# leejaeyong7/tiny-cuda-nn

Measured on AMD Instinct MI355X. Metric: training_step throughput (samples/s) HashGrid+64-wide FFMLP, batch=256k; % fp16-MFMA peak, higher is better.
Workload: dtype f16

## Files before the change

### include/tcnn_amd.h

```cpp
#ifndef TCNN_AMD_H
#define TCNN_AMD_H

#include <stddef.h>
#include <stdint.h>

#ifdef __cplusplus
extern "C" {
#endif

#define TCNN_OK 0
#define TCNN_ERROR 1

#define TCNN_PRECISION_FP32 0
#define TCNN_PRECISION_FP16 1

#define TCNN_GRADIENT_IGNORE 0
#define TCNN_GRADIENT_OVERWRITE 1
#define TCNN_GRADIENT_ACCUMULATE 2

#define TCNN_LAYOUT_SOA 0
#define TCNN_LAYOUT_AOS 1

#define TCNN_LOG_INFO 0
#define TCNN_LOG_DEBUG 1
// ... 55 lines not shown
size_t      tcnn_module_n_params(tcnn_module_t m);
int         tcnn_module_param_precision(tcnn_module_t m);
int         tcnn_module_output_precision(tcnn_module_t m);
int         tcnn_module_initialize_params(tcnn_module_t m, uint64_t seed, float* params_full_precision, float scale);
const char* tcnn_module_hyperparams(tcnn_module_t m);
const char* tcnn_module_name(tcnn_module_t m);

int  tcnn_create_from_config(uint32_t n_input_dims, uint32_t n_output_dims, const char* config_json, tcnn_trainer_t* out);
int  tcnn_create_from_config_seeded(uint32_t n_input_dims, uint32_t n_output_dims, const char* config_json, uint32_t seed, tcnn_trainer_t* out);
int  tcnn_create_from_config_precision(uint32_t n_input_dims, uint32_t n_output_dims, const char* config_json, uint32_t seed, int precision, tcnn_trainer_t* out);
int  tcnn_trainer_precision(tcnn_trainer_t t);
void tcnn_trainer_destroy(tcnn_trainer_t t);

int  tcnn_trainer_training_step(tcnn_trainer_t t, tcnn_stream_t stream, uint32_t n_elements, const float* input, int input_layout,
                                const float* target, const float* data_pdf, int run_optimizer, float* dL_dinput, int use_inference_params,
                                int gradient_mode, const void* external_dL_dy, tcnn_train_ctx_t* ctx_out);
int  tcnn_trainer_loss(tcnn_trainer_t t, tcnn_stream_t stream, tcnn_train_ctx_t ctx, float* loss_out);
int  tcnn_trainer_forward(tcnn_trainer_t t, tcnn_stream_t stream, float loss_scale, uint32_t n_elements, const float* input, int input_layout, const float* target,
                          const float* data_pdf, int use_inference_params, int prepare_input_gradients, const void* external_dL_dy, tcnn_train_ctx_t* ctx_out);
int  tcnn_trainer_backward(tcnn_trainer_t t, tcnn_stream_t stream, tcnn_train_ctx_t ctx, uint32_t n_elements, const float* input, int input_layout,
                           float* dL_dinput, int use_inference_params, int gradient_mode);
int  tcnn_trainer_optimizer_step(tcnn_trainer_t t, tcnn_stream_t stream, float loss_scale);
void tcnn_train_ctx_destroy(tcnn_train_ctx_t ctx);
const void*  tcnn_train_ctx_output(tcnn_train_ctx_t ctx);
const void*  tcnn_train_ctx_dL_doutput(tcnn_train_ctx_t ctx);
const float* tcnn_train_ctx_L(tcnn_train_ctx_t ctx);

int  tcnn_trainer_inference(tcnn_trainer_t t, tcnn_stream_t stream, uint32_t n_elements, const float* input, int input_layout,
                            float* output, int output_layout, int use_inference_params);
int  tcnn_trainer_inference_mixed_precision(tcnn_trainer_t t, tcnn_stream_t stream, uint32_t n_elements, const float* input, int input_layout,
                                            void* output_half, int use_inference_params);

size_t   tcnn_trainer_n_params(tcnn_trainer_t t);
uint32_t tcnn_trainer_padded_output_width(tcnn_trainer_t t);
float*   tcnn_trainer_params_full_precision(tcnn_trainer_t t);
void*    tcnn_trainer_params(tcnn_trainer_t t);
void*    tcnn_trainer_params_inference(tcnn_trainer_t t);
void*    tcnn_trainer_param_gradients(tcnn_trainer_t t);
int      tcnn_trainer_set_params_full_precision(tcnn_trainer_t t, const float* params, size_t n_params, int device_ptr);
int      tcnn_trainer_set_params(tcnn_trainer_t t, const void* params_half, size_t n_params, int device_ptr);
int      tcnn_trainer_initialize_params(tcnn_trainer_t t);
int      tcnn_trainer_update_hyperparams(tcnn_trainer_t t, const char* json);
const char* tcnn_trainer_hyperparams(tcnn_trainer_t t);
int      tcnn_trainer_serialize(tcnn_trainer_t t, int serialize_optimizer, const void** out_bytes, size_t* out_size);
int      tcnn_trainer_deserialize(tcnn_trainer_t t, const void* bytes, size_t size);
const char* tcnn_trainer_network_hyperparams(tcnn_trainer_t t);
uint32_t tcnn_trainer_optimizer_step_count(tcnn_trainer_t t);
int  tcnn_trainer_profile_next_step(tcnn_trainer_t t);
int  tcnn_trainer_profile_collect(tcnn_trainer_t t, tcnn_stream_t stream, float* ms_per_piece , uint32_t* n_steps);
size_t tcnn_trainer_params_updated_in_flush(tcnn_trainer_t t);
size_t tcnn_trainer_image_preps(tcnn_trainer_t t);
size_t tcnn_trainer_scatter_wide_fallbacks(tcnn_trainer_t t);
size_t tcnn_trainer_optimizer_prologue_steps(tcnn_trainer_t t);
size_t tcnn_trainer_list_scatters(tcnn_trainer_t t);
size_t tcnn_module_list_scatters(tcnn_module_t m);
size_t tcnn_trainer_list_gradient_tails(tcnn_trainer_t t);
const char* tcnn_trainer_last_step_kernel(tcnn_trainer_t t);

int   tcnn_module_set_max_level(tcnn_module_t m, float max_level);
float tcnn_module_max_level(tcnn_module_t m);
int   tcnn_module_set_max_level_gpu(tcnn_module_t m, const float* per_sample);
int   tcnn_trainer_set_max_level(tcnn_trainer_t t, float max_level);
int   tcnn_trainer_set_max_level_gpu(tcnn_trainer_t t, const float* per_sample);
float tcnn_trainer_max_level(tcnn_trainer_t t);
int tcnn_train_ctx_keeps_weight_gradient_slabs(tcnn_trainer_t t, tcnn_train_ctx_t ctx);


int         tcnn_module_layer_sizes(tcnn_module_t m, uint32_t* rows_cols, size_t capacity, size_t* n_layers_out);
int         tcnn_optimizer_create(const char* optimizer_json, size_t n_params, const uint32_t* layer_sizes, size_t n_layers, tcnn_optimizer_t* out);
int         tcnn_optimizer_create_precision(const char* optimizer_json, size_t n_params, const uint32_t* layer_sizes, size_t n_layers, int weight_precision, tcnn_optimizer_t* out);
int         tcnn_optimizer_weight_precision(tcnn_optimizer_t o);
void        tcnn_optimizer_destroy(tcnn_optimizer_t o);
int         tcnn_optimizer_step(tcnn_optimizer_t o, tcnn_stream_t stream, float loss_scale, float* params_full_precision, void* params_half,
                                const void* gradients, int gradient_precision);
uint32_t    tcnn_optimizer_step_count(tcnn_optimizer_t o);
size_t      tcnn_optimizer_n_params(tcnn_optimizer_t o);
float       tcnn_optimizer_learning_rate(tcnn_optimizer_t o);
int         tcnn_optimizer_set_learning_rate(tcnn_optimizer_t o, float learning_rate);
int         tcnn_optimizer_update_hyperparams(tcnn_optimizer_t o, const char* json);
const char* tcnn_optimizer_hyperparams(tcnn_optimizer_t o);
void*       tcnn_optimizer_custom_weights(tcnn_optimizer_t o);
int         tcnn_optimizer_weights_restored(tcnn_optimizer_t o, tcnn_stream_t stream, const void* params_half);
int         tcnn_optimizer_serialize(tcnn_optimizer_t o, const void** out_bytes, size_t* out_size);
int         tcnn_optimizer_deserialize(tcnn_optimizer_t o, const void* bytes, size_t size);

#ifdef __cplusplus
}
#endif
#endif
```

### tiny-cuda-nn_amd/csrc/capi.cpp

```cpp
#include "../../include/tcnn_amd.h"

#include "model.h"

#include <mutex>
#include <string>

using namespace tcnn_amd;

namespace {
thread_local std::string g_last_error;
tcnn_amd::Switches g_switches;
std::mutex g_switches_mutex;

bool env_is(const char* name, char c) {
	const char* e = getenv(name);
	return e && e[0] == c;
}
int env_01(const char* name) {
	const char* e = getenv(name);
	return (e && (e[0] == '0' || e[0] == '1')) ? e[0] - '0' : -1;
}

template <typename F>
int guarded(F&& f) {
// ... 22 lines not shown
	std::string name_text;
};

struct tcnn_context_s {
	std::unique_ptr<ModelContext> ctx;
};

struct tcnn_trainer_s {
	std::unique_ptr<Trainer> trainer;
	std::string hyperparams_text;
	std::string network_hyperparams_text;
	std::vector<uint8_t> snapshot;
};

struct tcnn_train_ctx_s {
	std::unique_ptr<TrainContext> ctx;
};

struct tcnn_optimizer_s {
	std::unique_ptr<Optimizer> optimizer;
	size_t n_params = 0;
	std::string hyperparams_text;
	std::vector<uint8_t> snapshot;
};

namespace tcnn_amd {
Switches switches() {
	std::lock_guard<std::mutex> lock{g_switches_mutex};
	return g_switches;
}
void switches_reload() {
	Switches w;
	w.grid_planes = !env_is("TCNN_AMD_GRID_PLANES", '0');
	w.grid_rows_planes = !env_is("TCNN_AMD_GRID_ROWS_PLANES", '0');
	{ const char* e = getenv("TCNN_AMD_GRID_SCATTER"); w.grid_scatter_lds = !(e && std::string{e} == "atomic"); }
	w.scatter_records = !env_is("TCNN_AMD_SCATTER_RECORDS", '0');
	w.scatter_tune = !env_is("TCNN_AMD_SCATTER_TUNE", '0');
	w.scatter_lists = env_01("TCNN_AMD_SCATTER_LISTS");
	w.scatter_wide = env_is("TCNN_AMD_SCATTER_WIDE", '1');
	w.fused_step = !env_is("TCNN_AMD_FUSED_STEP", '0');
	w.side_jobs = !env_is("TCNN_AMD_SIDE_JOBS", '0');
	w.live_image = !env_is("TCNN_AMD_LIVE_IMAGE", '0');
	w.adam_steps32 = env_is("TCNN_AMD_ADAM_STEPS32", '1');
	w.adam_in_reduce = !env_is("TCNN_AMD_ADAM_IN_REDUCE", '0');
	w.adam_prologue = !env_is("TCNN_AMD_ADAM_PROLOGUE", '0');
	w.adam_prologue_refused = env_is("TCNN_AMD_ADAM_PROLOGUE", 'r');
	w.mlp_r32 = !env_is("TCNN_AMD_MLP_R32", '0');
	w.mlp_r32a = env_01("TCNN_AMD_MLP_R32A");
	w.mlp_regs = !env_is("TCNN_AMD_MLP_REGS", '0');
	w.mlp_fast = !env_is("TCNN_AMD_MLP_FAST", '0');
	if (const char* e = getenv("TCNN_AMD_MLP_PRIO")) w.mlp_prio = (uint32_t)atoi(e);
	w.listgrad_in_mlp = !env_is("TCNN_AMD_LISTGRAD_IN_MLP", '0');
	w.mlp_layerwise = env_is("TCNN_AMD_MLP_LAYERWISE", '1');
	std::lock_guard<std::mutex> lock{g_switches_mutex};
	g_switches = w;
}
}

extern "C" {

const char* tcnn_last_error(void) { return g_last_error.c_str(); }
const char* tcnn_version(void) { return "tcnn_amd 0.1 (gfx950)"; }

uint32_t tcnn_batch_size_granularity(void) { return BATCH_SIZE_GRANULARITY; }

int tcnn_device(int* device_out) {
	return guarded([&] { HIP_CHECK_THROW(hipGetDevice(device_out)); });
}

int tcnn_set_device(int device) {
	return guarded([&] { HIP_CHECK_THROW(hipSetDevice(device)); });
}

void tcnn_free_temporary_memory(void) { Arena::instance().release_all(); }

int tcnn_gpu_malloc(size_t bytes, void** out) {
	return guarded([&] {
		CHECK_THROW(out != nullptr);
		*out = nullptr;
		if (bytes) HIP_CHECK_THROW(hipMalloc(out, bytes));
	});
}
int tcnn_gpu_free(void* ptr) {
	return guarded([&] { if (ptr) HIP_CHECK_THROW(hipFree(ptr)); });
}
int tcnn_gpu_memcpy(void* dst, const void* src, size_t bytes, int kind) {
	return guarded([&] {
		const hipMemcpyKind k = kind == TCNN_MEMCPY_HOST_TO_DEVICE ? hipMemcpyHostToDevice : kind == TCNN_MEMCPY_DEVICE_TO_HOST ? hipMemcpyDeviceToHost : hipMemcpyDeviceToDevice;
		if (bytes) HIP_CHECK_THROW(hipMemcpy(dst, src, bytes, k));
	});
}
int tcnn_gpu_memset(void* ptr, int value, size_t bytes) {
	return guarded([&] { if (bytes) HIP_CHECK_THROW(hipMemset(ptr, value, bytes)); });
}
int tcnn_stream_synchronize(tcnn_stream_t stream) {
	return guarded([&] { HIP_CHECK_THROW(hipStreamSynchronize((hipStream_t)stream)); });
}
int tcnn_generate_random_uniform(tcnn_stream_t stream, uint64_t rng_state_inc[2], size_t n, float* out, float lower, float upper) {
	return guarded([&] {
		CHECK_THROW(rng_state_inc != nullptr && (out != nullptr || n == 0));
		generate_random_uniform((hipStream_t)stream, rng_state_inc, n, out, lower, upper);
		HIP_CHECK_THROW(hipGetLastError());
	});
}
int tcnn_has_networks(void) { return 1; }
float tcnn_default_loss_scale(int precision) { return precision == TCNN_PRECISION_FP32 ? 1.0f : LOSS_SCALE_FP16; }
// ... 206 lines not shown

int tcnn_trainer_backward(tcnn_trainer_t t, tcnn_stream_t stream, tcnn_train_ctx_t ctx, uint32_t n, const float* input, int input_layout, float* dL_dinput,
                          int use_inference_params, int gradient_mode) {
	return guarded([&] {
		CHECK_THROW(t && t->trainer && ctx && ctx->ctx);
		Trainer& tr = *t->trainer;
		const uint32_t w = tr.model().input_width();
		MatViewMut dx = make_view_mut(dL_dinput, w, n, input_layout);
		tr.backward((hipStream_t)stream, *ctx->ctx, n, make_view(input, w, n, input_layout), dL_dinput ? &dx : nullptr, use_inference_params != 0, (GradientMode)gradient_mode);
	});
}

int tcnn_trainer_optimizer_step(tcnn_trainer_t t, tcnn_stream_t stream, float loss_scale) {
	return guarded([&] {
		CHECK_THROW(t && t->trainer);
		t->trainer->optimizer_step((hipStream_t)stream, loss_scale);
	});
}

void tcnn_train_ctx_destroy(tcnn_train_ctx_t ctx) { delete ctx; }
const void* tcnn_train_ctx_output(tcnn_train_ctx_t ctx) { return ctx->ctx->output.data(); }
const void* tcnn_train_ctx_dL_doutput(tcnn_train_ctx_t ctx) {
	if (guarded([&] { ctx->ctx->materialize(); }) != 0) return nullptr;
	return ctx->ctx->dL_doutput_ptr;
}
const float* tcnn_train_ctx_L(tcnn_train_ctx_t ctx) {
	if (guarded([&] { ctx->ctx->materialize(); }) != 0) return nullptr;
	return ctx->ctx->L.as<float>();
}

int tcnn_trainer_inference(tcnn_trainer_t t, tcnn_stream_t stream, uint32_t n, const float* input, int input_layout, float* output, int output_layout, int use_inference_params) {
	return guarded([&] {
		CHECK_THROW(t && t->trainer);
		Trainer& tr = *t->trainer;
		tr.inference((hipStream_t)stream, n, make_view(input, tr.model().input_width(), n, input_layout), make_view_mut(output, tr.model().output_width(), n, output_layout),
		             use_inference_params != 0);
	});
}

int tcnn_trainer_inference_mixed_precision(tcnn_trainer_t t, tcnn_stream_t stream, uint32_t n, const float* input, int input_layout, void* output_half, int use_inference_params) {
	return guarded([&] {
		CHECK_THROW(t && t->trainer && (output_half || n == 0));
		Trainer& tr = *t->trainer;
		tr.inference_mixed_precision((hipStream_t)stream, n, make_view(input, tr.model().input_width(), n, input_layout), output_half, use_inference_params != 0);
	});
}

size_t tcnn_trainer_n_params(tcnn_trainer_t t) { return t->trainer->n_params(); }
size_t tcnn_trainer_params_updated_in_flush(tcnn_trainer_t t) { return t->trainer->params_updated_in_flush(); }
size_t tcnn_trainer_image_preps(tcnn_trainer_t t) { return t->trainer->image_preps(); }
size_t tcnn_trainer_optimizer_prologue_steps(tcnn_trainer_t t) {
	try { return (size_t)t->trainer->prologue_steps(); } catch (const std::exception& e) { g_last_error = e.what(); return (size_t)-1; }
}
size_t tcnn_trainer_scatter_wide_fallbacks(tcnn_trainer_t t) {
	try { return (size_t)t->trainer->scatter_wide_fallbacks(); } catch (const std::exception& e) { g_last_error = e.what(); return (size_t)-1; }
}
size_t tcnn_trainer_list_scatters(tcnn_trainer_t t) { return (size_t)t->trainer->list_scatters(); }
size_t tcnn_trainer_list_gradient_tails(tcnn_trainer_t t) { return (size_t)t->trainer->list_gradient_tails(); }
const char* tcnn_trainer_last_step_kernel(tcnn_trainer_t t) { return t->trainer->last_step_kernel(); }
int tcnn_trainer_set_max_level(tcnn_trainer_t t, float max_level) {
	return guarded([&] {
		CHECK_THROW(t && t->trainer);
		if (!t->trainer->model().set_max_level(max_level)) no_grid(t->trainer->model());
	});
}
int tcnn_trainer_set_max_level_gpu(tcnn_trainer_t t, const float* per_sample) {
	return guarded([&] {
		CHECK_THROW(t && t->trainer);
		if (!t->trainer->model().set_max_level_gpu(per_sample)) no_grid(t->trainer->model());
	});
}
float tcnn_trainer_max_level(tcnn_trainer_t t) {
	float v = std::numeric_limits<float>::quiet_NaN();
	const float* per_sample = nullptr;
	guarded([&] {
		CHECK_THROW(t && t->trainer);
		if (!t->trainer->model().get_max_level(v, per_sample)) no_grid(t->trainer->model());
		g_last_error.clear();
	});
	return v;
}
int tcnn_train_ctx_keeps_weight_gradient_slabs(tcnn_trainer_t t, tcnn_train_ctx_t ctx) {
	return (t && ctx && ctx->ctx && ctx->ctx->model_ctx && t->trainer->model().context_keeps_slabs(*ctx->ctx->model_ctx)) ? 1 : 0;
}
uint32_t tcnn_trainer_padded_output_width(tcnn_trainer_t t) { return t->trainer->model().padded_output_width(); }
float* tcnn_trainer_params_full_precision(tcnn_trainer_t t) { return t->trainer->params_full_precision(); }
void* tcnn_trainer_params(tcnn_trainer_t t) { return t->trainer->params(); }
void* tcnn_trainer_params_inference(tcnn_trainer_t t) {
	void* p = t->trainer->params_inference();
	return p == t->trainer->params_unexposed() ? t->trainer->params() : p;
}
void* tcnn_trainer_param_gradients(tcnn_trainer_t t) { return t->trainer->param_gradients(); }

int tcnn_trainer_set_params_full_precision(tcnn_trainer_t t, const float* params, size_t n_params, int device_ptr) {
	return guarded([&] { t->trainer->set_params_full_precision(params, n_params, device_ptr != 0); });
}

int tcnn_trainer_set_params(tcnn_trainer_t t, const void* params_half, size_t n_params, int device_ptr) {
	return guarded([&] { t->trainer->set_params(params_half, n_params, device_ptr != 0); });
}

int tcnn_trainer_initialize_params(tcnn_trainer_t t) {
	return guarded([&] { t->trainer->initialize_params(); });
}

int tcnn_trainer_update_hyperparams(tcnn_trainer_t t, const char* json) {
	return guarded([&] { t->trainer->update_hyperparams(parse_or_empty(json)); });
}

const char* tcnn_trainer_hyperparams(tcnn_trainer_t t) {
	t->hyperparams_text = t->trainer->hyperparams().dump();
	return t->hyperparams_text.c_str();
}

const char* tcnn_trainer_network_hyperparams(tcnn_trainer_t t) {
	t->network_hyperparams_text = t->trainer->model().hyperparams().dump();
	return t->network_hyperparams_text.c_str();
}

uint32_t tcnn_trainer_optimizer_step_count(tcnn_trainer_t t) { return t->trainer->optimizer().step_count(); }

int tcnn_trainer_profile_next_step(tcnn_trainer_t t) {
	return guarded([&] {
		CHECK_THROW(t && t->trainer);
		t->trainer->profile().arm();
	});
}

int tcnn_trainer_profile_collect(tcnn_trainer_t t, tcnn_stream_t stream, float* ms_per_piece, uint32_t* n_steps) {
	return guarded([&] {
		CHECK_THROW(t && t->trainer && ms_per_piece && n_steps);
		*n_steps = t->trainer->profile().collect((hipStream_t)stream, ms_per_piece);
	});
}

int tcnn_trainer_serialize(tcnn_trainer_t t, int serialize_optimizer, const void** out_bytes, size_t* out_size) {
	return guarded([&] {
		CHECK_THROW(out_bytes != nullptr && out_size != nullptr);
		t->snapshot = Json::to_msgpack(t->trainer->serialize(serialize_optimizer != 0));
		*out_bytes = t->snapshot.data();
		*out_size = t->snapshot.size();
	});
}

int tcnn_trainer_deserialize(tcnn_trainer_t t, const void* bytes, size_t size) {
	return guarded([&] {
		CHECK_THROW(bytes != nullptr && size > 0);
		t->trainer->deserialize(Json::from_msgpack((const uint8_t*)bytes, size));
	});
}

int tcnn_module_layer_sizes(tcnn_module_t m, uint32_t* rows_cols, size_t capacity, size_t* n_layers_out) {
	return guarded([&] {
		CHECK_THROW(m && m->model && n_layers_out && (rows_cols || capacity == 0));
		const auto sizes = m->model->layer_sizes();
		*n_layers_out = sizes.size();
		for (size_t i = 0; i < sizes.size() && i < capacity; ++i) {
			rows_cols[2 * i] = sizes[i].first;
			rows_cols[2 * i + 1] = sizes[i].second;
		}
	});
}

int tcnn_optimizer_create(const char* optimizer_json, size_t n_params, const uint32_t* layer_sizes, size_t n_layers, tcnn_optimizer_t* out) {
	return tcnn_optimizer_create_precision(optimizer_json, n_params, layer_sizes, n_layers, TCNN_PRECISION_FP16, out);
}

int tcnn_optimizer_weight_precision(tcnn_optimizer_t o) {
	int v = -1;
	guarded([&] { CHECK_THROW(o && o->optimizer); v = (int)o->optimizer->weight_precision(); });
	return v;
}

int tcnn_optimizer_create_precision(const char* optimizer_json, size_t n_params, const uint32_t* layer_sizes, size_t n_layers, int weight_precision, tcnn_optimizer_t* out) {
	switches_reload();
	return guarded([&] {
		CHECK_THROW(out != nullptr && (layer_sizes != nullptr || n_layers == 0));
		if (weight_precision != TCNN_PRECISION_FP32 && weight_precision != TCNN_PRECISION_FP16) throw std::runtime_error{"Unknown precision " + std::to_string(weight_precision)};
		auto o = std::make_unique<tcnn_optimizer_s>();
		o->optimizer = create_optimizer(parse_or_empty(optimizer_json));
		std::vector<std::pair<uint32_t, uint32_t>> sizes;
		size_t n_matrix = 0;
		for (size_t i = 0; i < n_layers; ++i) {
			sizes.emplace_back(layer_sizes[2 * i], layer_sizes[2 * i + 1]);
			n_matrix += (size_t)layer_sizes[2 * i] * layer_sizes[2 * i + 1];
// ... 91 lines not shown
```

### tiny-cuda-nn_amd/csrc/k_grid_planes.hip

```cpp
#include "grid_device.h"
#include "mlp_side_jobs.h"

#include <algorithm>
#include <cstdio>
#include <cstdlib>
#include <vector>

namespace tcnn_amd {
namespace {

constexpr int FP_THREADS = 128;
#ifndef TCNN_FP_LIST_THREADS
#define TCNN_FP_LIST_THREADS 256
#endif
constexpr int FP_LIST_THREADS = TCNN_FP_LIST_THREADS;

constexpr int FP_MAX_CHUNKS = GRID_FILTER_MAX_CHUNKS;
constexpr int FP_PER_LANE = FP_MAX_CHUNKS / 64;

template <int D, int F, int FP_SPT, bool LISTS>
__global__ void __launch_bounds__(LISTS ? FP_LIST_THREADS : FP_THREADS) k_grid_fwd_planes(
	const GridMeta* __restrict__ meta, const uint32_t* __restrict__ work, const uint32_t max_items, const uint32_t blocks_per_xcd, const uint32_t n, const MatView x,
	const half_t* __restrict__ grid, half_t* __restrict__ out, unsigned long long* __restrict__ bits, const MlpPrepJob prep, const GridHitLists lists
) {
// ... 290 lines not shown
						for (int k = 0; k < FP_SPT; ++k) if (base + k * 64 < n) dst[k] = mine[k];
					}
				}
			}
		}
	}
}

template <int D, int F, int SPT>
void launch_planes(hipStream_t s, const GridMeta* dm, const uint32_t* work, uint32_t max_items, uint32_t blocks_per_xcd, uint32_t n, MatView x, const void* grid, void* out, uint64_t* bits,
                   const MlpPrepJob* prep_job, const GridHitLists* hit_lists) {
	MlpPrepJob prep{};
	if (prep_job) prep = *prep_job;
	if (hit_lists) {
		if constexpr (SPT == 8) throw std::runtime_error{"grid_forward_planes: hit lists come from the 2- and 4-samples-per-thread shapes"};
		else
		hipLaunchKernelGGL((k_grid_fwd_planes<D, F, SPT, true>), dim3(8 * blocks_per_xcd), dim3(FP_LIST_THREADS), 0, s, dm, work, max_items, blocks_per_xcd, n, x, (const half_t*)grid, (half_t*)out,
		                   nullptr, prep, *hit_lists);
	} else {
		hipLaunchKernelGGL((k_grid_fwd_planes<D, F, SPT, false>), dim3(8 * blocks_per_xcd), dim3(FP_THREADS), 0, s, dm, work, max_items, blocks_per_xcd, n, x, (const half_t*)grid, (half_t*)out,
		                   (unsigned long long*)bits, prep, GridHitLists{});
	}
	HIP_CHECK_THROW(hipGetLastError());
}

uint32_t max_scatter_chunks(const GridMeta& meta) {
	uint32_t m = 1;
	for (uint32_t l = 0; l < meta.n_levels; ++l) m = std::max(m, meta.levels[l].scatter_n_chunks);
	return m;
}

}

uint32_t grid_hit_item_samples(const GridMeta& meta) { return FP_LIST_THREADS * grid_planes_spt(meta); }

uint32_t grid_planes_spt(const GridMeta& meta) {
	uint32_t forced = 0;
#ifdef TCNN_AMD_DEV
	static const uint32_t dev_forced = getenv("TCNN_AMD_FWD_SPT") ? (uint32_t)atoi(getenv("TCNN_AMD_FWD_SPT")) : 0u;
	forced = dev_forced;
#endif
	if (max_scatter_chunks(meta) > (uint32_t)FP_MAX_CHUNKS) return 2u;
	if (forced == 8 || forced == 4 || forced == 2) return forced;
	if (meta.n_pos_dims == 3 && grid_scatter_prefers_lists(meta)) return 2u;
	return 4u;
}

bool grid_planes_supported(const GridMeta& meta, uint32_t n) {
	const uint32_t F = meta.n_features_per_level;
	return (F == 2 || F == 4 || F == 8) && (meta.n_pos_dims == 2 || meta.n_pos_dims == 3) && meta.n_levels < 256 && n % 64 == 0 && n > 0 &&
	       div_round_up(n, FP_THREADS * grid_planes_spt(meta)) < (1u << 24);
}

void grid_planes_plan(const GridMeta& meta, uint32_t n, bool hit_lists, std::vector<uint32_t>& work, uint32_t& max_items, uint32_t& blocks_per_xcd) {
	const uint32_t threads = hit_lists ? FP_LIST_THREADS : FP_THREADS;
	const uint32_t items_per_level = div_round_up(n, threads * grid_planes_spt(meta));
	float coarse_cost = 0.6f;
#ifdef TCNN_AMD_DEV
	if (const char* e = getenv("TCNN_AMD_FWD_COARSE_COST")) coarse_cost = (float)atof(e);
#endif
	std::vector<float> cost(meta.n_levels);
	double total = 0;
	for (uint32_t l = 0; l < meta.n_levels; ++l) {
		const size_t bytes = (size_t)meta.levels[l].size * meta.n_features_per_level * 2;
		cost[l] = bytes > (256u << 10) ? 1.0f : coarse_cost;
		total += (double)cost[l] * items_per_level;
	}
	uint32_t dbg_lo = 0, dbg_hi = meta.n_levels;
#ifdef TCNN_AMD_DEV
	if (const char* e = getenv("TCNN_AMD_FWD_LEVELS")) sscanf(e, "%u,%u", &dbg_lo, &dbg_hi);
#endif
	(void)total;
	size_t wide_bytes = (size_t)4 << 20;
#ifdef TCNN_AMD_DEV
	if (const char* e = getenv("TCNN_AMD_FWD_WIDE_MB")) wide_bytes = (size_t)std::max(atoi(e), 0) << 20;
#endif
	auto is_wide = [&](uint32_t l) { return wide_bytes > 0 && (size_t)meta.levels[l].size * meta.n_features_per_level * 2 > wide_bytes; };
	double narrow_total = 0;
	for (uint32_t l = 0; l < meta.n_levels; ++l) if (l >= dbg_lo && l <= dbg_hi && !is_wide(l)) narrow_total += (double)cost[l] * items_per_level;
	std::vector<std::vector<uint32_t>> runs(8);
	double acc = 0;
	for (uint32_t l = 0; l < meta.n_levels; ++l) {
		if (l < dbg_lo || l > dbg_hi || is_wide(l)) continue;
		for (uint32_t i = 0; i < items_per_level; ++i) {
			const uint32_t bin = std::min<uint32_t>((uint32_t)((acc + 0.5 * cost[l]) * 8.0 / narrow_total), 7u);
			runs[bin].push_back(l << 24 | i);
			acc += cost[l];
		}
	}
	{
		size_t longest = 0;
		for (auto& r : runs) longest = std::max(longest, r.size());
		uint32_t next = 0;
		for (uint32_t l = 0; l < meta.n_levels; ++l) {
			if (l < dbg_lo || l > dbg_hi || !is_wide(l)) continue;
			for (uint32_t i = 0; i < items_per_level; ++i) {
				size_t best = next % 8;
				for (size_t b = 0; b < 8; ++b) if (runs[b].size() < runs[best].size()) best = b;
				runs[best].push_back(l << 24 | i);
				++next;
			}
		}
		(void)longest;
	}
	max_items = 0;
	for (auto& r : runs) max_items = std::max<uint32_t>(max_items, (uint32_t)r.size());
	work.assign(8 + (size_t)8 * max_items, 0xffffffffu);
	for (uint32_t b = 0; b < 8; ++b) {
		work[b] = (uint32_t)runs[b].size();
		std::copy(runs[b].begin(), runs[b].end(), work.begin() + 8 + (size_t)b * max_items);
	}
	blocks_per_xcd = std::max(1u, std::min(256u * FP_THREADS / threads, max_items));
#ifdef TCNN_AMD_DEV
	if (const char* e = getenv("TCNN_AMD_FWD_BLOCKS_PER_XCD")) blocks_per_xcd = std::max(1, atoi(e));
#endif
}

void grid_forward_planes(hipStream_t stream, const GridMeta& meta, const GridMeta* dev_meta, const uint32_t* dev_work, uint32_t max_items, uint32_t blocks_per_xcd, uint32_t n,
                         MatView x, const void* grid, void* out_planes, uint64_t* chunk_bits, const MlpPrepJob* prep_job, const GridHitLists* hit_lists) {
	CHECK_THROW(grid_planes_supported(meta, n));
	CHECK_THROW(!hit_lists || (hit_lists->elems && hit_lists->heads && hit_lists->stragglers && hit_lists->counts && n <= grid_hit_max_samples(meta) &&
// ... 74 lines not shown
```

### tiny-cuda-nn_amd/csrc/k_misc.hip

```cpp
#include "tcnn_common.h"
#include "adam_device.h"
#include "grid_fixed.h"
#include "mlp_side_jobs.h"
#include "oneblob_device.h"

#include <hip/hip_fp16.h>

#include <cmath>
#include <limits>

namespace tcnn_amd {
namespace {

typedef _Float16 half_t;
typedef _Float16 h8 __attribute__((ext_vector_type(8)));
typedef _Float16 h4 __attribute__((ext_vector_type(4)));

template <typename T>
__global__ void __launch_bounds__(256) k_oneblob_fwd(const uint32_t n, const uint32_t n_dims, const uint32_t log2_bins, const MatView x, T* __restrict__ out, const uint32_t out_stride) {
	const uint32_t gid = blockIdx.x * blockDim.x + threadIdx.x;
	const uint32_t i = gid / out_stride;
	if (i >= n) return;
	const uint32_t j = gid - i * out_stride;
	const uint32_t n_bins = 1u << log2_bins;
// ... 677 lines not shown
	hipLaunchKernelGGL(k_adam_widen_steps, dim3(blocks_for(n, 256)), dim3(256), 0, stream, n, (const uint16_t*)steps16, (uint32_t*)steps32);
}

void adam_step(hipStream_t stream, const AdamHyper& h, size_t n, size_t n_matrix, float loss_scale, uint32_t current_step,
               float* w_fp, void* w_half, const void* gradients, float* m1, float* m2, void* steps, bool steps16, const float* debias_table, GradientPrecision precision, Precision weight_precision) {
	if (n == 0) return;
	const AdamArgs a = make_adam_args(h, loss_scale, current_step);
	if (weight_precision == Precision::Fp32) {
		CHECK_THROW(precision == GradientPrecision::Fp32);
		adam_launch_steps(stream, a, n, n_matrix, w_fp, (float*)nullptr, (const float*)gradients, m1, m2, steps, steps16, debias_table);
	} else if (precision == GradientPrecision::Fp32) adam_launch_steps(stream, a, n, n_matrix, w_fp, (half_t*)w_half, (const float*)gradients, m1, m2, steps, steps16, debias_table);
	else adam_launch_steps(stream, a, n, n_matrix, w_fp, (half_t*)w_half, (const half_t*)gradients, m1, m2, steps, steps16, debias_table);
}

namespace {
constexpr uint32_t PRO_THREADS = SLAB_REDUCE_ELEMS * SLAB_REDUCE_GROUPS;
constexpr uint32_t PRO_MAX_BLOCKS_PER_RANGE = 64;
__host__ __device__ inline uint32_t pro_range_blocks(const uint32_t n_elems) { return min(PRO_MAX_BLOCKS_PER_RANGE, max(1u, (n_elems / 4 + PRO_THREADS - 1) / PRO_THREADS)); }

template <typename STEP_T, typename DebiasOf>
__device__ inline void adam_quad(const AdamArgs& a, DebiasOf&& from_table, const float debias, const bool quad_matrix, const size_t i4, const h4 gv,
                                 float* __restrict__ w_fp, half_t* __restrict__ w, float* __restrict__ m1, float* __restrict__ m2, STEP_T* __restrict__ steps) {
	if (!quad_matrix && gv[0] == (half_t)0.0f && gv[1] == (half_t)0.0f && gv[2] == (half_t)0.0f && gv[3] == (half_t)0.0f) return;
	float4 wf = *(const float4*)(w_fp + i4), a1 = *(const float4*)(m1 + i4), a2 = *(const float4*)(m2 + i4);
	uint4 st = adam_load_steps(steps + i4);
	half_t wh[4];
	bool up[4];
	adam_one(a, from_table, debias, quad_matrix, gv[0], wf.x, wh[0], a1.x, a2.x, st.x, up[0]);
	adam_one(a, from_table, debias, quad_matrix, gv[1], wf.y, wh[1], a1.y, a2.y, st.y, up[1]);
	adam_one(a, from_table, debias, quad_matrix, gv[2], wf.z, wh[2], a1.z, a2.z, st.z, up[2]);
	adam_one(a, from_table, debias, quad_matrix, gv[3], wf.w, wh[3], a1.w, a2.w, st.w, up[3]);
	*(float4*)(w_fp + i4) = wf;
	*(float4*)(m1 + i4) = a1;
	*(float4*)(m2 + i4) = a2;
	adam_store_steps(steps + i4, st);
	if (up[0] && up[1] && up[2] && up[3]) {
		*(h4*)(w + i4) = h4{wh[0], wh[1], wh[2], wh[3]};
	} else {
#pragma unroll
		for (int e = 0; e < 4; ++e) if (up[e]) w[i4 + e] = wh[e];
	}
}

struct PrologueArgs {
	uint32_t n_reduce_blocks, reduce_elems, reduce_slabs;
	int reduce_accumulate;
	const float* slabs;
	const GridScatterRange* ranges;
	uint32_t n_ranges, n_range_blocks;
	int accumulate;
	unsigned long long* scratch;
	size_t range_base;
	size_t bulk_begin;
};

#ifndef TCNN_PRO_BOUNDS
#define TCNN_PRO_BOUNDS __launch_bounds__(PRO_THREADS)
#endif
#ifndef TCNN_PRO_Q
#define TCNN_PRO_Q 1
#endif
constexpr int PRO_Q = TCNN_PRO_Q;
template <typename STEP_T>
__global__ void TCNN_PRO_BOUNDS k_adam_prologue(const AdamArgs a, const size_t n, const size_t n_matrix, float* __restrict__ w_fp, half_t* __restrict__ w, half_t* __restrict__ g,
                                                               float* __restrict__ m1, float* __restrict__ m2, STEP_T* __restrict__ steps, const float* __restrict__ debias_table, const PrologueArgs p) {
	__shared__ float part[SLAB_REDUCE_GROUPS * SLAB_REDUCE_ELEMS];
	const float debias = debias_table[a.common_step];
	const auto from_table = [&](const uint32_t t) { return debias_table[t]; };
	const uint32_t tid = threadIdx.x;
	if (blockIdx.x < p.n_reduce_blocks) {
		const uint32_t e = tid & (SLAB_REDUCE_ELEMS - 1), grp = tid / SLAB_REDUCE_ELEMS;
		const uint32_t i = blockIdx.x * SLAB_REDUCE_ELEMS + e;
		float q[4] = {0, 0, 0, 0};
		if (i < p.reduce_elems) {
			uint32_t k = grp;
			for (; k + 3 * SLAB_REDUCE_GROUPS < p.reduce_slabs; k += 4 * SLAB_REDUCE_GROUPS) {
#pragma unroll
				for (int u = 0; u < 4; ++u) q[u] += p.slabs[(size_t)(k + u * SLAB_REDUCE_GROUPS) * p.reduce_elems + i];
			}
			for (; k < p.reduce_slabs; k += SLAB_REDUCE_GROUPS) q[0] += p.slabs[(size_t)k * p.reduce_elems + i];
		}
		part[grp * SLAB_REDUCE_ELEMS + e] = (q[0] + q[1]) + (q[2] + q[3]);
		__syncthreads();
		if (grp == 0 && i < p.reduce_elems) {
			float s = 0;
#pragma unroll
			for (int gi = 0; gi < SLAB_REDUCE_GROUPS; ++gi) s += part[gi * SLAB_REDUCE_ELEMS + e];
			if (p.reduce_accumulate) s += (float)g[i];
			const half_t gh = (half_t)s;
			g[i] = gh;
			bool up;
			half_t wh;
			uint32_t st1 = steps[i];
			adam_one(a, from_table, debias, i < n_matrix, gh, w_fp[i], wh, m1[i], m2[i], st1, up);
			steps[i] = (STEP_T)st1;
			if (up) w[i] = wh;
		}
		return;
	}
	const uint32_t b = blockIdx.x - p.n_reduce_blocks;
	if (b < p.n_range_blocks) {
		uint32_t ri = 0, first = 0;
		for (uint32_t nb = pro_range_blocks(p.ranges[0].n_elems); b >= first + nb; nb = pro_range_blocks(p.ranges[ri].n_elems)) { first += nb; ++ri; }
		const GridScatterRange r = p.ranges[ri];
		const uint32_t my = b - first, of = pro_range_blocks(r.n_elems);
		typedef unsigned long long u64x2 __attribute__((ext_vector_type(2)));
		u64x2* sc = (u64x2*)(p.scratch + r.scratch_begin);
		const size_t g0 = p.range_base + r.grad_begin;
		for (uint32_t quad = my * PRO_THREADS + tid; quad < r.n_elems / 4; quad += of * PRO_THREADS) {
			const u64x2 lo = sc[2 * quad], hi = sc[2 * quad + 1];
			sc[2 * quad] = u64x2{0, 0};
			sc[2 * quad + 1] = u64x2{0, 0};
			long long s[4] = {(long long)lo.x, (long long)lo.y, (long long)hi.x, (long long)hi.y};
			const size_t i4 = g0 + 4 * (size_t)quad;
			if (p.accumulate) {
				const h4 old = *(const h4*)(g + i4);
#pragma unroll
				for (int e = 0; e < 4; ++e) s[e] += half_to_fixed(old[e]);
			}
			const h4 gv = h4{fixed_to_half(s[0]), fixed_to_half(s[1]), fixed_to_half(s[2]), fixed_to_half(s[3])};
			*(h4*)(g + i4) = gv;
			adam_quad(a, from_table, debias, i4 < n_matrix, i4, gv, w_fp, w, m1, m2, steps);
		}
		return;
	}
	h4 gv[PRO_Q];
	bool live[PRO_Q];
#pragma unroll
	for (int k = 0; k < PRO_Q; ++k) {
		const size_t i4 = p.bulk_begin + (((size_t)(b - p.n_range_blocks) * PRO_Q + k) * PRO_THREADS + tid) * 4;
		live[k] = i4 < n;
		for (uint32_t r = 0; r < p.n_ranges; ++r) {
			const size_t rb = p.range_base + p.ranges[r].grad_begin;
			if (i4 >= rb && i4 < rb + p.ranges[r].n_elems) live[k] = false;
		}
		if (live[k]) gv[k] = *(const h4*)(g + i4);
	}
#pragma unroll
	for (int k = 0; k < PRO_Q; ++k) {
		const size_t i4 = p.bulk_begin + (((size_t)(b - p.n_range_blocks) * PRO_Q + k) * PRO_THREADS + tid) * 4;
		if (live[k]) adam_quad(a, from_table, debias, i4 < n_matrix, i4, gv[k], w_fp, w, m1, m2, steps);
	}
}
}

bool adam_step_with_prologue(hipStream_t stream, const AdamHyper& h, size_t n, size_t n_matrix, float loss_scale, uint32_t current_step,
                             float* w_fp, void* w_half, void* g_half, float* m1, float* m2, void* steps, bool steps16, const float* debias_table, const AdamPrologue& pro) {
	const auto aligned = [](const void* ptr, size_t bytes) { return ((uintptr_t)ptr & (bytes - 1)) == 0; };
	if (n == 0 || !(aligned(w_fp, 16) && aligned(m1, 16) && aligned(m2, 16) && aligned(steps, steps16 ? 8 : 16) && aligned(w_half, 8) && aligned(g_half, 8))) return false;
	PrologueArgs p{};
	p.bulk_begin = 0;
	if (pro.has_reduce) {
		if (pro.reduce_elems % 4 != 0 || pro.reduce_elems > n || n_matrix % 4 != 0) return false;
		p.n_reduce_blocks = div_round_up(pro.reduce_elems, (uint32_t)SLAB_REDUCE_ELEMS);
		p.reduce_elems = pro.reduce_elems;
		p.reduce_slabs = pro.reduce_slabs;
		p.reduce_accumulate = pro.reduce_accumulate;
		p.slabs = pro.slabs;
		p.bulk_begin = pro.reduce_elems;
	} else if (n_matrix % 4 != 0) return false;
	if ((n - p.bulk_begin) % 4 != 0) return false;
	if (!pro.ranges.empty()) {
		if ((const char*)pro.grad_base < (const char*)g_half || !aligned(pro.scratch, 16)) return false;
		p.range_base = (size_t)((const half_t*)pro.grad_base - (const half_t*)g_half);
		if (p.range_base % 4 != 0) return false;
		for (const GridScatterRange& r : pro.ranges) {
			if (r.grad_begin % 4 != 0 || r.n_elems % 4 != 0 || r.scratch_begin % 2 != 0 || p.range_base + r.grad_begin + r.n_elems > n || p.range_base + r.grad_begin < p.bulk_begin) return false;
		}
		for (bool moved = true; moved;) {
			moved = false;
			for (const GridScatterRange& r : pro.ranges) {
				if (r.n_elems && p.range_base + r.grad_begin == p.bulk_begin) { p.bulk_begin += r.n_elems; moved = true; }
			}
		}
		p.ranges = pro.dev_ranges;
		p.n_ranges = (uint32_t)pro.ranges.size();
		for (const GridScatterRange& r : pro.ranges) p.n_range_blocks += pro_range_blocks(r.n_elems);
		p.scratch = (unsigned long long*)pro.scratch;
		p.accumulate = pro.accumulate ? 1 : 0;
	}
	const AdamArgs a = make_adam_args(h, loss_scale, current_step);
	const uint32_t bulk_blocks = div_round_up((uint32_t)((n - p.bulk_begin) / 4), PRO_THREADS * (uint32_t)PRO_Q);
	const dim3 grid(p.n_reduce_blocks + p.n_range_blocks + bulk_blocks);
	if (steps16) hipLaunchKernelGGL(k_adam_prologue<uint16_t>, grid, dim3(PRO_THREADS), 0, stream, a, n, n_matrix, w_fp, (half_t*)w_half, (half_t*)g_half, m1, m2, (uint16_t*)steps, debias_table, p);
	else hipLaunchKernelGGL(k_adam_prologue<uint32_t>, grid, dim3(PRO_THREADS), 0, stream, a, n, n_matrix, w_fp, (half_t*)w_half, (half_t*)g_half, m1, m2, (uint32_t*)steps, debias_table, p);
	HIP_CHECK_THROW(hipGetLastError());
	return true;
}

void adam_fill_debias_table(hipStream_t stream, float beta1, float beta2, uint32_t from, uint32_t to, float* table) {
	if (to <= from) return;
	hipLaunchKernelGGL(k_adam_debias_table, dim3(blocks_for(to - from, 256)), dim3(256), 0, stream, beta1, beta2, from, to, table);
}

namespace {
template <typename G, typename W>
__global__ void __launch_bounds__(256) k_sgd(const size_t n, const float loss_scale, const float learning_rate, const float l2_reg, float* __restrict__ w_fp, W* __restrict__ w,
                                             const G* __restrict__ g) {
	const size_t i = (size_t)blockIdx.x * blockDim.x + threadIdx.x;
	if (i >= n) return;
	const float weight_fp = w_fp[i];
	float gradient = (float)g[i] / loss_scale;
	gradient += l2_reg * weight_fp;
	const float new_weight = weight_fp - learning_rate * gradient;
	w_fp[i] = new_weight;
	if constexpr (sizeof(W) == 2) w[i] = (W)new_weight;
}

template <typename W>
__global__ void __launch_bounds__(256) k_ema(const size_t n, const float decay, const float debias_old, const float debias_new, const W* __restrict__ weights, W* __restrict__ weights_ema,
                                             float* __restrict__ tmp) {
	const size_t i = (size_t)blockIdx.x * blockDim.x + threadIdx.x;
	if (i >= n) return;
	const float previous = tmp ? tmp[i] : (float)weights_ema[i];
	const float filtered = (previous * decay * debias_old + (float)weights[i] * (1 - decay)) * debias_new;
	if (tmp) tmp[i] = filtered;
	weights_ema[i] = (W)filtered;
}
template <typename W>
__global__ void __launch_bounds__(256) k_average_step(const size_t n, const uint32_t n_samples, const W* __restrict__ weights, W* __restrict__ current, W* __restrict__ average) {
	const size_t i = (size_t)blockIdx.x * blockDim.x + threadIdx.x;
	if (i >= n) return;
	const W weight = weights[i];
	average[i] = (W)((float)average[i] + ((float)weight - (float)current[i]) / (float)n_samples);
	current[i] = weight;
}
template <typename G>
__global__ void __launch_bounds__(256) k_batched_accumulate(const size_t n, const int first, const uint32_t multiplier, const G* __restrict__ gradients, float* __restrict__ pool) {
	const size_t i = (size_t)blockIdx.x * blockDim.x + threadIdx.x;
	if (i >= n) return;
	float v = first ? 0.0f : pool[i];
	v += (float)gradients[i] / (float)multiplier;
	pool[i] = v;
}
template <typename G>
__global__ void __launch_bounds__(1024) k_novo_second_moment(const size_t n, const float loss_scale, const float beta2, const G* __restrict__ gradients, float* __restrict__ moment) {
	__shared__ float part[1024];
	float acc = 0.0f;
	for (size_t i = threadIdx.x; i < n; i += 1024) {
		const float g = (float)gradients[i];
// ... 159 lines not shown
```

### tiny-cuda-nn_amd/csrc/model.h

```cpp
#pragma once

#include "json_lite.h"
#include "tcnn_common.h"
#include "mlp_side_jobs.h"

#include <algorithm>
#include <cctype>
#include <cstdio>
#include <cmath>
#include <cstring>
#include <functional>
#include <limits>
#include <map>
#include <memory>
#include <mutex>
#include <numeric>
#include <random>
#include <unordered_map>
#include <vector>

namespace tcnn_amd {

struct LogSink {
	void (*callback)(int, const char*, void*) = nullptr;
// ... 131 lines not shown
	template <typename T> T* as() const { return (T*)m_ptr; }
	size_t bytes() const { return m_bytes; }
private:
	void* m_ptr = nullptr;
	size_t m_bytes = 0;
};

struct Pcg32 {
	uint64_t st[2] = {0x853c49e6748fea9bULL, 0xda3e39cb94b95bdbULL};
	static constexpr uint64_t MULT = 0x5851f42d4c957f2dULL;
	Pcg32() = default;
	explicit Pcg32(uint64_t initstate, uint64_t initseq = 1) {
		st[0] = 0;
		st[1] = (initseq << 1u) | 1u;
		next_uint();
		st[0] += initstate;
		next_uint();
	}
	uint32_t next_uint() {
		const uint64_t old = st[0];
		st[0] = old * MULT + st[1];
		const uint32_t xorshifted = (uint32_t)(((old >> 18u) ^ old) >> 27u);
		const uint32_t rot = (uint32_t)(old >> 59u);
		return (xorshifted >> rot) | (xorshifted << ((~rot + 1u) & 31));
	}
	float next_float() {
		const uint32_t u = (next_uint() >> 9) | 0x3f800000u;
		float f;
		memcpy(&f, &u, 4);
		return f - 1.0f;
	}
};

struct EncodingContext {
	ArenaBuf to_reduce;
	ArenaBuf dy_dx;
	ArenaBuf chunk_mask;
	ArenaBuf hit_elems;
	GridHitLists hit_lists;
	uint64_t hit_generation = 0;
	const void* hit_stream = nullptr;
	uint32_t n = 0;
	GridForwardRoute route;
	std::vector<EncodingContext> nested;
};

struct BackwardHandoff {
	const MlpReduceJob* reduce_job = nullptr;
	AdamPrologue* prologue = nullptr;
	void* list_gradients = nullptr;
	bool reduce_carried = false;
};

struct ForwardPlan {
	GridForwardRoute route;
	const MlpPrepJob* prep_job = nullptr;
	const GridItemMap* item_map = nullptr;
};

class Encoding {
public:
	virtual ~Encoding() {}
	virtual uint32_t input_width() const = 0;
	virtual uint32_t output_width() const = 0;
	uint32_t padded_output_width() const { return output_width() + m_n_to_pad; }
	virtual uint32_t required_output_alignment() const { return 1; }
	virtual void set_padded_output_width(uint32_t padded) {
		CHECK_THROW(padded >= output_width());
		m_n_to_pad = padded - output_width();
	}
	void set_alignment(uint32_t alignment) {
		const uint32_t a = std::lcm(alignment, required_output_alignment());
		set_padded_output_width(next_multiple(output_width(), a));
	}
	virtual size_t n_params() const { return 0; }
	virtual void initialize_params(Pcg32& rng, float* params_full_precision, float scale) {}
	virtual EncodingContext forward(hipStream_t stream, uint32_t n, MatView x, const void* params, void* out, bool prepare_input_gradients, bool prepare_param_gradients, const ForwardPlan* plan = nullptr) = 0;
	virtual void backward(hipStream_t stream, const EncodingContext& ctx, uint32_t n, MatView x, const void* dL_dy, MatViewMut* dL_dx, const void* params, void* grads, GradientMode mode, const GridBackwardRoute& route, BackwardHandoff* handoff = nullptr) = 0;
	virtual GridBackwardRoute backward_route(const Switches& sw, hipStream_t stream, const EncodingContext& ctx, uint32_t n, MatView x, GridDyForm offer, bool want_dL_dx, GradientMode mode) { return {}; }
	void backward_rows(hipStream_t stream, const EncodingContext& ctx, uint32_t n, MatView x, const void* dL_dy, MatViewMut* dL_dx, const void* params, void* grads, GradientMode mode) {
		backward(stream, ctx, n, x, dL_dy, dL_dx, params, grads, mode, backward_route(switches(), stream, ctx, n, x, GridDyForm::Rows, dL_dx != nullptr, mode));
	}
	virtual void backward_backward_input(hipStream_t stream, const EncodingContext& ctx, uint32_t n, MatView x, MatView dL_ddLdx, const void* dL_dy, void* dL_ddLdy,
	                                     MatViewMut* dL_dx, const void* params, void* grads, GradientMode mode) {
		throw std::runtime_error{"DifferentiableObject::backward_backward_input_impl: not implemented error"};
	}
	virtual bool has_second_order() const { return false; }
	virtual bool second_order_reads_dL_dy() const { return true; }
	virtual bool as_identity(float& scale, float& offset) const { return false; }
	virtual uint32_t as_oneblob() const { return 0; }
	virtual uint64_t scatter_wide_fallbacks() { return 0; }
	virtual uint64_t list_scatters() const { return 0; }
	virtual GridForwardRoute forward_route(const Switches& sw, uint32_t n, bool as_planes, bool prepare_input_gradients, bool prepare_param_gradients) const { return {}; }
	virtual Json hyperparams() const = 0;
	bool fp32() const { return m_fp32; }
	virtual bool set_max_level(float max_level) { return false; }
	virtual bool set_max_level_gpu(const float* per_sample) { return false; }
	virtual bool get_max_level(float& max_level, const float*& per_sample) const { return false; }
protected:
	explicit Encoding(bool fp32) : m_fp32{fp32} {}
	bool m_fp32;
	uint32_t m_n_to_pad = 0;
};

inline GridType string_to_grid_type(const std::string& s) {
	if (equals_case_insensitive(s, "Hash")) return GridType::Hash;
	if (equals_case_insensitive(s, "Dense")) return GridType::Dense;
	if (equals_case_insensitive(s, "Tiled") || equals_case_insensitive(s, "Tile")) return GridType::Tiled;
	throw std::runtime_error{"Invalid grid type: " + s};
}
inline HashType string_to_hash_type(const std::string& s) {
	if (equals_case_insensitive(s, "Prime")) return HashType::Prime;
	if (equals_case_insensitive(s, "CoherentPrime")) return HashType::CoherentPrime;
	if (equals_case_insensitive(s, "ReversedPrime")) return HashType::ReversedPrime;
	if (equals_case_insensitive(s, "Rng")) return HashType::Rng;
	throw std::runtime_error{"Invalid hash type: " + s};
}
inline InterpolationType string_to_interpolation_type(const std::string& s) {
	if (equals_case_insensitive(s, "Nearest")) return InterpolationType::Nearest;
	if (equals_case_insensitive(s, "Linear")) return InterpolationType::Linear;
	if (equals_case_insensitive(s, "Smoothstep")) return InterpolationType::Smoothstep;
	throw std::runtime_error{"Invalid interpolation type: " + s};
}

class GridEncoding : public Encoding {
public:
	GridEncoding(uint32_t n_dims_to_encode, const Json& enc, bool fp32) : Encoding{fp32} {
		const uint32_t F = enc.value("n_features_per_level", 2u);
		if (F != 1 && F != 2 && F != 4 && F != 8) throw std::runtime_error{"GridEncoding: n_features_per_level must be 1, 2, 4, or 8."};
		const uint32_t log2_hashmap_size = enc.value("log2_hashmap_size", 19u);
		const std::string encoding_type = enc.value("otype", "Grid");
		const std::string default_type = equals_case_insensitive(encoding_type, "TiledGrid") ? "Tiled" : (equals_case_insensitive(encoding_type, "DenseGrid") ? "Dense" : "Hash");
		uint32_t n_features;
		if (enc.contains("n_features") || enc.contains("n_grid_features")) {
			n_features = enc.contains("n_features") ? enc.value("n_features", 0u) : enc.value("n_grid_features", 0u);
			if (enc.contains("n_levels")) throw std::runtime_error{"GridEncoding: may not specify n_features and n_levels simultaneously (one determines the other)"};
		} else {
			n_features = F * enc.value("n_levels", 16u);
		}
		const uint32_t n_levels = n_features / F;
		const GridType grid_type = string_to_grid_type(enc.value("type", default_type));
		const uint32_t base_resolution = enc.value("base_resolution", 16u);
		const float per_level_scale = enc.value("per_level_scale", grid_type == GridType::Dense ? std::exp(std::log(256.0f / (float)base_resolution) / (n_levels - 1)) : 2.0f);
		const HashType hash_type = string_to_hash_type(enc.value("hash", "CoherentPrime"));
		m_stochastic_interpolation = enc.value("stochastic_interpolation", false);
		if (m_stochastic_interpolation) throw std::runtime_error{"GridEncoding: stochastic_interpolation is not supported by this build"};
// ... 35 lines not shown
			lv.size = params_in_level;
			lv.scale = scale;
			uint32_t stride = 1;
			for (uint32_t d = 0; d < 4; ++d) lv.stride[d] = 0;
			for (uint32_t d = 0; d < n_dims_to_encode && stride <= params_in_level; ++d) {
				lv.stride[d] = stride;
				stride *= resolution;
			}
			lv.hashed = (grid_type == GridType::Hash && params_in_level < stride) ? 1u : 0u;
			lv.size_mask = (params_in_level & (params_in_level - 1)) == 0 ? params_in_level - 1 : 0;
			m_resolutions.push_back(resolution);
			offset += params_in_level;
		}
		m_n_entries = offset;
		m_n_params = (size_t)offset * F;
		if (F >= 2) {
			grid_scatter_setup_levels(m_meta);
			for (uint32_t i = 0; i < n_levels; ++i) {
				m_scatter_levels_ok &= m_meta.levels[i].scatter_binned || m_meta.levels[i].scatter_n_chunks <= grid_scatter_max_chunks();
				m_any_binned |= m_meta.levels[i].scatter_binned != 0;
			}
		}
	}

	const GridMeta* dev_meta() {
		if (!m_dev_meta.data()) {
			m_dev_meta.resize(sizeof(GridMeta));
			HIP_CHECK_THROW(hipMemcpy(m_dev_meta.data(), &m_meta, sizeof(GridMeta), hipMemcpyHostToDevice));
		}
		return (const GridMeta*)m_dev_meta.data();
	}

	static uint32_t powi(uint32_t base, uint32_t exponent) {
		uint32_t result = 1;
		for (uint32_t i = 0; i < exponent; ++i) result *= base;
		return result;
	}

	uint32_t input_width() const override { return m_meta.n_pos_dims; }
	uint32_t output_width() const override { return m_n_features; }
	uint32_t required_output_alignment() const override { return m_meta.n_features_per_level; }
	size_t n_params() const override { return m_n_params; }
	const GridMeta& meta() const { return m_meta; }
	const std::vector<uint32_t>& resolutions() const { return m_resolutions; }

	void initialize_params(Pcg32& rng, float* params_full_precision, float scale) override {
		generate_random_uniform(nullptr, rng.st, n_params(), params_full_precision, -1e-4f * scale, 1e-4f * scale);
	}

	EncodingContext forward(hipStream_t stream, uint32_t n, MatView x, const void* params, void* out, bool prepare_input_gradients, bool prepare_param_gradients, const ForwardPlan* plan) override {
		EncodingContext ctx;
		if ((!out && !prepare_input_gradients) || padded_output_width() == 0 || n == 0) return ctx;
		const GridForwardRoute route = plan ? plan->route : forward_route(switches(), n, false, prepare_input_gradients, prepare_param_gradients);
		if (route.kernel == GridForwardKernel::Planes) return forward_planes(stream, route, n, x, params, out, plan->prep_job, plan->item_map);
		if (route.kernel == GridForwardKernel::PlanesToRows) {
			ArenaBuf planes{stream, (size_t)n * padded_output_width() * sizeof(uint16_t)};
			ctx = forward_planes(stream, route, n, x, params, planes.data());
			grid_planes_to_rows(stream, m_meta, n, padded_output_width(), planes.data(), out, padded_output_width());
			return ctx;
		}
		ctx.route = route;
		if (prepare_input_gradients) ctx.dy_dx = ArenaBuf{stream, (size_t)n * m_n_features * m_meta.n_pos_dims * sizeof(float)};
		const bool want_filter = route.recorded == GridRecorded::BitPlanes;
		ArenaBuf mask;
		if (want_filter) mask = ArenaBuf{stream, (size_t)m_meta.n_levels * n * (GRID_FILTER_MAX_CHUNKS / 64) * sizeof(uint64_t)};
		grid_forward(stream, m_meta, dev_meta(), m_fp32, n, x, params, out, padded_output_width(), ctx.dy_dx.as<float>(), mask.as<uint64_t>());
		if (max_level_forward_active()) {
			const uint32_t F = m_meta.n_features_per_level, D = m_meta.n_pos_dims;
			if (out) zero_levels(stream, m_fp32 ? 4 : 2, n, F, padded_output_width(), F, out, false);
			if (ctx.dy_dx) zero_levels(stream, 4, n, F * D, (uint64_t)m_n_features * D, (uint64_t)F * D, ctx.dy_dx.data(), false);
		}
		if (want_filter) {
			ctx.chunk_mask = ArenaBuf{stream, (size_t)m_meta.n_levels * grid_scatter_max_chunks() * (n / 64) * sizeof(uint64_t)};
			ctx.n = n;
			grid_mask_to_bits(stream, m_meta, dev_meta(), n, mask.as<uint64_t>(), ctx.chunk_mask.as<uint64_t>());
		}
		return ctx;
	}

	GridFacts facts() const { return GridFacts{&m_meta, m_fp32, m_scatter_levels_ok, m_any_binned, m_n_to_pad}; }
	GridForwardRoute forward_route(const Switches& sw, uint32_t n, bool as_planes, bool prepare_input_gradients, bool prepare_param_gradients) const override {
		return grid_forward_route(facts(), sw, n, as_planes, prepare_input_gradients, prepare_param_gradients);
	}

	struct PlanesPlan {
		DeviceBuf dev_work;
		uint32_t max_items = 0, blocks_per_xcd = 0;
	};
	PlanesPlan& planes_plan(uint32_t n_, bool hit_lists) {
		const uint32_t n = n_ | (hit_lists ? 0x80000000u : 0u);
		auto it = m_planes_plans.find(n);
		if (it != m_planes_plans.end()) return *it->second;
		auto plan = std::make_unique<PlanesPlan>();
		std::vector<uint32_t> work;
		grid_planes_plan(m_meta, n_, hit_lists, work, plan->max_items, plan->blocks_per_xcd);
		plan->dev_work.resize(work.size() * sizeof(uint32_t));
		HIP_CHECK_THROW(hipMemcpy(plan->dev_work.data(), work.data(), work.size() * sizeof(uint32_t), hipMemcpyHostToDevice));
		return *(m_planes_plans[n] = std::move(plan));
	}

	EncodingContext forward_planes(hipStream_t stream, const GridForwardRoute& route, uint32_t n, MatView x, const void* params, void* out_planes,
	                               const MlpPrepJob* prep_job = nullptr, const GridItemMap* item_map = nullptr) {
		EncodingContext ctx;
		CHECK_THROW(route.planned && route.kernel != GridForwardKernel::Rows);
		ctx.route = route;
		const bool want_lists = route.recorded == GridRecorded::HitLists;
		if (want_lists) {
			HitCounters& hc = hit_counters(stream);
			GridHitLists& hl = ctx.hit_lists;
			hl.item_samples = grid_hit_item_samples(m_meta);
			hl.n_items = div_round_up(n, hl.item_samples);
			hl.item_capacity = hl.item_samples << (m_meta.n_pos_dims - 1);
			hl.straggler_capacity = n << (m_meta.n_pos_dims - 1);
			hl.map = grid_item_map(hl.item_samples, 0, 1);
			if (item_map && item_map->n_windows > 1 && item_map->window * item_map->n_windows == hl.item_samples && n % hl.item_samples == 0 &&
			    item_map->stride == hl.n_items * item_map->window && item_map->window % (64 * grid_planes_spt(m_meta)) == 0) hl.map = *item_map;
			const size_t L = m_meta.n_levels;
			const size_t elems_bytes = L * hl.n_items * hl.item_capacity * GRID_HIT_WORDS * sizeof(uint32_t), sidx_bytes = next_multiple_sz(L * hl.n_items * hl.item_capacity * sizeof(uint16_t), 256);
			const size_t heads_bytes = next_multiple_sz(L * hl.n_items * GRID_HIT_HEADS * sizeof(uint32_t), 256);
			ctx.hit_elems = ArenaBuf{stream, elems_bytes + sidx_bytes + heads_bytes + L * hl.straggler_capacity * 2 * sizeof(uint32_t)};
			hl.elems = ctx.hit_elems.as<uint32_t>();
			hl.sidx = (uint16_t*)((char*)ctx.hit_elems.data() + elems_bytes);
			hl.heads = (uint32_t*)((char*)ctx.hit_elems.data() + elems_bytes + sidx_bytes);
			hl.stragglers = (uint32_t*)((char*)ctx.hit_elems.data() + elems_bytes + sidx_bytes + heads_bytes);
			hl.counts = hc.sets[hc.next].as<uint32_t>();
			hl.zero_counts = hc.sets[hc.next ^ 1].as<uint32_t>();
			hc.next ^= 1;
#ifdef TCNN_AMD_DEV
			if (const char* e = getenv("TCNN_AMD_FWD_LISTS_DEV")) hl.dev_flags = (uint32_t)atoi(e);
#endif
			ctx.hit_generation = ++hc.generation;
			ctx.hit_stream = (const void*)stream;
			ctx.n = n;
		} else if (route.recorded == GridRecorded::BitPlanes) {
			ctx.chunk_mask = ArenaBuf{stream, (size_t)m_meta.n_levels * grid_scatter_max_chunks() * (n / 64) * sizeof(uint64_t)};
			ctx.n = n;
		}
		PlanesPlan& plan = planes_plan(n, want_lists);
		grid_forward_planes(stream, m_meta, dev_meta(), plan.dev_work.as<uint32_t>(), plan.max_items, plan.blocks_per_xcd, n, x, params, out_planes, ctx.chunk_mask.as<uint64_t>(), prep_job,
		                    want_lists ? &ctx.hit_lists : nullptr);
		if (m_n_to_pad) HIP_CHECK_THROW(hipMemsetAsync((uint16_t*)out_planes + (size_t)n * m_n_features, 0, (size_t)n * m_n_to_pad * sizeof(uint16_t), stream));
		if (max_level_forward_active()) {
			const uint32_t F = m_meta.n_features_per_level;
			zero_levels(stream, 2, n, F, F, (uint64_t)n * F, out_planes, false);
		}
		return ctx;
	}

	bool lists_current(hipStream_t stream, const EncodingContext& ctx, uint32_t n) { return ctx.hit_elems && ctx.n == n && ctx.hit_stream == (const void*)stream && hit_counters(stream).generation == ctx.hit_generation; }
	GridMaxLevel max_level_state() const { return m_max_level_gpu ? GridMaxLevel::PerSample : (levels_on(true) < m_meta.n_levels ? GridMaxLevel::Scalar : GridMaxLevel::None); }
	GridBackwardRoute backward_route(const Switches& sw, hipStream_t stream, const EncodingContext& ctx, uint32_t n, MatView x, GridDyForm offer, bool want_dL_dx, GradientMode mode) override {
		GridBackwardRoute r = grid_backward_route(facts(), sw, ctx.route, lists_current(stream, ctx, n), n, offer, want_dL_dx, mode, max_level_state(), x.stride_dim == 1 && x.stride_sample == m_meta.n_pos_dims);
		const GridHitLists& hl = ctx.hit_lists;
		r.tail = r.tail && hl.map.n_windows >= 2 && hl.n_items * hl.item_samples == n;
		if (r.tail) {
			r.list_tail.sidx = hl.sidx, r.list_tail.heads = hl.heads, r.list_tail.map = hl.map;
			r.list_tail.n_items = hl.n_items, r.list_tail.item_capacity = hl.item_capacity;
			r.tail_bytes = grid_list_gradients_bytes(m_meta, hl);
		}
		return r;
	}

	void backward(hipStream_t stream, const EncodingContext& ctx, uint32_t n, MatView x, const void* dL_dy, MatViewMut* dL_dx, const void* params, void* grads, GradientMode mode, const GridBackwardRoute& route, BackwardHandoff* handoff) override {
		if ((!dL_dx && mode == GradientMode::Ignore) || n == 0) return;
		const BackwardHandoff offer = handoff ? *handoff : BackwardHandoff{};
		const auto all_levels = [&](const void* dy) {
			const bool carried = backward_all_levels(stream, ctx, n, x, dy, dL_dx, params, grads, mode, route, offer);
			if (handoff) handoff->reduce_carried = carried;
		};
		const GridMaxLevel max_level = max_level_state();
		if (max_level == GridMaxLevel::None) return all_levels(dL_dy);
		if (max_level == GridMaxLevel::PerSample) {
			const uint32_t F = m_meta.n_features_per_level;
			const bool dy_planes = route.dy == GridDyForm::Planes;
			const size_t elem = dy_planes ? 2 : (m_fp32 ? 4 : 2);
			ArenaBuf masked{stream, (size_t)n * padded_output_width() * elem};
			zero_levels(stream, elem, n, F, dy_planes ? F : padded_output_width(), dy_planes ? (uint64_t)n * F : F, masked.data(), true, dL_dy);
			return all_levels(masked.data());
		}
		GradientTail tail{*this, stream, grads, mode, levels_on(true)};
		all_levels(dL_dy);
		tail.settle();
	}

	bool backward_all_levels(hipStream_t stream, const EncodingContext& ctx, uint32_t n, MatView x, const void* dL_dy, MatViewMut* dL_dx, const void* params, void* grads, GradientMode mode,
	                         const GridBackwardRoute& route, const BackwardHandoff& offer) {
		const uint32_t F = m_meta.n_features_per_level;
		const bool dy_planes = route.dy != GridDyForm::Rows, accumulate = mode == GradientMode::Accumulate;
		uint32_t dy_stride_sample = dy_planes ? F : padded_output_width(), dy_stride_level = dy_planes ? n * F : F;
		bool carried = false;
		if (mode != GradientMode::Ignore) CHECK_THROW(grads != nullptr && route.kernel != GridGradientKernel::None);
		switch (mode == GradientMode::Ignore ? GridGradientKernel::None : route.kernel) {
		case GridGradientKernel::None: break;
// ... 211 lines not shown
private:
	void zero_levels(hipStream_t stream, size_t elem_bytes, uint32_t n, uint32_t width, uint64_t sample_stride, uint64_t level_stride, void* data, bool gradient_rule,
	                 const void* src = nullptr) const {
		const uint32_t level0 = m_max_level_gpu ? 0u : levels_on(gradient_rule);
		grid_zero_levels(stream, elem_bytes, n, m_meta.n_levels, level0, width, sample_stride, level_stride, data, src, m_max_level_gpu, m_n_features, m_meta.n_features_per_level, gradient_rule);
	}
	struct GradientTail {
		hipStream_t stream;
		char* tail = nullptr;
		size_t bytes = 0;
		bool accumulate = false;
		ArenaBuf saved;
		GradientTail(const GridEncoding& e, hipStream_t s, void* grads, GradientMode mode, uint32_t l_bwd) : stream{s} {
			if (!grads || mode == GradientMode::Ignore || l_bwd >= e.m_meta.n_levels) return;
			const size_t elem = e.m_fp32 ? 4 : 2, first = (size_t)e.m_meta.levels[l_bwd].offset * e.m_meta.n_features_per_level;
			tail = (char*)grads + first * elem;
			bytes = (e.n_params() - first) * elem;
			accumulate = mode == GradientMode::Accumulate;
			if (accumulate) {
				saved = ArenaBuf{stream, bytes};
				HIP_CHECK_THROW(hipMemcpyAsync(saved.data(), tail, bytes, hipMemcpyDeviceToDevice, stream));
			}
		}
		void settle() {
			if (!tail) return;
			if (accumulate) HIP_CHECK_THROW(hipMemcpyAsync(tail, saved.data(), bytes, hipMemcpyDeviceToDevice, stream));
			else HIP_CHECK_THROW(hipMemsetAsync(tail, 0, bytes, stream));
		}
	};

public:
	Json hyperparams() const override {
		static const char* types[] = {"Hash", "Dense", "Tiled"};
		static const char* interps[] = {"Nearest", "Linear", "Smoothstep"};
		static const char* hashes[] = {"Prime", "CoherentPrime", "ReversedPrime", "Rng"};
		Json j = Json::object();
		j["otype"] = "Grid";
		j["type"] = types[m_meta.grid_type];
		j["n_levels"] = m_meta.n_levels;
		j["n_features_per_level"] = m_meta.n_features_per_level;
		j["base_resolution"] = m_base_resolution;
		j["per_level_scale"] = m_per_level_scale;
		j["interpolation"] = interps[m_meta.interpolation];
		j["hash"] = hashes[m_meta.hash_type];
		if (m_meta.grid_type == (uint32_t)GridType::Hash) j["log2_hashmap_size"] = m_log2_hashmap_size;
		return j;
	}

private:
	GridMeta m_meta;
	DeviceBuf m_dev_meta;
	std::map<std::pair<uint32_t, const void*>, std::unique_ptr<ScatterPlan>> m_scatter_plans;
	std::map<const void*, std::unique_ptr<HitCounters>> m_hit_counters;
	std::map<uint32_t, std::unique_ptr<PlanesPlan>> m_planes_plans;
	bool m_scatter_levels_ok = true;
	bool m_any_binned = false;
	uint64_t m_list_scatters = 0;
	float m_max_level = 1000.f;
	const float* m_max_level_gpu = nullptr;
	std::vector<uint32_t> m_resolutions;
	uint32_t m_n_features, m_log2_hashmap_size, m_base_resolution, m_n_entries;
	float m_per_level_scale;
	bool m_stochastic_interpolation;
	size_t m_n_params;
};

class OneBlobEncoding : public Encoding {
public:
	OneBlobEncoding(uint32_t n_bins, uint32_t n_dims_to_encode, bool fp32) : Encoding{fp32}, m_n_bins{n_bins}, m_n_dims{n_dims_to_encode} {
		if ((n_bins & (n_bins - 1)) != 0 || n_bins == 0) throw std::runtime_error{"Number of bins must be a power of 2"};
	}
	uint32_t input_width() const override { return m_n_dims; }
	uint32_t output_width() const override { return m_n_dims * m_n_bins; }
	uint32_t as_oneblob() const override {
		const char* e = getenv("TCNN_AMD_FUSE_ONEBLOB");
		return (!m_fp32 && m_n_bins >= 32 && !(e && e[0] == '0')) ? m_n_bins : 0;
	}
	EncodingContext forward(hipStream_t stream, uint32_t n, MatView x, const void* params, void* out, bool prepare_input_gradients, bool prepare_param_gradients, const ForwardPlan* plan) override {
		if (out && padded_output_width() > 0) oneblob_forward(stream, m_fp32, n, m_n_dims, m_n_bins, x, out, padded_output_width());
		return {};
	}
	void backward(hipStream_t stream, const EncodingContext& ctx, uint32_t n, MatView x, const void* dL_dy, MatViewMut* dL_dx, const void* params, void* grads, GradientMode mode, const GridBackwardRoute&, BackwardHandoff*) override {
		if (!dL_dx) return;
		oneblob_backward_input(stream, m_fp32, n, m_n_dims, m_n_bins, x, dL_dy, padded_output_width(), *dL_dx);
	}
	Json hyperparams() const override {
		Json j = Json::object();
		j["otype"] = "OneBlob";
		j["n_bins"] = m_n_bins;
		return j;
	}
private:
	uint32_t m_n_bins, m_n_dims;
};

inline void zero_input_gradient(hipStream_t stream, uint32_t n, uint32_t n_dims, const MatViewMut& dL_dx) {
	if (n == 0 || n_dims == 0) return;
	const bool aos = dL_dx.stride_dim == 1 && dL_dx.stride_sample == n_dims, soa = dL_dx.stride_sample == 1 && dL_dx.stride_dim == n;
	if (aos || soa) {
		HIP_CHECK_THROW(hipMemsetAsync(dL_dx.data, 0, (size_t)n * n_dims * sizeof(float), stream));
	} else {
		for (uint32_t d = 0; d < n_dims; ++d) {
			HIP_CHECK_THROW(hipMemset2DAsync(dL_dx.data + (size_t)d * dL_dx.stride_dim, (size_t)dL_dx.stride_sample * sizeof(float), 0, sizeof(float), n, stream));
		}
	}
}

// ... 1045 lines not shown
	Activation m_activation, m_output_activation;
	MlpDesc m_desc;
	size_t m_n_params;
	mutable LiveImage m_live;
	mutable int m_live_state = 0;
};

struct ModelContext {
	virtual ~ModelContext() {}
};

class Model {
public:
	virtual ~Model() {}
	virtual uint32_t input_width() const = 0;
	virtual uint32_t output_width() const = 0;
	virtual uint32_t padded_output_width() const = 0;
	virtual size_t n_params() const = 0;
	virtual Precision precision() const = 0;
	virtual std::vector<std::pair<uint32_t, uint32_t>> layer_sizes() const = 0;
	virtual void initialize_params(Pcg32& rng, float* params_full_precision, float scale) = 0;
	virtual uint64_t list_scatters() const { return 0; }
	virtual uint64_t list_gradient_tails() const { return 0; }
	virtual Encoding* input_encoding() { return nullptr; }
	bool set_max_level(float max_level) { Encoding* e = input_encoding(); return e && e->set_max_level(max_level); }
	bool set_max_level_gpu(const float* per_sample) { Encoding* e = input_encoding(); return e && e->set_max_level_gpu(per_sample); }
	bool get_max_level(float& max_level, const float*& per_sample) { Encoding* e = input_encoding(); return e && e->get_max_level(max_level, per_sample); }
	virtual void inference(hipStream_t stream, uint32_t n, MatView input, void* output, const void* params) = 0;
	virtual void inference_f32(hipStream_t stream, uint32_t n, MatView input, MatViewMut output, const void* params) {
		check_batch(n);
		if (n == 0) return;
		const uint32_t pw = padded_output_width();
		ArenaBuf tmp{stream, (size_t)n * pw * (precision() == Precision::Fp32 ? 4 : 2)};
		inference(stream, n, input, tmp.data(), params);
		trim_and_cast(stream, precision() == Precision::Fp32, n, pw, output_width(), tmp.data(), output);
	}
	virtual std::unique_ptr<ModelContext> forward(hipStream_t stream, uint32_t n, MatView input, void* output, const void* params, bool prepare_input_gradients) = 0;
	virtual void backward(hipStream_t stream, const ModelContext& ctx, uint32_t n, MatView input, const void* output, const void* dL_doutput,
	                      MatViewMut* dL_dinput, const void* params, void* gradients, GradientMode mode) = 0;
	virtual void backward_backward_input(hipStream_t stream, const ModelContext& ctx, uint32_t n, MatView input, MatView dL_ddLdinput, const void* dL_doutput,
	                                     void* dL_ddLdoutput, MatViewMut* dL_dinput, const void* params, void* gradients, GradientMode mode) {
		throw std::runtime_error{"DifferentiableObject::backward_backward_input_impl: not implemented error"};
	}
	virtual Json hyperparams() const = 0;
	std::string name() const { return hyperparams().value("otype", "<Unknown>"); }

	static void check_batch(uint32_t n) {
		if (n % BATCH_SIZE_GRANULARITY != 0) throw std::runtime_error{"batch size " + std::to_string(n) + " is not a multiple of BATCH_SIZE_GRANULARITY = 256"};
	}
};

struct StepProfile {
	enum Piece { Encode = 0, MlpKernel = 1, EncodingBackward = 2, Optimizer = 3, N_PIECES = 4 };
	struct Sample { hipEvent_t begin[N_PIECES], end[N_PIECES]; bool used[N_PIECES]; };
	std::vector<Sample> samples;
	bool armed = false;
	Sample* current = nullptr;

	void arm() { armed = true; }
	void begin_step() {
		current = nullptr;
		if (!armed) return;
		armed = false;
		samples.emplace_back();
		current = &samples.back();
		for (int i = 0; i < N_PIECES; ++i) {
			current->used[i] = false;
			HIP_CHECK_THROW(hipEventCreateWithFlags(&current->begin[i], 0x20000000u));
			HIP_CHECK_THROW(hipEventCreateWithFlags(&current->end[i], 0x20000000u));
		}
	}
	void mark(hipStream_t stream, Piece p, bool end) {
		if (!current) return;
		HIP_CHECK_THROW(hipEventRecord(end ? current->end[p] : current->begin[p], stream));
		if (end) current->used[p] = true;
	}
	void end_step() { current = nullptr; }
	uint32_t collect(hipStream_t stream, float* ms) {
		HIP_CHECK_THROW(hipStreamSynchronize(stream));
		for (int i = 0; i < N_PIECES; ++i) ms[i] = 0.0f;
		for (Sample& s : samples) {
			for (int i = 0; i < N_PIECES; ++i) {
				float t = 0.0f;
				if (s.used[i]) HIP_CHECK_THROW(hipEventElapsedTime(&t, s.begin[i], s.end[i]));
				ms[i] += t;
				(void)hipEventDestroy(s.begin[i]);
				(void)hipEventDestroy(s.end[i]);
			}
		}
		const uint32_t n = (uint32_t)samples.size();
		samples.clear();
		return n;
	}
	~StepProfile() {
		for (Sample& s : samples)
			for (int i = 0; i < N_PIECES; ++i) {
				(void)hipEventDestroy(s.begin[i]);
				(void)hipEventDestroy(s.end[i]);
			}
	}
};

struct FusedStepData {
	const float* target = nullptr;
	const float* data_pdf = nullptr;
	const void* external_dL_dy = nullptr;
	LossType loss = LossType::L2;
	float loss_scale = 1.0f;
	void* out = nullptr;
	void* dL_dout = nullptr;
	float* L = nullptr;
	bool compact_context = false;
	MatViewMut* dL_dinput = nullptr;
	const void* params = nullptr;
	void* gradients = nullptr;
	GradientMode mode = GradientMode::Overwrite;
	StepProfile* profile = nullptr;
};
enum class OptimizerPlace { None, InReduce, Prologue, OwnLaunch };
struct OptimizerOffer {
	const AdamInReduce* in_reduce = nullptr;
	AdamPrologue* prologue = nullptr;
};

class NetworkWithInputEncoding : public Model {
public:
	NetworkWithInputEncoding(uint32_t n_dims_to_encode, uint32_t n_output_dims, const Json& encoding, const Json& network, Precision precision = Precision::Fp16) {
		m_encoding = create_encoding(n_dims_to_encode, encoding, Network::REQUIRED_ALIGNMENT, precision == Precision::Fp32);
		Json local = network.is_object() ? network : Json::object();
		local["n_input_dims"] = m_encoding->padded_output_width();
		local["n_output_dims"] = n_output_dims;
		m_network.reset(new Network{local, precision});
	}

	uint32_t input_width() const override { return m_encoding->input_width(); }
	uint32_t output_width() const override { return m_network->output_width(); }
	uint32_t padded_output_width() const override { return m_network->padded_output_width(); }
	size_t n_params() const override { return m_network->n_params() + m_encoding->n_params(); }
	Precision precision() const override { return m_network->precision(); }
	std::vector<std::pair<uint32_t, uint32_t>> layer_sizes() const override { return m_network->layer_sizes(); }
	Encoding& encoding() { return *m_encoding; }
	Encoding* input_encoding() override { return m_encoding.get(); }
	Network& network() { return *m_network; }

	void initialize_params(Pcg32& rng, float* params_full_precision, float scale) override {
		m_network->initialize_params(rng, params_full_precision, scale);
		m_encoding->initialize_params(rng, params_full_precision + m_network->n_params(), scale);
	}

	void inference(hipStream_t stream, uint32_t n, MatView input, void* output, const void* params) override {
		inference_fused(stream, n, input, output, nullptr, params);
	}
	void inference_f32(hipStream_t stream, uint32_t n, MatView input, MatViewMut output, const void* params) override {
		inference_fused(stream, n, input, nullptr, &output, params);
	}

	void inference_fused(hipStream_t stream, uint32_t n, MatView input, void* output_half, const MatViewMut* output_f32, const void* params) {
		check_batch(n);
		if (n == 0) return;
		const _Float16* p = (const _Float16*)params;
		if (m_network->layerwise()) {
			ArenaBuf network_input{stream, (size_t)n * m_encoding->padded_output_width() * elem()}, out_tmp;
			m_encoding->forward(stream, n, input, encoding_params(params), network_input.data(), false, false);
			if (!output_half) out_tmp = ArenaBuf{stream, (size_t)n * m_network->padded_output_width() * elem()};
			m_network->inference(stream, n, network_input.data(), output_half ? output_half : out_tmp.data(), params);
			if (output_f32) trim_and_cast(stream, elem() == 4, n, m_network->padded_output_width(), m_network->output_width(), output_half ? output_half : out_tmp.data(), *output_f32);
			return;
		}
		MlpIo io{};
		io.out_half = output_half;
		if (output_f32) {
			io.out_f32 = *output_f32;
			io.out_f32_dims = m_network->output_width();
		}
		ArenaBuf network_input;
		float scale = 1, offset = 0;
		if (m_encoding->as_identity(scale, offset)) {
			io.x_f32 = input;
			io.x_f32_dims = m_encoding->input_width();
			io.x_scale = scale;
			io.x_offset = offset;
		} else if (m_encoding->as_oneblob() && m_encoding->padded_output_width() == m_network->input_width() && (m_network->desc().width == 64 || m_network->desc().width == 128)) {
			io.x_f32 = input;
			io.x_f32_dims = m_encoding->input_width();
			io.x_oneblob_bins = m_encoding->as_oneblob();
		} else {
			network_input = ArenaBuf{stream, (size_t)n * m_encoding->padded_output_width() * 2};
			io.x_half = network_input.data();
			const ForwardPlan plan{m_encoding->forward_route(switches(), n, true, false, false)};
			io.x_plane_features = plan.route.plane_features;
			m_encoding->forward(stream, n, input, p + m_network->n_params(), network_input.data(), false, false, &plan);
		}
		m_network->inference_io(stream, n, io, p);
	}
// ... 91 lines not shown
			m_network->backward(stream, ctx.network_ctx, n, ctx.network_input.data(), output.data(), dL_doutput, g_e.data(), p, nullptr, GradientMode::Ignore);
		}
		Network::SecondOrderPass pass = m_network->second_order_begin(stream, n, ctx.network_input.data(), dL_doutput, p, want_grads || want_q);
		m_encoding->backward_backward_input(stream, ctx.encoding_ctx, n, input, dL_ddLdinput, g_e.data(), t.data(), dL_dinput, encoding_params(p), encoding_params(g), mode);
		if (want_q) q = ArenaBuf{stream, enc_bytes};
		m_network->second_order_finish(stream, pass, n, t.data(), dL_ddLdoutput, q.data(), p, g, mode);
		if (!want_q) return;
		ArenaBuf dx_more;
		MatViewMut dx_view{nullptr, m_encoding->input_width(), 1u};
		if (dL_dinput) {
			dx_more = ArenaBuf{stream, (size_t)n * m_encoding->input_width() * sizeof(float)};
			dx_view.data = dx_more.as<float>();
		}
		m_encoding->backward_rows(stream, ctx.encoding_ctx, n, input, q.data(), dL_dinput ? &dx_view : nullptr, encoding_params(p), enc_grads ? encoding_params(g) : nullptr,
		                          enc_grads ? GradientMode::Accumulate : GradientMode::Ignore);
		if (dL_dinput) add_input_gradient(stream, n, m_encoding->input_width(), MatView{dx_view.data, dx_view.stride_sample, dx_view.stride_dim}, *dL_dinput);
	}

	static bool use_fused_step() { return switches().fused_step; }
	bool fused_step_supported(uint32_t n) const { return use_fused_step() && !m_network->layerwise() && mlp_train_any_kernel(m_network->desc(), n); }
	bool reduction_carries_update(bool want_dL_dinput, GradientMode mode) const { return m_encoding->n_params() == 0 && !want_dL_dinput && mode == GradientMode::Overwrite; }
	bool live_image_kept() const { return m_live_image_kept; }
	void invalidate_live_image() { m_network->invalidate_live_image(); }
	size_t image_preps() const { return m_image_preps; }
	const char* last_train_kernel() const { return m_last_train_kernel; }
	uint64_t scatter_wide_fallbacks() { return m_encoding->scatter_wide_fallbacks(); }
	uint64_t list_scatters() const override { return m_encoding->list_scatters(); }
	uint64_t list_gradient_tails() const override { return m_list_gradient_tails; }
	bool context_keeps_slabs(const ModelContext& c) const { const Ctx* x = dynamic_cast<const Ctx*>(&c); return x && (bool)x->slabs_kept; }
	bool fused_compact_context_supported(uint32_t n) const {
		if (m_network->layerwise()) return false;
		const bool ok = use_fused_step() && mlp_train_compact_context(m_network->desc(), n) && m_network->padded_output_width() == 16;
		if (!ok && use_fused_step() && n > (1u << 22) && mlp_train_compact_context(m_network->desc(), 1u << 22)) {
			static bool told = false;
			if (!told) {
				told = true;
				const std::string msg = "training_step: batches of more than 4194304 rows run the general fused MLP kernel (several times slower for this network); split the batch to stay on the fast path";
				log_message(TCNN_LOG_WARNING, msg);
				fprintf(stderr, "tcnn_amd warning: %s\n", msg.c_str());
			}
		}
		return ok;
	}

	std::unique_ptr<ModelContext> fused_step(hipStream_t stream, uint32_t n, MatView input, const FusedStepData& step, const OptimizerOffer& optimizer) {
		check_batch(n);
		auto ctx = std::make_unique<Ctx>();
		if (step.profile) step.profile->mark(stream, StepProfile::Encode, false);
		const Switches sw = switches();
		const GridForwardRoute route = m_encoding->forward_route(sw, n, true, step.dL_dinput != nullptr, step.mode != GradientMode::Ignore);
		GridItemMap item_map;
		const bool mapped = sw.listgrad_in_mlp && route.recorded == GridRecorded::HitLists && route.plane_features &&
		                    mlp_train_item_map(mlp_train_plan(m_network->desc(), step_request(n, step, route.plane_features, 0, true, route.plane_features, false)), item_map);
		fused_encode(stream, *ctx, n, input, step.params, route, step.dL_dinput != nullptr, step.mode != GradientMode::Ignore, sw.side_jobs, mapped ? &item_map : nullptr);
		if (step.profile) step.profile->mark(stream, StepProfile::Encode, true);
		fused_mlp_and_scatter(stream, sw, *ctx, n, input, step, optimizer);
		return ctx;
	}

	void fused_encode(hipStream_t stream, Ctx& ctx, uint32_t n, MatView input, const void* params, const GridForwardRoute& route, bool prepare_input_gradients, bool prepare_param_gradients,
	                  bool prep_image = false, const GridItemMap* item_map = nullptr) {
		const _Float16* p = (const _Float16*)params;
		const uint32_t n_net = (uint32_t)m_network->n_params();
		if (m_network->layerwise()) throw std::runtime_error{"NetworkWithInputEncoding::fused_encode: a layer-by-layer network has no fused training step"};
		if (!prepare_input_gradients && m_encoding->as_oneblob() && m_encoding->padded_output_width() == m_network->input_width() &&
		    mlp_train_oneblob_in_kernel(m_network->desc(), n, m_encoding->as_oneblob())) {
			ctx.oneblob_bins = m_encoding->as_oneblob();
			ctx.fused = true;
			return;
		}
		ctx.network_input = ArenaBuf{stream, (size_t)n * m_encoding->padded_output_width() * 2};
		ForwardPlan plan{route, nullptr, item_map};
		MlpPrepJob job;
		if (route.plane_features && prep_image) {
			ctx.image = ArenaBuf{stream, mlp_image_bytes(m_network->desc())};
			job.desc = m_network->desc();
			job.params = params;
			job.image = ctx.image.data();
			plan.prep_job = &job;
		}
		ctx.encoding_ctx = m_encoding->forward(stream, n, input, p + n_net, ctx.network_input.data(), prepare_input_gradients, prepare_param_gradients, &plan);
		ctx.fused = true;
	}

	MlpTrainRequest step_request(uint32_t n, const FusedStepData& step, uint32_t x_plane_f, uint32_t oneblob_bins, bool need_dx, uint32_t plane_f, bool records) const {
		MlpTrainRequest request;
		request.n = n;
		request.x_plane_features = x_plane_f;
		request.oneblob_bins = oneblob_bins;
		request.oneblob_dims = oneblob_bins ? m_encoding->input_width() : 0u;
		request.dims = m_network->output_width();
		request.loss = step.loss;
		request.external_dL_dy = step.external_dL_dy != nullptr;
		request.data_pdf = step.data_pdf != nullptr;
		request.out = step.out != nullptr;
		request.dL_dx = need_dx;
		request.dx_plane_features = plane_f;
		request.dx_record_dims = records ? m_encoding->input_width() : 0u;
		request.gradients = step.mode != GradientMode::Ignore;
		request.compact_context = step.compact_context;
		return request;
	}

	void fused_mlp_and_scatter(hipStream_t stream, const Switches& sw, const Ctx& ctx, uint32_t n, MatView input, const FusedStepData& step, const OptimizerOffer& optimizer) {
		const void* params = step.params;
		MatViewMut* dL_dinput = step.dL_dinput;
		const GradientMode mode = step.mode;
		StepProfile* profile = step.profile;
		const _Float16* p = (const _Float16*)params;
		_Float16* g = (_Float16*)step.gradients;
		const uint32_t n_net = (uint32_t)m_network->n_params();
		const bool need_dx = m_encoding->n_params() > 0 || dL_dinput;
		ArenaBuf dL_dnetwork_input;
		const GridBackwardRoute route = need_dx ? m_encoding->backward_route(sw, stream, ctx.encoding_ctx, n, input, GridDyForm::Records, dL_dinput != nullptr, mode) : GridBackwardRoute{};
		const bool records = route.dy == GridDyForm::Records;
		if (need_dx) dL_dnetwork_input = ArenaBuf{stream, records ? (size_t)n * route.record_planes * 16 : (size_t)n * m_encoding->padded_output_width() * 2};

		const MlpDesc& d = m_network->desc();
		const bool with_adam = optimizer.in_reduce != nullptr;
		CHECK_THROW(!with_adam || reduction_carries_update(dL_dinput != nullptr, mode));
		Network::LiveImage* live = with_adam && !ctx.image && sw.live_image ? m_network->live_image() : nullptr;
		m_live_image_kept = false;
		ArenaBuf prepared;
		const void* image_data;
		if (ctx.image) image_data = ctx.image.data();
// ... 141 lines not shown
private:
	Precision m_precision;
	std::unique_ptr<Encoding> m_encoding;
};

inline LossType create_loss(const Json& loss) {
	const std::string otype = loss.value("otype", "RelativeL2");
	static const std::pair<const char*, LossType> table[] = {
		{"L2", LossType::L2}, {"RelativeL2", LossType::RelativeL2}, {"RelativeL2Luminance", LossType::RelativeL2Luminance}, {"L1", LossType::L1},
		{"RelativeL1", LossType::RelativeL1}, {"Mape", LossType::Mape}, {"Smape", LossType::Smape}, {"CrossEntropy", LossType::CrossEntropy}, {"Variance", LossType::Variance}};
	for (const auto& kv : table) if (equals_case_insensitive(otype, kv.first)) return kv.second;
	throw std::runtime_error{"Invalid loss type: " + otype};
}
inline const char* to_string(LossType t) {
	static const char* names[] = {"L2", "RelativeL2", "L1", "RelativeL1", "Mape", "Smape", "CrossEntropy", "Variance", "RelativeL2Luminance"};
	return names[(uint32_t)t];
}
inline bool loss_in_fused_kernel(LossType t) { return t == LossType::L2 || t == LossType::RelativeL2; }

inline Json device_to_binary(const void* device, size_t n_bytes) {
	std::vector<uint8_t> host(n_bytes);
	if (n_bytes) HIP_CHECK_THROW(hipMemcpy(host.data(), device, n_bytes, hipMemcpyDeviceToHost));
	return Json::binary(std::move(host));
}
inline std::vector<uint8_t> binary_of(const Json& j) {
	if (j.is_binary()) return j.get_binary();
	if (j.is_object()) {
		const Json& arr = j["bytes"];
		std::vector<uint8_t> bytes(arr.size());
		for (size_t i = 0; i < bytes.size(); ++i) bytes[i] = (uint8_t)arr.at(i).as_double();
		return bytes;
	}
	throw std::runtime_error{"Invalid json type: must be either binary or object"};
}

class Optimizer {
public:
	virtual ~Optimizer() {}
	virtual void allocate(size_t n_weights, const std::vector<std::pair<uint32_t, uint32_t>>& layer_sizes) = 0;
	void allocate(size_t n_weights, const std::vector<std::pair<uint32_t, uint32_t>>& layer_sizes, Precision weight_precision) {
		set_weight_precision(weight_precision);
		allocate(n_weights, layer_sizes);
	}
	virtual void set_weight_precision(Precision p) { m_weight_precision = p; }
	Precision weight_precision() const { return m_weight_precision; }
	bool fp32_weights() const { return m_weight_precision == Precision::Fp32; }
	size_t weight_bytes() const { return fp32_weights() ? sizeof(float) : 2; }
	virtual void step(hipStream_t stream, float loss_scale, float* weights_full_precision, void* weights, const void* gradients, GradientPrecision precision = GradientPrecision::Fp16) = 0;
	virtual bool takes_prologue() const { return false; }
	virtual bool can_step_in_reduce() const { return false; }
	virtual AdamInReduce begin_step_in_reduce(hipStream_t stream, float loss_scale, float* weights_full_precision, void* weights) {
		throw std::runtime_error{"Optimizer: this optimizer's step cannot be applied by the slab reduction"};
	}
	virtual bool step_with_prologue(hipStream_t stream, float loss_scale, float* weights_full_precision, void* weights, void* gradients, const AdamPrologue& prologue) { return false; }
	virtual float learning_rate() const = 0;
	virtual void set_learning_rate(float val) = 0;
	virtual uint32_t step_count() const = 0;
	virtual size_t n_weights() const = 0;
	virtual void* custom_weights() const { return nullptr; }
	virtual void update_hyperparams(const Json& params) = 0;
	virtual Json hyperparams() const = 0;
	virtual Json serialize() const = 0;
	virtual void deserialize(const Json& data, size_t n_weights) = 0;
	virtual void weights_restored(hipStream_t stream, const void* weights) {}
protected:
	void* checked_weights(float* weights_full_precision, void* weights, GradientPrecision precision) const {
		if (!fp32_weights()) return weights;
		if (weights != nullptr && weights != (void*)weights_full_precision) throw std::runtime_error{"Optimizer: with fp32 weights there is one weight vector (weights must be null or weights_full_precision)."};
		if (precision != GradientPrecision::Fp32) throw std::runtime_error{"Optimizer: with fp32 weights the gradients must be fp32."};
		return weights_full_precision;
	}
	Precision m_weight_precision = Precision::Fp16;
};
inline std::unique_ptr<Optimizer> create_optimizer(const Json& params);

class AdamOptimizer : public Optimizer {
public:
	explicit AdamOptimizer(const Json& params) { update_hyperparams(params); }
	float learning_rate() const override { return m_h.learning_rate; }
	void set_learning_rate(float val) override { m_h.learning_rate = val; }
	size_t n_weights() const override { return m_n_weights; }

	void allocate(size_t n_weights, const std::vector<std::pair<uint32_t, uint32_t>>& layer_sizes) override {
		m_n_weights = n_weights;
		if (n_weights * sizeof(float) > m_first_moments.bytes()) {
			m_first_moments.resize(n_weights * sizeof(float));
			m_second_moments.resize(n_weights * sizeof(float));
		}
		m_steps16 = narrow_steps_enabled();
		m_param_steps.resize(0);
		m_param_steps.resize(n_weights * step_bytes());
		m_first_moments.memset(0);
		m_second_moments.memset(0);
		m_param_steps.memset(0);
		m_n_matrix = 0;
		for (const auto& ls : layer_sizes) m_n_matrix += (size_t)ls.first * ls.second;
	}

	Json serialize() const override {
		auto blob = [](const DeviceBuf& buf, size_t n_bytes) { return device_to_binary(buf.data(), n_bytes); };
		Json data = Json::object();
		data["current_step"] = Json((uint32_t)m_current_step);
		data["base_learning_rate"] = Json((float)m_h.learning_rate);
		data["first_moments_binary"] = blob(m_first_moments, m_n_weights * sizeof(float));
		data["second_moments_binary"] = blob(m_second_moments, m_n_weights * sizeof(float));
		if (m_steps16) {
			std::vector<uint16_t> narrow(m_n_weights);
// ... 1 lines not shown
			std::vector<uint8_t> wide(m_n_weights * sizeof(uint32_t));
			for (size_t i = 0; i < m_n_weights; ++i) {
				const uint32_t v = narrow[i];
				std::memcpy(wide.data() + 4 * i, &v, 4);
			}
			data["param_steps_binary"] = Json::binary(std::move(wide));
		} else {
			data["param_steps_binary"] = blob(m_param_steps, m_n_weights * sizeof(uint32_t));
		}
		return data;
	}
	void deserialize(const Json& data, size_t n_weights) override {
		auto load = [&](DeviceBuf& buf, const std::vector<uint8_t>& bytes, size_t elem) {
			if (bytes.size() != n_weights * elem) throw std::runtime_error{"Adam: snapshot state has the wrong size."};
			buf.resize(bytes.size());
			if (!bytes.empty()) HIP_CHECK_THROW(hipMemcpy(buf.data(), bytes.data(), bytes.size(), hipMemcpyHostToDevice));
		};
		m_n_weights = n_weights;
		load(m_first_moments, binary_of(data["first_moments_binary"]), sizeof(float));
		load(m_second_moments, binary_of(data["second_moments_binary"]), sizeof(float));
		m_current_step = (uint32_t)data["current_step"].as_double();
		m_steps16 = narrow_steps_enabled() && m_current_step < NARROW_STEP_LIMIT;
		if (data.contains("param_steps_binary")) {
			const std::vector<uint8_t>& bytes = binary_of(data["param_steps_binary"]);
			if (bytes.size() != n_weights * sizeof(uint32_t)) throw std::runtime_error{"Adam: snapshot state has the wrong size."};
			std::vector<uint16_t> narrow(m_steps16 ? n_weights : 0);
			for (size_t i = 0; m_steps16 && i < n_weights; ++i) {
				uint32_t v;
				std::memcpy(&v, bytes.data() + 4 * i, 4);
				if (v >= NARROW_STEP_LIMIT) m_steps16 = false;
				else narrow[i] = (uint16_t)v;
			}
			m_param_steps.resize(0);
			m_param_steps.resize(n_weights * step_bytes());
			if (n_weights) HIP_CHECK_THROW(hipMemcpy(m_param_steps.data(), m_steps16 ? (const void*)narrow.data() : (const void*)bytes.data(), n_weights * step_bytes(), hipMemcpyHostToDevice));
		} else {
			m_param_steps.resize(0);
			m_param_steps.resize(n_weights * step_bytes());
			m_param_steps.memset(0);
		}
		m_h.learning_rate = (float)data["base_learning_rate"].as_double();
	}

	void step(hipStream_t stream, float loss_scale, float* weights_full_precision, void* weights, const void* gradients, GradientPrecision precision = GradientPrecision::Fp16) override {
		weights = checked_weights(weights_full_precision, weights, precision);
		++m_current_step;
		ensure_debias_table(stream);
		ensure_step_width(stream);
		adam_step(stream, m_h, m_n_weights, m_n_matrix, loss_scale, m_current_step, weights_full_precision, weights, gradients,
		          m_first_moments.as<float>(), m_second_moments.as<float>(), m_param_steps.data(), m_steps16, m_debias.as<float>(), precision, m_weight_precision);
	}

	bool takes_prologue() const override { return !fp32_weights(); }
	bool step_with_prologue(hipStream_t stream, float loss_scale, float* weights_full_precision, void* weights, void* gradients, const AdamPrologue& prologue) override {
		if (fp32_weights() || switches().adam_prologue_refused) return false;
		++m_current_step;
		ensure_debias_table(stream);
		ensure_step_width(stream);
		if (adam_step_with_prologue(stream, m_h, m_n_weights, m_n_matrix, loss_scale, m_current_step, weights_full_precision, weights, gradients, m_first_moments.as<float>(),
		                            m_second_moments.as<float>(), m_param_steps.data(), m_steps16, m_debias.as<float>(), prologue)) return true;
		--m_current_step;
		return false;
	}

	static constexpr uint32_t NARROW_STEP_LIMIT = 65535;
	static bool narrow_steps_enabled() { return !switches().adam_steps32; }
	size_t step_bytes() const { return m_steps16 ? sizeof(uint16_t) : sizeof(uint32_t); }
	void ensure_step_width(hipStream_t stream) {
		if (!m_steps16 || m_current_step < NARROW_STEP_LIMIT) return;
		DeviceBuf wide;
		wide.resize(m_n_weights * sizeof(uint32_t));
		adam_widen_steps(stream, m_n_weights, m_param_steps.data(), wide.data());
		HIP_CHECK_THROW(hipStreamSynchronize(stream));
		m_param_steps = std::move(wide);
		m_steps16 = false;
	}

	bool can_step_in_reduce() const override { return !fp32_weights(); }
	AdamInReduce begin_step_in_reduce(hipStream_t stream, float loss_scale, float* weights_full_precision, void* weights) override {
		if (fp32_weights()) return Optimizer::begin_step_in_reduce(stream, loss_scale, weights_full_precision, weights);
		++m_current_step;
		ensure_debias_table(stream);
		ensure_step_width(stream);
		AdamInReduce out;
		out.args = make_adam_args(m_h, loss_scale, m_current_step);
		out.w_fp = weights_full_precision;
		out.w_half = weights;
		out.m1 = m_first_moments.as<float>();
		out.m2 = m_second_moments.as<float>();
		out.steps = m_param_steps.data();
		out.steps16 = m_steps16 ? 1u : 0u;
		out.debias_table = m_debias.as<float>();
		return out;
	}

	void ensure_debias_table(hipStream_t stream) {
		const bool stale = m_debias_beta1 != m_h.beta1 || m_debias_beta2 != m_h.beta2;
		if (!stale && m_current_step < m_debias_filled) return;
		const uint32_t want = next_multiple(m_current_step + 1, 4096u) + 4096u;
		if ((size_t)want * sizeof(float) > m_debias.bytes()) {
			HIP_CHECK_THROW(hipStreamSynchronize(stream));
			m_debias.resize((size_t)want * 2 * sizeof(float));
			m_debias_filled = 0;
		}
		const uint32_t from = stale ? 0u : m_debias_filled;
		adam_fill_debias_table(stream, m_h.beta1, m_h.beta2, from, want, m_debias.as<float>());
		m_debias_filled = want;
		m_debias_beta1 = m_h.beta1;
		m_debias_beta2 = m_h.beta2;
	}

	void update_hyperparams(const Json& p) override {
		if (!p.is_object()) return;
		if (p.contains("beta1")) m_h.beta1 = (float)p["beta1"].as_double();
		if (p.contains("beta2")) m_h.beta2 = (float)p["beta2"].as_double();
// ... 638 lines not shown
	const void* dL_doutput_ptr = nullptr;
	ArenaBuf L;
	std::unique_ptr<ModelContext> model_ctx;
	uint32_t n = 0;

	bool compact = false;
	uint32_t dims = 0, padded_width = 0;
	hipStream_t stream = nullptr;
	ArenaBuf compact_dL_doutput;
	ArenaBuf compact_L;
	void materialize();
};

inline void TrainContext::materialize() {
	if (!compact || L) return;
	L = ArenaBuf{stream, (size_t)n * padded_width * sizeof(float)};
	dL_doutput = ArenaBuf{stream, (size_t)n * padded_width * 2};
	dL_doutput_ptr = dL_doutput.data();
	CHECK_THROW(padded_width == 16);
	mlp_expand_context(stream, n, dims, compact_dL_doutput.data(), compact_L.as<float>(), dL_doutput.data(), L.as<float>());
}

inline MatView make_view(const float* data, uint32_t width, uint32_t n, int layout) {
	return layout == 1 ? MatView{data, width, 1u} : MatView{data, 1u, n};
}
inline MatViewMut make_view_mut(float* data, uint32_t width, uint32_t n, int layout) {
	return layout == 1 ? MatViewMut{data, width, 1u} : MatViewMut{data, 1u, n};
}

class Trainer {
public:
	Trainer(uint32_t n_input_dims, uint32_t n_output_dims, const Json& config, uint32_t seed, Precision precision = Precision::Fp16) : m_fp32{precision == Precision::Fp32} {
		const Json encoding = config.value("encoding", Json::object());
		const Json loss = config.value("loss", Json::object());
		const Json optimizer = config.value("optimizer", Json::object());
		const Json network = config.value("network", Json::object());
		m_loss = create_loss(loss);
		m_optimizer = create_optimizer(optimizer);
		if (m_fp32) {
			const std::string otype = network.is_object() ? network.value("otype", "MLP") : std::string{"MLP"};
			if (equals_case_insensitive(otype, "MegakernelMLP") || equals_case_insensitive(otype, "FullyFusedMLP")) {
				throw std::runtime_error{"FullyFusedMLP can only be used if the network precision is set to __half."};
			}
		}
		m_model.reset(new NetworkWithInputEncoding{n_input_dims, n_output_dims, encoding, network, precision});
		std::seed_seq seq{seed};
		std::vector<uint32_t> seeds(2);
		seq.generate(std::begin(seeds), std::end(seeds));
		m_rng = Pcg32{seeds.front()};
		m_scalar.resize(sizeof(float) * 2048);
		initialize_params();
	}

	void initialize_params() {
		const size_t n = m_model->n_params();
		m_optimizer->allocate(n, m_model->layer_sizes(), precision());
		m_params_fp.resize(n * sizeof(float));
		m_grads.resize(n * elem());
		m_params_fp.memset(0);
		m_grads.memset(0);
		m_model->initialize_params(m_rng, m_params_fp.as<float>(), 1.0f);
		if (!m_fp32) {
			m_params.resize(n * 2);
			m_params.memset(0);
			cast_float_to_half(nullptr, n, m_params_fp.as<float>(), m_params.data());
		}
		HIP_CHECK_THROW(hipDeviceSynchronize());
	}

	std::unique_ptr<TrainContext> forward(hipStream_t stream, float loss_scale, uint32_t n, MatView input, const float* target, const float* data_pdf,
	                                      bool use_inference_params, bool prepare_input_gradients, const void* external_dL_dy) {
		auto ctx = std::make_unique<TrainContext>();
		ctx->n = n;
		const uint32_t pw = m_model->padded_output_width();
		ctx->output = ArenaBuf{stream, (size_t)n * pw * elem()};
		ctx->model_ctx = m_model->forward(stream, n, input, ctx->output.data(), use_inference_params ? params_inference() : working_params(), prepare_input_gradients);
		ctx->L = ArenaBuf{stream, (size_t)n * pw * sizeof(float)};
		if (external_dL_dy) {
			ctx->dL_doutput_ptr = external_dL_dy;
			HIP_CHECK_THROW(hipMemsetAsync(ctx->L.data(), 0, ctx->L.bytes(), stream));
		} else {
			CHECK_THROW(target != nullptr);
			ctx->dL_doutput = ArenaBuf{stream, (size_t)n * pw * elem()};
			ctx->dL_doutput_ptr = ctx->dL_doutput.data();
			loss_evaluate(stream, m_loss, n, pw, m_model->output_width(), loss_scale, ctx->output.data(), target, ctx->L.as<float>(), ctx->dL_doutput.data(), data_pdf, precision());
		}
		return ctx;
	}

	void backward(hipStream_t stream, const TrainContext& ctx, uint32_t n, MatView input, MatViewMut* dL_dinput, bool use_inference_params, GradientMode mode) {
		const_cast<TrainContext&>(ctx).materialize();
		m_model->backward(stream, *ctx.model_ctx, n, input, ctx.output.data(), ctx.dL_doutput_ptr, dL_dinput, use_inference_params ? params_inference() : working_params(), m_grads.data(), mode);
	}

	size_t params_updated_in_flush() const { return m_params_updated_in_flush; }
	size_t m_prologue_steps = 0;

	OptimizerPlace optimizer_place(bool run_optimizer, GradientMode mode, bool want_dL_dinput) const {
		if (!run_optimizer) return OptimizerPlace::None;
		const Switches sw = switches();
		if (sw.adam_in_reduce && m_optimizer->can_step_in_reduce() && m_model->reduction_carries_update(want_dL_dinput, mode)) return OptimizerPlace::InReduce;
		if (sw.adam_prologue && mode != GradientMode::Ignore && m_optimizer->takes_prologue()) return OptimizerPlace::Prologue;
		return OptimizerPlace::OwnLaunch;
	}

	void run_prologue_alone(hipStream_t stream, const AdamPrologue& p) {
		MlpReduceJob job;
		if (p.has_reduce) {
			job.n_elems = p.reduce_elems;
			job.n_slabs = p.reduce_slabs;
			job.slabs = p.slabs;
			job.grad = m_grads.data();
			job.accumulate = p.reduce_accumulate;
		}
		if (!p.ranges.empty()) grid_scatter_finalize(stream, p.dev_ranges, (uint32_t)p.ranges.size(), p.scratch, p.grad_base, p.accumulate, p.has_reduce ? &job : nullptr);
		else if (p.has_reduce) mlp_reduce_slabs(stream, p.reduce_elems, p.reduce_slabs, p.slabs, m_grads.data(), p.reduce_accumulate != 0);
	}

	void optimizer_step(hipStream_t stream, float loss_scale) {
		m_model->invalidate_live_image();
		m_optimizer->step(stream, loss_scale, m_params_fp.as<float>(), working_params(), m_grads.data(), m_fp32 ? GradientPrecision::Fp32 : GradientPrecision::Fp16);
	}

	std::unique_ptr<TrainContext> training_step(hipStream_t stream, uint32_t n, MatView input, const float* target, const float* data_pdf, bool run_optimizer,
	                                            MatViewMut* dL_dinput, bool use_inference_params, GradientMode mode, const void* external_dL_dy) {
		const float loss_scale = m_fp32 ? 1.0f : LOSS_SCALE_FP16;
		std::unique_ptr<TrainContext> ctx;
		const bool other_weights = use_inference_params && params_inference() != working_params();
		if (!m_fp32 && m_model->fused_step_supported(n) && (external_dL_dy || loss_in_fused_kernel(m_loss)) && !other_weights) {
			ctx = std::make_unique<TrainContext>();
			ctx->n = n;
			const uint32_t pw = m_model->padded_output_width();
			ctx->output = ArenaBuf{stream, (size_t)n * pw * 2};
			ctx->compact = !external_dL_dy && mode != GradientMode::Ignore && m_model->fused_compact_context_supported(n);
			if (ctx->compact) {
				CHECK_THROW(target != nullptr);
				ctx->dims = m_model->output_width();
				ctx->padded_width = pw;
				ctx->stream = stream;
				ctx->compact_dL_doutput = ArenaBuf{stream, (size_t)n * ctx->dims * 2};
				ctx->compact_L = ArenaBuf{stream, (size_t)n * ctx->dims * sizeof(float)};
			} else {
				ctx->L = ArenaBuf{stream, (size_t)n * pw * sizeof(float)};
				if (external_dL_dy) {
					ctx->dL_doutput_ptr = external_dL_dy;
					HIP_CHECK_THROW(hipMemsetAsync(ctx->L.data(), 0, ctx->L.bytes(), stream));
				} else {
					CHECK_THROW(target != nullptr);
					ctx->dL_doutput = ArenaBuf{stream, (size_t)n * pw * 2};
					ctx->dL_doutput_ptr = ctx->dL_doutput.data();
				}
			}
			m_params_updated_in_flush = 0;
			m_profile.begin_step();
			const OptimizerPlace place = optimizer_place(run_optimizer, mode, dL_dinput != nullptr);
			AdamInReduce in_reduce;
			AdamPrologue prologue;
			OptimizerOffer offer;
			if (place == OptimizerPlace::InReduce) {
				in_reduce = m_optimizer->begin_step_in_reduce(stream, loss_scale, m_params_fp.as<float>(), m_params.data());
				offer.in_reduce = &in_reduce;
			} else if (place == OptimizerPlace::Prologue) offer.prologue = &prologue;
			FusedStepData step;
			step.target = target, step.data_pdf = data_pdf, step.external_dL_dy = external_dL_dy;
			step.loss = m_loss;
			step.loss_scale = loss_scale;
			step.out = ctx->output.data();
			step.dL_dout = ctx->compact ? ctx->compact_dL_doutput.data() : ctx->dL_doutput.data();
			step.L = ctx->compact ? ctx->compact_L.as<float>() : ctx->L.as<float>();
			step.compact_context = ctx->compact;
			step.dL_dinput = dL_dinput;
			step.params = m_params.data(), step.gradients = m_grads.data();
			step.mode = mode;
			step.profile = &m_profile;
			ctx->model_ctx = m_model->fused_step(stream, n, input, step, offer);
			if (m_params_exposed || (place != OptimizerPlace::None && !m_model->live_image_kept())) m_model->invalidate_live_image();
			if (place != OptimizerPlace::None) {
				m_profile.mark(stream, StepProfile::Optimizer, false);
				if (place == OptimizerPlace::InReduce) m_params_updated_in_flush = m_model->n_params();
				else if (prologue.pending && m_optimizer->step_with_prologue(stream, loss_scale, m_params_fp.as<float>(), m_params.data(), m_grads.data(), prologue)) ++m_prologue_steps;
				else {
					if (prologue.pending) run_prologue_alone(stream, prologue);
					m_optimizer->step(stream, loss_scale, m_params_fp.as<float>(), m_params.data(), m_grads.data());
				}
				m_profile.mark(stream, StepProfile::Optimizer, true);
			}
			m_profile.end_step();
			m_last_step_kernel = m_model->last_train_kernel();
			return ctx;
		} else {
			m_last_step_kernel = "unfused";
			ctx = forward(stream, loss_scale, n, input, target, data_pdf, use_inference_params, dL_dinput != nullptr, external_dL_dy);
			backward(stream, *ctx, n, input, dL_dinput, use_inference_params, mode);
		}
		m_params_updated_in_flush = 0;
		if (run_optimizer) optimizer_step(stream, loss_scale);
		return ctx;
	}

	float loss(hipStream_t stream, const TrainContext& ctx) {
		float* partials = m_scalar.as<float>();
		float* result = partials + 1024;
		if (ctx.compact && !ctx.L) reduce_sum(stream, (size_t)ctx.n * ctx.dims, ctx.compact_L.as<float>(), partials, result);
		else reduce_sum(stream, (size_t)ctx.n * m_model->padded_output_width(), ctx.L.as<float>(), partials, result);
		float host = 0;
		HIP_CHECK_THROW(hipMemcpyAsync(&host, result, sizeof(float), hipMemcpyDeviceToHost, stream));
		HIP_CHECK_THROW(hipStreamSynchronize(stream));
		return host;
	}

	void inference(hipStream_t stream, uint32_t n, MatView input, MatViewMut output, bool use_inference_params) {
		Model::check_batch(n);
		if (n == 0) return;
		m_model->inference_f32(stream, n, input, output, use_inference_params ? params_inference() : working_params());
	}

	void inference_mixed_precision(hipStream_t stream, uint32_t n, MatView input, void* output_half, bool use_inference_params) {
		Model::check_batch(n);
		if (n == 0) return;
		m_model->inference(stream, n, input, output_half, use_inference_params ? params_inference() : working_params());
	}

	void set_params_full_precision(const float* params, size_t n_params, bool device_ptr) {
		if (n_params != m_model->n_params()) throw std::runtime_error{"Can't set fp params because buffer has the wrong size."};
		m_model->invalidate_live_image();
		HIP_CHECK_THROW(hipMemcpy(m_params_fp.data(), params, sizeof(float) * n_params, device_ptr ? hipMemcpyDeviceToDevice : hipMemcpyHostToDevice));
		if (!m_fp32) cast_float_to_half(nullptr, n_params, m_params_fp.as<float>(), m_params.data());
		if (params_inference() != working_params()) HIP_CHECK_THROW(hipMemcpy(params_inference(), working_params(), elem() * n_params, hipMemcpyDeviceToDevice));
		HIP_CHECK_THROW(hipDeviceSynchronize());
	}

	void set_params(const void* params, size_t n_params, bool device_ptr) {
		if (n_params != m_model->n_params()) throw std::runtime_error{"Can't set params because buffer has the wrong size."};
		if (m_fp32) return set_params_full_precision((const float*)params, n_params, device_ptr);
		m_model->invalidate_live_image();
		HIP_CHECK_THROW(hipMemcpy(m_params.data(), params, 2 * n_params, device_ptr ? hipMemcpyDeviceToDevice : hipMemcpyHostToDevice));
		cast_half_to_float(nullptr, n_params, m_params.data(), m_params_fp.as<float>());
		if (params_inference() != m_params.data()) HIP_CHECK_THROW(hipMemcpy(params_inference(), m_params.data(), 2 * n_params, hipMemcpyDeviceToDevice));
		HIP_CHECK_THROW(hipDeviceSynchronize());
	}

	void update_hyperparams(const Json& params) {
		m_optimizer->update_hyperparams(params.value("optimizer", Json::object()));
	}

	Json serialize(bool serialize_optimizer) {
		HIP_CHECK_THROW(hipDeviceSynchronize());
		const size_t n = m_model->n_params();
		Json data = Json::object();
		data["n_params"] = Json((uint64_t)n);
		data["params_type"] = m_fp32 ? "float" : "__half";
		data["params_binary"] = device_to_binary(params_inference(), elem() * n);
		if (serialize_optimizer) data["optimizer"] = m_optimizer->serialize();
		return data;
	}

	void deserialize(const Json& data) {
		const std::string type = data.value("params_type", "__half");
		const std::vector<uint8_t> bytes = binary_of(data["params_binary"]);
		if (type == "float") {
			if (bytes.size() % sizeof(float) != 0) throw std::runtime_error{"Can't set fp params because buffer has the wrong size."};
			set_params_full_precision((const float*)bytes.data(), bytes.size() / sizeof(float), false);
		} else if (type == "__half" && m_fp32) {
			if (bytes.size() != 2 * m_model->n_params()) throw std::runtime_error{"Can't set params because buffer has the wrong size."};
			DeviceBuf half;
			half.resize(bytes.size());
			DeviceBuf wide;
			wide.resize(bytes.size() * 2);
			if (!bytes.empty()) HIP_CHECK_THROW(hipMemcpy(half.data(), bytes.data(), bytes.size(), hipMemcpyHostToDevice));
			cast_half_to_float(nullptr, bytes.size() / 2, half.data(), wide.as<float>());
			HIP_CHECK_THROW(hipDeviceSynchronize());
			set_params_full_precision(wide.as<float>(), bytes.size() / 2, true);
		} else if (type == "__half") {
			if (bytes.size() % 2 != 0) throw std::runtime_error{"Can't set params because buffer has the wrong size."};
			set_params(bytes.data(), bytes.size() / 2, false);
		} else {
			throw std::runtime_error{"Trainer: snapshot parameters must be of type float of __half"};
		}
		if (data.contains("optimizer")) {
			m_optimizer->deserialize(data["optimizer"], m_model->n_params());
			m_optimizer->weights_restored(nullptr, working_params());
		}
		HIP_CHECK_THROW(hipDeviceSynchronize());
	}

	Json hyperparams() const {
		Json j = Json::object();
		j["otype"] = "Trainer";
		j["optimizer"] = m_optimizer->hyperparams();
		Json l = Json::object();
		l["otype"] = to_string(m_loss);
		j["loss"] = l;
		return j;
	}

	NetworkWithInputEncoding& model() { return *m_model; }
	Optimizer& optimizer() { return *m_optimizer; }
	StepProfile& profile() { return m_profile; }
	void* params_inference() const { void* custom = m_optimizer->custom_weights(); return custom ? custom : working_params(); }
	Precision precision() const { return m_fp32 ? Precision::Fp32 : Precision::Fp16; }
	size_t elem() const { return m_fp32 ? sizeof(float) : 2; }
	void* working_params() const { return m_fp32 ? m_params_fp.data() : m_params.data(); }
	size_t n_params() const { return m_model->n_params(); }
	float* params_full_precision() { expose_params(); return m_params_fp.as<float>(); }
	void* params() { expose_params(); return working_params(); }
	const void* params_unexposed() const { return working_params(); }
	size_t image_preps() const { return m_model->image_preps(); }
	uint64_t scatter_wide_fallbacks() { return m_model->scatter_wide_fallbacks(); }
	uint64_t list_scatters() const { return m_model->list_scatters(); }
	uint64_t list_gradient_tails() const { return m_model->list_gradient_tails(); }
	size_t prologue_steps() const { return m_prologue_steps; }
	const char* last_step_kernel() const { return m_last_step_kernel; }
	void* param_gradients() const { return m_grads.data(); }

private:
	std::unique_ptr<NetworkWithInputEncoding> m_model;
	std::unique_ptr<Optimizer> m_optimizer;
	LossType m_loss;
	Pcg32 m_rng;
	DeviceBuf m_params_fp, m_params, m_grads, m_scalar;
	StepProfile m_profile;
	size_t m_params_updated_in_flush = 0;
	const char* m_last_step_kernel = "";
	bool m_params_exposed = false;
	const bool m_fp32 = false;
	void expose_params() {
		m_params_exposed = true;
		m_model->invalidate_live_image();
	}
};

}
```

### tiny-cuda-nn_amd/csrc/tcnn_common.h

```cpp
#pragma once

#include <hip/hip_runtime.h>

#include <cstddef>
#include <cstdint>
#include <stdexcept>
#include <string>
#include <vector>

namespace tcnn_amd {

enum class Activation : uint32_t { None = 0, ReLU = 1, LeakyReLU = 2, Exponential = 3, Sine = 4, Sigmoid = 5, Squareplus = 6, Softplus = 7, Tanh = 8 };
enum class GridType : uint32_t { Hash = 0, Dense = 1, Tiled = 2 };
enum class HashType : uint32_t { Prime = 0, CoherentPrime = 1, ReversedPrime = 2, Rng = 3 };
enum class InterpolationType : uint32_t { Nearest = 0, Linear = 1, Smoothstep = 2 };
enum class LossType : uint32_t { L2 = 0, RelativeL2 = 1, L1 = 2, RelativeL1 = 3, Mape = 4, Smape = 5, CrossEntropy = 6, Variance = 7, RelativeL2Luminance = 8 };
enum class Precision : uint32_t { Fp32 = 0, Fp16 = 1 };
enum class GradientPrecision : uint32_t { Fp32 = 0, Fp16 = 1 };
enum class GradientMode : uint32_t { Ignore = 0, Overwrite = 1, Accumulate = 2 };

constexpr uint32_t BATCH_SIZE_GRANULARITY = 256;
constexpr float LOSS_SCALE_FP16 = 128.0f;
constexpr uint32_t MAX_N_LEVELS = 128;
constexpr uint32_t MAX_MLP_LAYERS = 16;

#define TCNN_STR2(x) #x
#define TCNN_STR(x) TCNN_STR2(x)
#define CHECK_THROW(x) \
	do { if (!(x)) throw std::runtime_error{std::string{__FILE__ ":" TCNN_STR(__LINE__) " check failed: " #x}}; } while (0)
#define HIP_CHECK_THROW(x) \
	do { hipError_t _e = (x); if (_e != hipSuccess) throw std::runtime_error{std::string{__FILE__ ":" TCNN_STR(__LINE__) " " #x " failed: "} + hipGetErrorString(_e)}; } while (0)

inline uint32_t div_round_up(uint32_t v, uint32_t d) { return (v + d - 1) / d; }

struct Switches {
	bool grid_planes = true;
	bool grid_rows_planes = true;
	bool grid_scatter_lds = true;
	bool scatter_records = true;
	bool scatter_tune = true;
	int scatter_lists = -1;
	bool scatter_wide = false;
	bool fused_step = true;
	bool side_jobs = true;
	bool live_image = true;
	bool adam_steps32 = false;
	bool adam_in_reduce = true;
	bool adam_prologue = true;
	bool adam_prologue_refused = false;
	bool mlp_r32 = true;
	int mlp_r32a = -1;
	bool mlp_regs = true;
	bool mlp_fast = true;
	uint32_t mlp_prio = 1;
	bool listgrad_in_mlp = true;
	bool mlp_layerwise = false;
};
Switches switches();
void switches_reload();
inline uint32_t next_multiple(uint32_t v, uint32_t d) { return div_round_up(v, d) * d; }

struct GridLevel {
	uint32_t offset;
	uint32_t size;
	float    scale;
	uint32_t hashed;
	uint32_t stride[4];
	uint32_t size_mask;
	uint32_t scatter_per_chunk;
	uint32_t scatter_shift;
	uint32_t scatter_n_chunks;
	uint32_t scatter_binned;
};

struct GridMeta {
	uint32_t n_pos_dims;
	uint32_t n_features_per_level;
	uint32_t n_levels;
	uint32_t grid_type;
	uint32_t hash_type;
	uint32_t interpolation;
	uint32_t primes[4];
	GridLevel levels[MAX_N_LEVELS];
};

struct MatView {
	const float* data;
	uint32_t stride_sample;
	uint32_t stride_dim;
};
struct MatViewMut {
	float* data;
	uint32_t stride_sample;
	uint32_t stride_dim;
};

void grid_forward(hipStream_t stream, const GridMeta& meta, const GridMeta* dev_meta, bool fp32, uint32_t n, MatView x, const void* grid, void* out, uint32_t out_stride, float* dy_dx,
                  uint64_t* chunk_mask);
bool grid_planes_supported(const GridMeta& meta, uint32_t n);
bool grid_planes_to_rows_supported(const GridMeta& meta, uint32_t n, uint32_t width);
void grid_planes_to_rows(hipStream_t stream, const GridMeta& meta, uint32_t n, uint32_t width, const void* planes, void* rows, uint32_t row_stride);
void grid_rows_to_planes(hipStream_t stream, const GridMeta& meta, uint32_t n, uint32_t width, const void* rows, uint32_t row_stride, void* planes);
uint32_t grid_planes_spt(const GridMeta& meta);
void grid_planes_plan(const GridMeta& meta, uint32_t n, bool hit_lists, std::vector<uint32_t>& work, uint32_t& max_items, uint32_t& blocks_per_xcd);
struct MlpPrepJob;
inline constexpr uint32_t grid_hit_mask_shift(uint32_t n_pos_dims) { return 32u - (1u << n_pos_dims); }
constexpr uint32_t GRID_HIT_COUNT_STRIDE = 64;
constexpr uint32_t GRID_HIT_HEADS = 65;
constexpr uint32_t GRID_HIT_WORDS = 2;
struct GridItemMap {
	uint32_t window = 0, window_shift = 0, stride = 0, n_windows = 0;
	bool operator==(const GridItemMap& o) const { return window == o.window && window_shift == o.window_shift && stride == o.stride && n_windows == o.n_windows; }
};
inline GridItemMap grid_item_map(uint32_t window, uint32_t stride, uint32_t n_windows) {
	GridItemMap m;
	m.window = window, m.stride = stride, m.n_windows = n_windows;
	while ((1u << m.window_shift) < window) ++m.window_shift;
	return m;
}
#if defined(__HIPCC__)
__host__ __device__
#endif
inline uint32_t grid_item_sample(const GridItemMap& m, uint32_t item, uint32_t pos) { return (item << m.window_shift) + (pos & (m.window - 1u)) + (pos >> m.window_shift) * m.stride; }
struct GridHitLists {
	uint32_t* elems = nullptr;
	uint16_t* sidx = nullptr;
	uint32_t* heads = nullptr;
	uint32_t* stragglers = nullptr;
	uint32_t* counts = nullptr;
	uint32_t* zero_counts = nullptr;
	uint32_t n_items = 0, item_samples = 0, item_capacity = 0, straggler_capacity = 0;
	GridItemMap map;
	uint32_t dev_flags = 0;
};
struct GridListTail {
	const uint16_t* sidx = nullptr;
	const uint32_t* heads = nullptr;
	void* gvals = nullptr;
	uint32_t n_items = 0, item_capacity = 0, n_levels = 0, level_mask = 0;
	GridItemMap map;
};
uint32_t grid_hit_item_samples(const GridMeta& meta);
inline uint32_t grid_hit_max_samples(const GridMeta& meta) { return meta.n_pos_dims <= 2 ? (1u << 24) : (1u << 22); }
void grid_forward_planes(hipStream_t stream, const GridMeta& meta, const GridMeta* dev_meta, const uint32_t* dev_work, uint32_t max_items, uint32_t blocks_per_xcd, uint32_t n,
                         MatView x, const void* grid, void* out_planes, uint64_t* chunk_bits, const MlpPrepJob* prep_job = nullptr, const GridHitLists* hit_lists = nullptr);
void grid_backward(hipStream_t stream, const GridMeta& meta, const GridMeta* dev_meta, bool fp32_grad, uint32_t n, MatView x, const void* dL_dy, bool dy_fp32, uint32_t dy_stride, void* grad);

struct GridScatterTask {
	uint32_t level;
	uint32_t entry_begin, n_entries;
	uint32_t sample_begin, sample_end;
	uint32_t flush_atomic;
	uint32_t scratch_begin;
	uint32_t pad;
};
struct GridScatterRange { size_t grad_begin; uint32_t n_elems; uint32_t scratch_begin; uint32_t pad; };
struct MlpReduceJob;
// ... 8 lines not shown
bool grid_backward_lds(hipStream_t stream, const GridMeta& meta, const GridMeta* dev_meta, const GridScatterTask* dev_tasks, uint32_t n_tasks,
                       const GridScatterRange* dev_ranges, uint32_t n_ranges, uint64_t* scratch, uint32_t n, MatView x,
                       const void* dL_dy, uint32_t dy_stride_sample, uint32_t dy_stride_level, void* grad, const uint64_t* chunk_bits, bool accumulate, bool dy_records = false,
                       uint64_t* task_times = nullptr,
                       const MlpReduceJob* reduce_job = nullptr);
uint32_t grid_scatter_lists_lds_bytes();
void grid_scatter_lists_plan(const GridMeta& meta, uint32_t n, std::vector<GridScatterTask>& tasks, std::vector<GridScatterRange>& shared_ranges, size_t& scratch_elems);
bool grid_backward_lists(hipStream_t stream, const GridMeta& meta, const GridMeta* dev_meta, const GridScatterTask* dev_tasks, uint32_t n_tasks,
                         const GridScatterRange* dev_ranges, uint32_t n_ranges, uint64_t* scratch, uint32_t n, MatView x,
                         const void* dL_dy, uint32_t dy_stride_sample, uint32_t dy_stride_level, void* grad, const GridHitLists& lists, void* gvals, bool accumulate,
                         const MlpReduceJob* reduce_job, uint32_t* fallback_count = nullptr, bool gvals_filled = false);
size_t grid_list_gradients_bytes(const GridMeta& meta, const GridHitLists& lists);
bool grid_scatter_finalize(hipStream_t stream, const GridScatterRange* dev_ranges, uint32_t n_ranges, uint64_t* scratch, void* grad, bool accumulate, const MlpReduceJob* reduce_job);
bool grid_scatter_records_supported(const GridMeta& meta);
uint32_t grid_scatter_record_planes(const GridMeta& meta);

struct GridFacts {
	const GridMeta* meta;
	bool fp32, scatter_levels_ok, any_binned;
	uint32_t n_to_pad;
};
enum class GridForwardKernel : uint32_t { Rows, Planes, PlanesToRows };
enum class GridRecorded : uint32_t { Nothing, BitPlanes, HitLists };
struct GridForwardRoute {
	bool planned = false;
	GridForwardKernel kernel = GridForwardKernel::Rows;
	GridRecorded recorded = GridRecorded::Nothing;
	bool lds = false;
	uint32_t plane_features = 0;
};
inline bool grid_lds_gradients(const GridFacts& g, const Switches& sw, uint32_t n) {
	return !g.fp32 && g.meta->n_features_per_level >= 2 && sw.grid_scatter_lds && g.scatter_levels_ok && n % 64 == 0;
}
inline bool grid_hit_lists_wanted(const GridFacts& g, const Switches& sw, uint32_t n) {
	const GridMeta& meta = *g.meta;
	if (sw.scatter_lists == 0) return false;
	if (g.any_binned || n > grid_hit_max_samples(meta) || meta.n_pos_dims > 3 || meta.hash_type == (uint32_t)HashType::Rng) return false;
	if (sw.scatter_lists == 1) return true;
	if (meta.n_pos_dims == 2 && n < (1u << 16)) return false;
	return grid_scatter_prefers_lists(meta);
}
inline GridForwardRoute grid_forward_route(const GridFacts& g, const Switches& sw, uint32_t n, bool as_planes, bool input_gradients, bool param_gradients) {
	const GridMeta& meta = *g.meta;
	const uint32_t F = meta.n_features_per_level;
	GridForwardRoute r;
	r.planned = true;
	r.lds = grid_lds_gradients(g, sw, n);
	const bool planes = !input_gradients && !g.fp32 && sw.grid_planes && g.n_to_pad % F == 0 && grid_planes_supported(meta, n);
	if (planes && as_planes) r.kernel = GridForwardKernel::Planes;
	else if (planes && sw.grid_rows_planes && grid_planes_to_rows_supported(meta, n, meta.n_levels * F + g.n_to_pad)) r.kernel = GridForwardKernel::PlanesToRows;
	if (r.kernel == GridForwardKernel::Planes) r.plane_features = F;
	if (param_gradients && r.lds) r.recorded = (r.kernel != GridForwardKernel::Rows && grid_hit_lists_wanted(g, sw, n)) ? GridRecorded::HitLists : GridRecorded::BitPlanes;
	return r;
}

enum class GridDyForm : uint32_t { Rows, Planes, Records };
enum class GridGradientKernel : uint32_t { None, Atomic, AtomicScratch32, BitPlanes, Lists };
enum class GridMaxLevel : uint32_t { None, Scalar, PerSample };
struct GridBackwardRoute {
	GridDyForm dy = GridDyForm::Rows;
	uint32_t plane_features = 0, record_planes = 0;
	GridGradientKernel kernel = GridGradientKernel::None;
	bool binned = false, tune = false, prologue = false;
	bool tail = false;
	GridListTail list_tail;
	size_t tail_bytes = 0;
};
inline GridBackwardRoute grid_backward_route(const GridFacts& g, const Switches& sw, const GridForwardRoute& fwd, bool lists_current, uint32_t n, GridDyForm offer, bool want_dL_dx,
                                             GradientMode mode, GridMaxLevel max_level, bool x_contiguous) {
	const GridMeta& meta = *g.meta;
	const uint32_t F = meta.n_features_per_level;
	GridBackwardRoute r;
	if (mode == GradientMode::Ignore) return r;
	if (!(fwd.planned ? fwd.lds : grid_lds_gradients(g, sw, n))) {
		r.kernel = (!g.fp32 && F == 1) ? GridGradientKernel::AtomicScratch32 : GridGradientKernel::Atomic;
		return r;
	}
	const bool lists = fwd.recorded == GridRecorded::HitLists && lists_current;
	r.kernel = lists ? GridGradientKernel::Lists : GridGradientKernel::BitPlanes;
	r.binned = !lists && g.any_binned;
	r.tune = !lists && sw.scatter_tune;
	r.prologue = max_level != GridMaxLevel::Scalar && !g.any_binned;
	if (offer == GridDyForm::Rows || want_dL_dx) return r;
	r.dy = GridDyForm::Planes, r.plane_features = F;
	if (offer == GridDyForm::Records && fwd.recorded != GridRecorded::HitLists && g.n_to_pad == 0 && max_level != GridMaxLevel::PerSample && sw.scatter_records && !g.any_binned &&
	    grid_scatter_records_supported(meta) && x_contiguous) {
		r.dy = GridDyForm::Records, r.record_planes = grid_scatter_record_planes(meta);
		return r;
	}
	r.tail = offer == GridDyForm::Records && lists && F == 2 && max_level == GridMaxLevel::None && sw.listgrad_in_mlp && meta.n_levels <= 16 &&
	         (grid_hit_item_samples(meta) << (meta.n_pos_dims - 1)) <= 2048;
	if (r.tail) {
		r.list_tail.n_levels = meta.n_levels;
		for (uint32_t l = 0; l < meta.n_levels; ++l) {
			const GridLevel& lv = meta.levels[l];
			if (lv.scatter_n_chunks > 1 && lv.scatter_n_chunks <= GRID_FILTER_MAX_CHUNKS && !lv.scatter_binned) r.list_tail.level_mask |= 1u << l;
		}
	}
	return r;
}

void ppng1_forward(hipStream_t stream, bool fp32_out, uint32_t n, uint32_t F, uint32_t Q, uint32_t C, uint32_t R, int32_t log2_min_freq, int32_t log2_max_freq, MatView x,
                   const void* features, void* out, uint32_t out_stride);
void ppng1_backward(hipStream_t stream, bool fp32_dy, uint32_t n, uint32_t F, uint32_t Q, uint32_t C, uint32_t R, int32_t log2_min_freq, int32_t log2_max_freq, MatView x,
                    const void* features, const void* dL_dy, uint32_t dy_stride, uint64_t* scratch, void* grad, bool accumulate);

// ... 149 lines not shown
void mlp_layer_backward_keep_f32(hipStream_t stream, uint32_t n, const float* d_out, uint32_t ldo, const float* wt, uint32_t rows, uint32_t cols, uint32_t activation, const float* aux,
                                 float* g_in, float* d_in, uint32_t ldi);
void mlp_layer_curvature_backward_f32(hipStream_t stream, uint32_t n, const float* p_out, uint32_t ldo, const float* wt, uint32_t rows, uint32_t cols, uint32_t activation,
                                      const float* aux, const float* r_in, float* p_in, uint32_t ldi);
void mlp_layer_delta_f32(hipStream_t stream, size_t n_elems, uint32_t activation, const float* g, const float* aux, float* delta);
void mlp_activation_backward_output_f32(hipStream_t stream, size_t n_elems, uint32_t activation, const float* dL_dout, const float* out, float* result);
size_t wgrad_panels_workspace_floats_f32(const WgradPanel* panels, uint32_t count, uint32_t n);
void mlp_wgrad_panels_f32(hipStream_t stream, uint32_t n, const WgradPanel* panels, uint32_t count, bool accumulate, float* workspace);

void loss_evaluate(hipStream_t stream, LossType type, uint32_t n, uint32_t stride, uint32_t dims, float loss_scale,
                   const void* pred_half, const float* target, float* values, void* grads_half, const float* data_pdf, Precision precision = Precision::Fp16);
void reduce_sum(hipStream_t stream, size_t n, const float* values, float* partials, float* result_dev);

struct AdamHyper {
	float learning_rate = 1e-3f, beta1 = 0.9f, beta2 = 0.999f, epsilon = 1e-8f, l2_reg = 1e-8f;
	float relative_decay = 0.0f, absolute_decay = 0.0f, clipping_magnitude = 0.0f, non_matrix_learning_rate_factor = 1.0f;
	bool adabound = false, optimize_matrix_params = true, optimize_non_matrix_params = true;
};
struct AdamArgs {
	float relative_weight_decay, absolute_weight_decay, weight_clipping_magnitude, loss_scale, learning_rate, non_matrix_learning_rate_factor;
	float beta1, beta2, epsilon, lower_lr_bound, upper_lr_bound, l2_reg;
	uint32_t optimize_matrix_params, optimize_non_matrix_params;
	float inv_loss_scale;
	uint32_t inv_loss_scale_exact;
	uint32_t common_step;
};
AdamArgs make_adam_args(const AdamHyper& h, float loss_scale, uint32_t current_step);
constexpr uint32_t IMAGE_INV_WIDTH = 4;
struct AdamInReduce {
	AdamArgs args;
	float* w_fp = nullptr;
	void* w_half = nullptr;
	float* m1 = nullptr;
	float* m2 = nullptr;
	void* steps = nullptr;
	uint32_t steps16 = 0;
	const float* debias_table = nullptr;
	void* image = nullptr;
	const uint32_t* image_inv = nullptr;
};
struct AdamPrologue {
	bool pending = false;
	const GridScatterRange* dev_ranges = nullptr;
	std::vector<GridScatterRange> ranges;
	uint64_t* scratch = nullptr;
	void* grad_base = nullptr;
	bool accumulate = false;
	bool has_reduce = false;
	uint32_t reduce_elems = 0, reduce_slabs = 0;
	const float* slabs = nullptr;
	int reduce_accumulate = 0;
};
bool adam_step_with_prologue(hipStream_t stream, const AdamHyper& h, size_t n, size_t n_matrix, float loss_scale, uint32_t current_step,
                             float* w_fp, void* w_half, void* g_half, float* m1, float* m2, void* steps, bool steps16, const float* debias_table, const AdamPrologue& p);
void adam_step(hipStream_t stream, const AdamHyper& h, size_t n, size_t n_matrix, float loss_scale, uint32_t current_step,
               float* w_fp, void* w_half, const void* gradients, float* m1, float* m2, void* steps, bool steps16, const float* debias_table,
               GradientPrecision precision = GradientPrecision::Fp16, Precision weight_precision = Precision::Fp16);
void adam_widen_steps(hipStream_t stream, size_t n, const void* steps16, void* steps32);
void adam_fill_debias_table(hipStream_t stream, float beta1, float beta2, uint32_t from, uint32_t to, float* table);
void copy_columns(hipStream_t stream, size_t elem_bytes, uint32_t n, const void* src, uint32_t src_stride, uint32_t src_col, void* dst, uint32_t dst_stride, uint32_t dst_col, uint32_t width);
void sgd_step(hipStream_t stream, size_t n, float loss_scale, float learning_rate, float l2_reg, float* weights_full_precision, void* weights, const void* gradients,
              GradientPrecision precision = GradientPrecision::Fp16, Precision weight_precision = Precision::Fp16);
void ema_step(hipStream_t stream, size_t n, float decay, float debias_old, float debias_new, const void* weights, void* weights_ema, float* tmp, Precision weight_precision = Precision::Fp16);
void average_step(hipStream_t stream, size_t n, uint32_t n_samples, const void* weights, void* current_sample, void* average, Precision weight_precision = Precision::Fp16);
void batched_accumulate(hipStream_t stream, size_t n, bool first, uint32_t multiplier, const void* gradients, float* pool, GradientPrecision precision = GradientPrecision::Fp16);
void lookahead_step(hipStream_t stream, size_t n, float alpha, float* weights_full_precision, void* weights, void* weights_lookahead, Precision weight_precision = Precision::Fp16);
void novograd_layer_step(hipStream_t stream, size_t n, float relative_decay, float absolute_decay, float loss_scale, float learning_rate, float beta1, float beta2, float epsilon,
                         float* weights_full_precision, void* weights, const void* gradients, float* first_moments, float* layer_second_moment,
                         GradientPrecision precision = GradientPrecision::Fp16, Precision weight_precision = Precision::Fp16);

void generate_random_uniform(hipStream_t stream, uint64_t* state_inc_host, size_t n, float* out, float lower, float upper);
void cast_float_to_half(hipStream_t stream, size_t n, const float* in, void* out);
void cast_half_to_float(hipStream_t stream, size_t n, const void* in, float* out);
void trim_and_cast(hipStream_t stream, bool fp32, uint32_t n, uint32_t in_stride, uint32_t dims, const void* in, MatViewMut out);
void fill_half(hipStream_t stream, size_t n, void* out, float value);
void grid_zero_levels(hipStream_t stream, size_t elem_bytes, uint32_t n, uint32_t n_levels, uint32_t level0, uint32_t width, uint64_t sample_stride, uint64_t level_stride,
                      void* data, const void* src, const float* per_sample, uint32_t n_grid_features, uint32_t F, bool gradient_rule);

}
```

### tiny-cuda-nn_amd/tinycudann/_C.py

```python
import ctypes as C
import json
import os

_PKG = os.path.dirname(os.path.dirname(os.path.abspath(__file__)))
LIB_PATH = os.path.join(_PKG, "libtcnn_amd.so")
if os.environ.get("TCNN_AMD_LIB"):
    LIB_PATH = os.path.abspath(os.environ["TCNN_AMD_LIB"])

if not os.path.exists(LIB_PATH):
    raise ImportError(
        f"{LIB_PATH} not found: the HIP extension has not been built. Run `python tiny-cuda-nn_amd/build.py` "
        "(or __graft_entry__.build()). There is no CPU fallback."
    )

import torch

lib = C.CDLL(LIB_PATH)

_hip = None


def hip_runtime():
    global _hip
    if _hip is None:
# ... 36 lines not shown
    "tcnn_create_network_precision": (_int, [_u32, _u32, _cp, _int, _pp]),
    "tcnn_module_destroy": (None, [_vp]),
    "tcnn_module_inference": (_int, [_vp, _vp, _u32, _vp, _vp, _vp]),
    "tcnn_module_forward": (_int, [_vp, _vp, _u32, _vp, _vp, _vp, _int, _pp]),
    "tcnn_module_backward": (_int, [_vp, _vp, _vp, _u32, _vp, _vp, _vp, _vp, _vp, _vp]),
    "tcnn_module_backward_backward_input": (_int, [_vp, _vp, _vp, _u32, _vp, _vp, _vp, _vp, _vp, _vp, _vp]),
    "tcnn_module_backward_backward_input_mode": (_int, [_vp, _vp, _vp, _u32, _vp, _vp, _vp, _vp, _vp, _vp, _vp, _int]),
    "tcnn_context_destroy": (None, [_vp]),
    "tcnn_module_n_input_dims": (_u32, [_vp]),
    "tcnn_module_n_output_dims": (_u32, [_vp]),
    "tcnn_module_n_params": (_sz, [_vp]),
    "tcnn_module_list_scatters": (_sz, [_vp]),
    "tcnn_module_set_max_level": (_int, [_vp, _f32]),
    "tcnn_module_max_level": (_f32, [_vp]),
    "tcnn_module_set_max_level_gpu": (_int, [_vp, _vp]),
    "tcnn_module_param_precision": (_int, [_vp]),
    "tcnn_module_output_precision": (_int, [_vp]),
    "tcnn_module_initialize_params": (_int, [_vp, _u64, _vp, _f32]),
    "tcnn_module_hyperparams": (_cp, [_vp]),
    "tcnn_module_name": (_cp, [_vp]),
    "tcnn_create_from_config": (_int, [_u32, _u32, _cp, _pp]),
    "tcnn_create_from_config_seeded": (_int, [_u32, _u32, _cp, _u32, _pp]),
    "tcnn_create_from_config_precision": (_int, [_u32, _u32, _cp, _u32, _int, _pp]),
    "tcnn_trainer_precision": (_int, [_vp]),
    "tcnn_trainer_destroy": (None, [_vp]),
    "tcnn_trainer_training_step": (_int, [_vp, _vp, _u32, _vp, _int, _vp, _vp, _int, _vp, _int, _int, _vp, _pp]),
    "tcnn_trainer_loss": (_int, [_vp, _vp, _vp, C.POINTER(C.c_float)]),
    "tcnn_trainer_forward": (_int, [_vp, _vp, _f32, _u32, _vp, _int, _vp, _vp, _int, _int, _vp, _pp]),
    "tcnn_trainer_backward": (_int, [_vp, _vp, _vp, _u32, _vp, _int, _vp, _int, _int]),
    "tcnn_trainer_optimizer_step": (_int, [_vp, _vp, _f32]),
    "tcnn_train_ctx_destroy": (None, [_vp]),
    "tcnn_train_ctx_output": (_vp, [_vp]),
    "tcnn_train_ctx_dL_doutput": (_vp, [_vp]),
    "tcnn_train_ctx_L": (_vp, [_vp]),
    "tcnn_trainer_inference": (_int, [_vp, _vp, _u32, _vp, _int, _vp, _int, _int]),
    "tcnn_trainer_inference_mixed_precision": (_int, [_vp, _vp, _u32, _vp, _int, _vp, _int]),
    "tcnn_trainer_n_params": (_sz, [_vp]),
    "tcnn_trainer_padded_output_width": (_u32, [_vp]),
    "tcnn_trainer_params_full_precision": (_vp, [_vp]),
    "tcnn_trainer_params": (_vp, [_vp]),
    "tcnn_trainer_params_inference": (_vp, [_vp]),
    "tcnn_trainer_param_gradients": (_vp, [_vp]),
    "tcnn_trainer_set_params_full_precision": (_int, [_vp, _vp, _sz, _int]),
    "tcnn_trainer_set_params": (_int, [_vp, _vp, _sz, _int]),
    "tcnn_trainer_initialize_params": (_int, [_vp]),
    "tcnn_trainer_update_hyperparams": (_int, [_vp, _cp]),
    "tcnn_trainer_hyperparams": (_cp, [_vp]),
    "tcnn_trainer_network_hyperparams": (_cp, [_vp]),
    "tcnn_trainer_optimizer_step_count": (_u32, [_vp]),
    "tcnn_trainer_params_updated_in_flush": (C.c_size_t, [_vp]),
    "tcnn_trainer_image_preps": (C.c_size_t, [_vp]),
    "tcnn_trainer_scatter_wide_fallbacks": (C.c_size_t, [_vp]),
    "tcnn_trainer_optimizer_prologue_steps": (C.c_size_t, [_vp]),
    "tcnn_trainer_list_scatters": (C.c_size_t, [_vp]),
    "tcnn_trainer_list_gradient_tails": (C.c_size_t, [_vp]),
    "tcnn_trainer_last_step_kernel": (_cp, [_vp]),
    "tcnn_trainer_set_max_level": (_int, [_vp, _f32]),
    "tcnn_trainer_set_max_level_gpu": (_int, [_vp, _vp]),
    "tcnn_trainer_max_level": (_f32, [_vp]),
    "tcnn_train_ctx_keeps_weight_gradient_slabs": (C.c_int, [_vp, _vp]),
    "tcnn_trainer_profile_next_step": (_int, [_vp]),
    "tcnn_trainer_profile_collect": (_int, [_vp, _vp, C.POINTER(C.c_float), C.POINTER(_u32)]),
    "tcnn_trainer_serialize": (_int, [_vp, _int, _pp, C.POINTER(_sz)]),
    "tcnn_trainer_deserialize": (_int, [_vp, _vp, _sz]),
    "tcnn_module_layer_sizes": (_int, [_vp, C.POINTER(_u32), _sz, C.POINTER(_sz)]),
    "tcnn_optimizer_create": (_int, [_cp, _sz, C.POINTER(_u32), _sz, _pp]),
    "tcnn_optimizer_create_precision": (_int, [_cp, _sz, C.POINTER(_u32), _sz, _int, _pp]),
    "tcnn_optimizer_weight_precision": (_int, [_vp]),
    "tcnn_optimizer_destroy": (None, [_vp]),
    "tcnn_optimizer_step": (_int, [_vp, _vp, _f32, _vp, _vp, _vp, _int]),
    "tcnn_optimizer_step_count": (_u32, [_vp]),
    "tcnn_optimizer_n_params": (_sz, [_vp]),
    "tcnn_optimizer_learning_rate": (_f32, [_vp]),
    "tcnn_optimizer_set_learning_rate": (_int, [_vp, _f32]),
    "tcnn_optimizer_update_hyperparams": (_int, [_vp, _cp]),
    "tcnn_optimizer_hyperparams": (_cp, [_vp]),
    "tcnn_optimizer_custom_weights": (_vp, [_vp]),
    "tcnn_optimizer_weights_restored": (_int, [_vp, _vp, _vp]),
    "tcnn_optimizer_serialize": (_int, [_vp, _pp, C.POINTER(_sz)]),
    "tcnn_optimizer_deserialize": (_int, [_vp, _vp, _sz]),
}

for _name, (_res, _args) in _SIGNATURES.items():
    _fn = getattr(lib, _name)
    _fn.restype = _res
    _fn.argtypes = _args


class Precision:
    Fp32 = 0
    Fp16 = 1


class LogSeverity:
    Info, Debug, Warning, Error, Success = range(5)


def check(status):
    if status != 0:
        raise RuntimeError(lib.tcnn_last_error().decode("utf-8", "replace"))


def to_json_bytes(obj):
    if obj is None:
        return b"{}"
    if isinstance(obj, (bytes, bytearray)):
# ... 25 lines not shown
```

### tiny-cuda-nn_amd/tinycudann/native.py

```python
import ctypes as C
import json

import torch

from . import _C

LAYOUT_SOA, LAYOUT_AOS = 0, 1
GRADIENT_IGNORE, GRADIENT_OVERWRITE, GRADIENT_ACCUMULATE = 0, 1, 2


_PRECISIONS = {None: _C.Precision.Fp16, torch.float16: _C.Precision.Fp16, torch.float32: _C.Precision.Fp32}


def _trainer_precision(dtype):
    if dtype not in _PRECISIONS:
        raise ValueError(f"Trainer only supports fp32 or fp16 precision, but got {dtype}")
    return _PRECISIONS[dtype]


def _ptr(t):
    return None if t is None else t.data_ptr()


def _stream(stream=None):
# ... 35 lines not shown


class Trainer:

    def __init__(self, n_input_dims, n_output_dims, config, seed=1337, dtype=None):
        precision = _trainer_precision(dtype)
        if not torch.cuda.is_available():
            raise EnvironmentError("tcnn_amd needs a ROCm GPU (gfx950): torch.cuda.is_available() is False.")
        torch.cuda.init()
        h = C.c_void_p()
        _C.check(_C.lib.tcnn_create_from_config_precision(n_input_dims, n_output_dims, _C.to_json_bytes(config), seed, precision, C.byref(h)))
        self._h = h
        self.dtype = torch.float32 if precision == _C.Precision.Fp32 else torch.half
        self.default_loss_scale = _C.default_loss_scale(precision)
        self.n_input_dims = n_input_dims
        self.n_output_dims = n_output_dims
        self.padded_output_width = int(_C.lib.tcnn_trainer_padded_output_width(h))
        self._max_level_gpu = None

    def __del__(self):
        h, self._h = getattr(self, "_h", None), None
        if h and _C is not None and getattr(_C, 'lib', None) is not None:
            _C.lib.tcnn_trainer_destroy(h)

    def training_step(self, input, target, data_pdf=None, run_optimizer=True, dL_dinput=None, use_inference_params=False,
                      gradient_mode=GRADIENT_OVERWRITE, external_dL_dy=None, input_layout=LAYOUT_AOS, stream=None):
        n = input.shape[0] if input_layout == LAYOUT_AOS else input.shape[1]
        self._check_max_level_rows(n)
        ctx = C.c_void_p()
        _C.check(_C.lib.tcnn_trainer_training_step(self._h, _stream(stream), n, _ptr(input), input_layout, _ptr(target), _ptr(data_pdf),
                                                   int(run_optimizer), _ptr(dL_dinput), int(use_inference_params), gradient_mode,
                                                   _ptr(self._checked_dy(external_dL_dy)), C.byref(ctx)))
        return ForwardContext(ctx, n, self.padded_output_width, self.dtype)

    def _checked_dy(self, external_dL_dy):
        if external_dL_dy is not None and self.dtype == torch.float32 and external_dL_dy.dtype != torch.float32:
            raise TypeError(f"tcnn: external_dL_dy must be {self.dtype}, the trainer's precision, not {external_dL_dy.dtype}")
        return external_dL_dy

    PROFILE_PIECES = ("encode", "mlp_kernel", "encoding_backward", "optimizer")

    def profile_next_step(self):
        _C.check(_C.lib.tcnn_trainer_profile_next_step(self._h))

    def params_updated_in_flush(self):
        return int(_C.lib.tcnn_trainer_params_updated_in_flush(self._h))

    def image_preps(self):
        return int(_C.lib.tcnn_trainer_image_preps(self._h))

    def optimizer_prologue_steps(self):
        return int(_C.lib.tcnn_trainer_optimizer_prologue_steps(self._h))

    def list_scatters(self):
        return int(_C.lib.tcnn_trainer_list_scatters(self._h))

    def list_gradient_tails(self):
        return int(_C.lib.tcnn_trainer_list_gradient_tails(self._h))

    def last_step_kernel(self):
        return _C.lib.tcnn_trainer_last_step_kernel(self._h).decode()

    def context_keeps_slabs(self, ctx):
        return bool(_C.lib.tcnn_train_ctx_keeps_weight_gradient_slabs(self._h, ctx._h))

    def scatter_wide_fallbacks(self):
        return int(_C.lib.tcnn_trainer_scatter_wide_fallbacks(self._h))

    def profile_collect(self, stream=None):
        ms = (C.c_float * 4)()
        n = C.c_uint32()
        _C.check(_C.lib.tcnn_trainer_profile_collect(self._h, _stream(stream), ms, C.byref(n)))
        k = max(n.value, 1)
        return {name: ms[i] / k for i, name in enumerate(self.PROFILE_PIECES)}, n.value

    def loss(self, ctx, stream=None):
        out = C.c_float()
        _C.check(_C.lib.tcnn_trainer_loss(self._h, _stream(stream), ctx._h, C.byref(out)))
        return out.value

    def forward(self, input, target, loss_scale=None, data_pdf=None, prepare_input_gradients=False, external_dL_dy=None, input_layout=LAYOUT_AOS, stream=None):
        n = input.shape[0] if input_layout == LAYOUT_AOS else input.shape[1]
        self._check_max_level_rows(n)
        ctx = C.c_void_p()
        loss_scale = self.default_loss_scale if loss_scale is None else loss_scale
        _C.check(_C.lib.tcnn_trainer_forward(self._h, _stream(stream), loss_scale, n, _ptr(input), input_layout, _ptr(target), _ptr(data_pdf), 0,
                                             int(prepare_input_gradients), _ptr(self._checked_dy(external_dL_dy)), C.byref(ctx)))
        return ForwardContext(ctx, n, self.padded_output_width, self.dtype)

    def backward(self, ctx, input, dL_dinput=None, gradient_mode=GRADIENT_OVERWRITE, input_layout=LAYOUT_AOS, stream=None):
        self._check_max_level_rows(ctx.n)
        _C.check(_C.lib.tcnn_trainer_backward(self._h, _stream(stream), ctx._h, ctx.n, _ptr(input), input_layout, _ptr(dL_dinput), 0, gradient_mode))

    def optimizer_step(self, loss_scale=None, stream=None):
        loss_scale = self.default_loss_scale if loss_scale is None else loss_scale
        _C.check(_C.lib.tcnn_trainer_optimizer_step(self._h, _stream(stream), loss_scale))

    def inference(self, input, output=None, input_layout=LAYOUT_AOS, output_layout=LAYOUT_AOS, stream=None):
        n = input.shape[0] if input_layout == LAYOUT_AOS else input.shape[1]
        if output is None:
            shape = (n, self.n_output_dims) if output_layout == LAYOUT_AOS else (self.n_output_dims, n)
            output = torch.empty(shape, dtype=torch.float32, device=input.device)
        self._check_max_level_rows(n)
        _C.check(_C.lib.tcnn_trainer_inference(self._h, _stream(stream), n, _ptr(input), input_layout, _ptr(output), output_layout, 1))
        return output

# ... 98 lines not shown
```

Baseline: 1.411 billion.

## Defer fine-level Adam update to overlap with next step's coarse grid forward

Splits the Adam update at a hash-grid level boundary. Parameters below the split are updated in the prologue kernel as before, while the fine-level tail is deferred to a separate range kernel on a side stream. The next step's planes forward runs the coarse levels first, then waits on an event before the fine levels that need the updated parameters. A cost model picks the split level that hides the most optimizer time, and a host join is added wherever parameters or gradients are exposed. This adds an extra kernel launch and event dependency, plus concurrency that may contend with the forward kernel for bandwidth.

```diff
diff --git a/include/tcnn_amd.h b/include/tcnn_amd.h
--- a/include/tcnn_amd.h
+++ b/include/tcnn_amd.h
@@ -131,6 +131,7 @@
 size_t tcnn_trainer_image_preps(tcnn_trainer_t t);
 size_t tcnn_trainer_scatter_wide_fallbacks(tcnn_trainer_t t);
 size_t tcnn_trainer_optimizer_prologue_steps(tcnn_trainer_t t);
+size_t tcnn_trainer_deferred_optimizer_steps(tcnn_trainer_t t);
 size_t tcnn_trainer_list_scatters(tcnn_trainer_t t);
 size_t tcnn_module_list_scatters(tcnn_module_t m);
 size_t tcnn_trainer_list_gradient_tails(tcnn_trainer_t t);
diff --git a/tiny-cuda-nn_amd/csrc/capi.cpp b/tiny-cuda-nn_amd/csrc/capi.cpp
--- a/tiny-cuda-nn_amd/csrc/capi.cpp
+++ b/tiny-cuda-nn_amd/csrc/capi.cpp
@@ -98,6 +98,9 @@
 	if (const char* e = getenv("TCNN_AMD_MLP_PRIO")) w.mlp_prio = (uint32_t)atoi(e);
 	w.listgrad_in_mlp = !env_is("TCNN_AMD_LISTGRAD_IN_MLP", '0');
 	w.mlp_layerwise = env_is("TCNN_AMD_MLP_LAYERWISE", '1');
+	w.adam_overlap = !env_is("TCNN_AMD_ADAM_OVERLAP", '0');
+	if (const char* e = getenv("TCNN_AMD_ADAM_OVERLAP_SPLIT")) w.adam_overlap_split = *e ? atoi(e) : -1;
+	if (const char* e = getenv("TCNN_AMD_ADAM_OVERLAP_WGS")) w.adam_overlap_wgs = (uint32_t)std::max(1, atoi(e));
 	std::lock_guard<std::mutex> lock{g_switches_mutex};
 	g_switches = w;
 }
@@ -410,6 +413,9 @@
 size_t tcnn_trainer_optimizer_prologue_steps(tcnn_trainer_t t) {
 	try { return (size_t)t->trainer->prologue_steps(); } catch (const std::exception& e) { g_last_error = e.what(); return (size_t)-1; }
 }
+size_t tcnn_trainer_deferred_optimizer_steps(tcnn_trainer_t t) {
+	try { return (size_t)t->trainer->deferred_steps(); } catch (const std::exception& e) { g_last_error = e.what(); return (size_t)-1; }
+}
 size_t tcnn_trainer_scatter_wide_fallbacks(tcnn_trainer_t t) {
 	try { return (size_t)t->trainer->scatter_wide_fallbacks(); } catch (const std::exception& e) { g_last_error = e.what(); return (size_t)-1; }
 }
@@ -488,7 +494,7 @@
 int tcnn_trainer_profile_collect(tcnn_trainer_t t, tcnn_stream_t stream, float* ms_per_piece, uint32_t* n_steps) {
 	return guarded([&] {
 		CHECK_THROW(t && t->trainer && ms_per_piece && n_steps);
-		*n_steps = t->trainer->profile().collect((hipStream_t)stream, ms_per_piece);
+		*n_steps = t->trainer->profile_collect((hipStream_t)stream, ms_per_piece);
 	});
 }
 
diff --git a/tiny-cuda-nn_amd/csrc/k_grid_planes.hip b/tiny-cuda-nn_amd/csrc/k_grid_planes.hip
--- a/tiny-cuda-nn_amd/csrc/k_grid_planes.hip
+++ b/tiny-cuda-nn_amd/csrc/k_grid_planes.hip
@@ -366,7 +366,7 @@
 	       div_round_up(n, FP_THREADS * grid_planes_spt(meta)) < (1u << 24);
 }
 
-void grid_planes_plan(const GridMeta& meta, uint32_t n, bool hit_lists, std::vector<uint32_t>& work, uint32_t& max_items, uint32_t& blocks_per_xcd) {
+void grid_planes_plan(const GridMeta& meta, uint32_t n, bool hit_lists, std::vector<uint32_t>& work, uint32_t& max_items, uint32_t& blocks_per_xcd, uint32_t level_begin, uint32_t level_end) {
 	const uint32_t threads = hit_lists ? FP_LIST_THREADS : FP_THREADS;
 	const uint32_t items_per_level = div_round_up(n, threads * grid_planes_spt(meta));
 	float coarse_cost = 0.6f;
@@ -380,7 +380,8 @@
 		cost[l] = bytes > (256u << 10) ? 1.0f : coarse_cost;
 		total += (double)cost[l] * items_per_level;
 	}
-	uint32_t dbg_lo = 0, dbg_hi = meta.n_levels;
+	uint32_t dbg_lo = level_begin, dbg_hi = std::min(level_end, meta.n_levels) - 1;
+	if (level_end <= level_begin) dbg_lo = 1, dbg_hi = 0;
 #ifdef TCNN_AMD_DEV
 	if (const char* e = getenv("TCNN_AMD_FWD_LEVELS")) sscanf(e, "%u,%u", &dbg_lo, &dbg_hi);
 #endif
diff --git a/tiny-cuda-nn_amd/csrc/k_misc.hip b/tiny-cuda-nn_amd/csrc/k_misc.hip
--- a/tiny-cuda-nn_amd/csrc/k_misc.hip
+++ b/tiny-cuda-nn_amd/csrc/k_misc.hip
@@ -753,6 +753,7 @@
 	unsigned long long* scratch;
 	size_t range_base;
 	size_t bulk_begin;
+	size_t bulk_end;
 };
 
 #ifndef TCNN_PRO_BOUNDS
@@ -830,7 +831,7 @@
 #pragma unroll
 	for (int k = 0; k < PRO_Q; ++k) {
 		const size_t i4 = p.bulk_begin + (((size_t)(b - p.n_range_blocks) * PRO_Q + k) * PRO_THREADS + tid) * 4;
-		live[k] = i4 < n;
+		live[k] = i4 < p.bulk_end;
 		for (uint32_t r = 0; r < p.n_ranges; ++r) {
 			const size_t rb = p.range_base + p.ranges[r].grad_begin;
 			if (i4 >= rb && i4 < rb + p.ranges[r].n_elems) live[k] = false;
@@ -846,7 +847,7 @@
 }
 
 bool adam_step_with_prologue(hipStream_t stream, const AdamHyper& h, size_t n, size_t n_matrix, float loss_scale, uint32_t current_step,
-                             float* w_fp, void* w_half, void* g_half, float* m1, float* m2, void* steps, bool steps16, const float* debias_table, const AdamPrologue& pro) {
+                             float* w_fp, void* w_half, void* g_half, float* m1, float* m2, void* steps, bool steps16, const float* debias_table, const AdamPrologue& pro, size_t bulk_end) {
 	const auto aligned = [](const void* ptr, size_t bytes) { return ((uintptr_t)ptr & (bytes - 1)) == 0; };
 	if (n == 0 || !(aligned(w_fp, 16) && aligned(m1, 16) && aligned(m2, 16) && aligned(steps, steps16 ? 8 : 16) && aligned(w_half, 8) && aligned(g_half, 8))) return false;
 	PrologueArgs p{};
@@ -860,13 +861,14 @@
 		p.slabs = pro.slabs;
 		p.bulk_begin = pro.reduce_elems;
 	} else if (n_matrix % 4 != 0) return false;
-	if ((n - p.bulk_begin) % 4 != 0) return false;
+	p.bulk_end = std::min(bulk_end, n);
+	if (p.bulk_end < p.bulk_begin || (p.bulk_end - p.bulk_begin) % 4 != 0 || (n - p.bulk_end) % 4 != 0 || (p.bulk_end < n && p.bulk_end < n_matrix)) return false;
 	if (!pro.ranges.empty()) {
 		if ((const char*)pro.grad_base < (const char*)g_half || !aligned(pro.scratch, 16)) return false;
 		p.range_base = (size_t)((const half_t*)pro.grad_base - (const half_t*)g_half);
 		if (p.range_base % 4 != 0) return false;
 		for (const GridScatterRange& r : pro.ranges) {
-			if (r.grad_begin % 4 != 0 || r.n_elems % 4 != 0 || r.scratch_begin % 2 != 0 || p.range_base + r.grad_begin + r.n_elems > n || p.range_base + r.grad_begin < p.bulk_begin) return false;
+			if (r.grad_begin % 4 != 0 || r.n_elems % 4 != 0 || r.scratch_begin % 2 != 0 || p.range_base + r.grad_begin + r.n_elems > p.bulk_end || p.range_base + r.grad_begin < p.bulk_begin) return false;
 		}
 		for (bool moved = true; moved;) {
 			moved = false;
@@ -881,12 +883,45 @@
 		p.accumulate = pro.accumulate ? 1 : 0;
 	}
 	const AdamArgs a = make_adam_args(h, loss_scale, current_step);
-	const uint32_t bulk_blocks = div_round_up((uint32_t)((n - p.bulk_begin) / 4), PRO_THREADS * (uint32_t)PRO_Q);
+	p.bulk_begin = std::min(p.bulk_begin, p.bulk_end);
+	const uint32_t bulk_blocks = div_round_up((uint32_t)((p.bulk_end - p.bulk_begin) / 4), PRO_THREADS * (uint32_t)PRO_Q);
 	const dim3 grid(p.n_reduce_blocks + p.n_range_blocks + bulk_blocks);
 	if (steps16) hipLaunchKernelGGL(k_adam_prologue<uint16_t>, grid, dim3(PRO_THREADS), 0, stream, a, n, n_matrix, w_fp, (half_t*)w_half, (half_t*)g_half, m1, m2, (uint16_t*)steps, debias_table, p);
 	else hipLaunchKernelGGL(k_adam_prologue<uint32_t>, grid, dim3(PRO_THREADS), 0, stream, a, n, n_matrix, w_fp, (half_t*)w_half, (half_t*)g_half, m1, m2, (uint32_t*)steps, debias_table, p);
 	HIP_CHECK_THROW(hipGetLastError());
 	return true;
+}
+
+namespace {
+template <typename STEP_T>
+__global__ void __launch_bounds__(256) k_adam_range(const AdamArgs a, const size_t begin, const size_t end, const size_t n_matrix, float* __restrict__ w_fp, half_t* __restrict__ w,
+                                                    const half_t* __restrict__ g, float* __restrict__ m1, float* __restrict__ m2, STEP_T* __restrict__ steps, const float* __restrict__ debias_table) {
+	const float debias = debias_table[a.common_step];
+	const auto from_table = [&](const uint32_t t) { return debias_table[t]; };
+	const size_t stride = (size_t)gridDim.x * 1024;
+	for (size_t i4 = begin + ((size_t)blockIdx.x * 256 + threadIdx.x) * 4; i4 < end; i4 += stride) {
+		const h4 gv = *(const h4*)(g + i4);
+		adam_quad(a, from_table, debias, i4 < n_matrix, i4, gv, w_fp, w, m1, m2, steps);
+	}
+}
+}
+
+void adam_step_range(hipStream_t stream, const AdamHyper& h, size_t begin, size_t end, size_t n_matrix, float loss_scale, uint32_t current_step,
+                     float* w_fp, void* w_half, const void* g_half, float* m1, float* m2, void* steps, bool steps16, const float* debias_table, uint32_t wgs_per_cu) {
+	if (end <= begin) return;
+	const auto aligned = [](const void* ptr, size_t bytes) { return ((uintptr_t)ptr & (bytes - 1)) == 0; };
+	CHECK_THROW(begin % 4 == 0 && (end - begin) % 4 == 0 && aligned(w_fp, 16) && aligned(m1, 16) && aligned(m2, 16) && aligned(steps, steps16 ? 8 : 16) && aligned(w_half, 8) && aligned(g_half, 8));
+	static const uint32_t n_cus = [] {
+		int dev = 0, cus = 0;
+		if (hipGetDevice(&dev) != hipSuccess || hipDeviceGetAttribute(&cus, hipDeviceAttributeMultiprocessorCount, dev) != hipSuccess || cus <= 0) cus = 256;
+		return (uint32_t)cus;
+	}();
+	const AdamArgs a = make_adam_args(h, loss_scale, current_step);
+	const size_t quads = (end - begin) / 4;
+	const uint32_t blocks = (uint32_t)std::min<size_t>((size_t)n_cus * std::max(wgs_per_cu, 1u), (quads + 255) / 256);
+	if (steps16) hipLaunchKernelGGL(k_adam_range<uint16_t>, dim3(blocks), dim3(256), 0, stream, a, begin, end, n_matrix, w_fp, (half_t*)w_half, (const half_t*)g_half, m1, m2, (uint16_t*)steps, debias_table);
+	else hipLaunchKernelGGL(k_adam_range<uint32_t>, dim3(blocks), dim3(256), 0, stream, a, begin, end, n_matrix, w_fp, (half_t*)w_half, (const half_t*)g_half, m1, m2, (uint32_t*)steps, debias_table);
+	HIP_CHECK_THROW(hipGetLastError());
 }
 
 void adam_fill_debias_table(hipStream_t stream, float beta1, float beta2, uint32_t from, uint32_t to, float* table) {
diff --git a/tiny-cuda-nn_amd/csrc/model.h b/tiny-cuda-nn_amd/csrc/model.h
--- a/tiny-cuda-nn_amd/csrc/model.h
+++ b/tiny-cuda-nn_amd/csrc/model.h
@@ -207,10 +207,15 @@
 	bool reduce_carried = false;
 };
 
+struct ForwardSplit {
+	uint32_t split_level = 0;
+	hipEvent_t ready = nullptr;
+};
 struct ForwardPlan {
 	GridForwardRoute route;
 	const MlpPrepJob* prep_job = nullptr;
 	const GridItemMap* item_map = nullptr;
+	const ForwardSplit* split = nullptr;
 };
 
 class Encoding {
@@ -247,6 +252,7 @@
 	virtual uint64_t scatter_wide_fallbacks() { return 0; }
 	virtual uint64_t list_scatters() const { return 0; }
 	virtual GridForwardRoute forward_route(const Switches& sw, uint32_t n, bool as_planes, bool prepare_input_gradients, bool prepare_param_gradients) const { return {}; }
+	virtual bool grid_facts(GridFacts& out) const { return false; }
 	virtual Json hyperparams() const = 0;
 	bool fp32() const { return m_fp32; }
 	virtual bool set_max_level(float max_level) { return false; }
@@ -388,7 +394,7 @@
 		EncodingContext ctx;
 		if ((!out && !prepare_input_gradients) || padded_output_width() == 0 || n == 0) return ctx;
 		const GridForwardRoute route = plan ? plan->route : forward_route(switches(), n, false, prepare_input_gradients, prepare_param_gradients);
-		if (route.kernel == GridForwardKernel::Planes) return forward_planes(stream, route, n, x, params, out, plan->prep_job, plan->item_map);
+		if (route.kernel == GridForwardKernel::Planes) return forward_planes(stream, route, n, x, params, out, plan->prep_job, plan->item_map, plan->split);
 		if (route.kernel == GridForwardKernel::PlanesToRows) {
 			ArenaBuf planes{stream, (size_t)n * padded_output_width() * sizeof(uint16_t)};
 			ctx = forward_planes(stream, route, n, x, params, planes.data());
@@ -415,6 +421,7 @@
 	}
 
 	GridFacts facts() const { return GridFacts{&m_meta, m_fp32, m_scatter_levels_ok, m_any_binned, m_n_to_pad}; }
+	bool grid_facts(GridFacts& out) const override { out = facts(); return true; }
 	GridForwardRoute forward_route(const Switches& sw, uint32_t n, bool as_planes, bool prepare_input_gradients, bool prepare_param_gradients) const override {
 		return grid_forward_route(facts(), sw, n, as_planes, prepare_input_gradients, prepare_param_gradients);
 	}
@@ -423,20 +430,21 @@
 		DeviceBuf dev_work;
 		uint32_t max_items = 0, blocks_per_xcd = 0;
 	};
-	PlanesPlan& planes_plan(uint32_t n_, bool hit_lists) {
-		const uint32_t n = n_ | (hit_lists ? 0x80000000u : 0u);
+	PlanesPlan& planes_plan(uint32_t n_, bool hit_lists, uint32_t level_begin = 0, uint32_t level_end = MAX_N_LEVELS) {
+		level_end = std::min(level_end, m_meta.n_levels);
+		const uint64_t n = n_ | (hit_lists ? 0x80000000u : 0u) | (uint64_t)level_begin << 32 | (uint64_t)level_end << 40;
 		auto it = m_planes_plans.find(n);
 		if (it != m_planes_plans.end()) return *it->second;
 		auto plan = std::make_unique<PlanesPlan>();
 		std::vector<uint32_t> work;
-		grid_planes_plan(m_meta, n_, hit_lists, work, plan->max_items, plan->blocks_per_xcd);
+		grid_planes_plan(m_meta, n_, hit_lists, work, plan->max_items, plan->blocks_per_xcd, level_begin, level_end);
 		plan->dev_work.resize(work.size() * sizeof(uint32_t));
 		HIP_CHECK_THROW(hipMemcpy(plan->dev_work.data(), work.data(), work.size() * sizeof(uint32_t), hipMemcpyHostToDevice));
 		return *(m_planes_plans[n] = std::move(plan));
 	}
 
 	EncodingContext forward_planes(hipStream_t stream, const GridForwardRoute& route, uint32_t n, MatView x, const void* params, void* out_planes,
-	                               const MlpPrepJob* prep_job = nullptr, const GridItemMap* item_map = nullptr) {
+	                               const MlpPrepJob* prep_job = nullptr, const GridItemMap* item_map = nullptr, const ForwardSplit* split = nullptr) {
 		EncodingContext ctx;
 		CHECK_THROW(route.planned && route.kernel != GridForwardKernel::Rows);
 		ctx.route = route;
@@ -472,9 +480,22 @@
 			ctx.chunk_mask = ArenaBuf{stream, (size_t)m_meta.n_levels * grid_scatter_max_chunks() * (n / 64) * sizeof(uint64_t)};
 			ctx.n = n;
 		}
-		PlanesPlan& plan = planes_plan(n, want_lists);
-		grid_forward_planes(stream, m_meta, dev_meta(), plan.dev_work.as<uint32_t>(), plan.max_items, plan.blocks_per_xcd, n, x, params, out_planes, ctx.chunk_mask.as<uint64_t>(), prep_job,
-		                    want_lists ? &ctx.hit_lists : nullptr);
+		if (split && split->split_level > 0 && split->split_level < m_meta.n_levels) {
+			PlanesPlan& early = planes_plan(n, want_lists, 0, split->split_level);
+			PlanesPlan& late = planes_plan(n, want_lists, split->split_level, m_meta.n_levels);
+			GridHitLists early_lists = ctx.hit_lists;
+			early_lists.zero_counts = nullptr;
+			grid_forward_planes(stream, m_meta, dev_meta(), early.dev_work.as<uint32_t>(), early.max_items, early.blocks_per_xcd, n, x, params, out_planes, ctx.chunk_mask.as<uint64_t>(), prep_job,
+			                    want_lists ? &early_lists : nullptr);
+			HIP_CHECK_THROW(hipStreamWaitEvent(stream, split->ready, 0));
+			grid_forward_planes(stream, m_meta, dev_meta(), late.dev_work.as<uint32_t>(), late.max_items, late.blocks_per_xcd, n, x, params, out_planes, ctx.chunk_mask.as<uint64_t>(), nullptr,
+			                    want_lists ? &ctx.hit_lists : nullptr);
+		} else {
+			if (split) HIP_CHECK_THROW(hipStreamWaitEvent(stream, split->ready, 0));
+			PlanesPlan& plan = planes_plan(n, want_lists);
+			grid_forward_planes(stream, m_meta, dev_meta(), plan.dev_work.as<uint32_t>(), plan.max_items, plan.blocks_per_xcd, n, x, params, out_planes, ctx.chunk_mask.as<uint64_t>(), prep_job,
+			                    want_lists ? &ctx.hit_lists : nullptr);
+		}
 		if (m_n_to_pad) HIP_CHECK_THROW(hipMemsetAsync((uint16_t*)out_planes + (size_t)n * m_n_features, 0, (size_t)n * m_n_to_pad * sizeof(uint16_t), stream));
 		if (max_level_forward_active()) {
 			const uint32_t F = m_meta.n_features_per_level;
@@ -792,7 +813,7 @@
 	DeviceBuf m_dev_meta;
 	std::map<std::pair<uint32_t, const void*>, std::unique_ptr<ScatterPlan>> m_scatter_plans;
 	std::map<const void*, std::unique_ptr<HitCounters>> m_hit_counters;
-	std::map<uint32_t, std::unique_ptr<PlanesPlan>> m_planes_plans;
+	std::map<uint64_t, std::unique_ptr<PlanesPlan>> m_planes_plans;
 	bool m_scatter_levels_ok = true;
 	bool m_any_binned = false;
 	uint64_t m_list_scatters = 0;
@@ -1944,7 +1965,8 @@
 
 struct StepProfile {
 	enum Piece { Encode = 0, MlpKernel = 1, EncodingBackward = 2, Optimizer = 3, N_PIECES = 4 };
-	struct Sample { hipEvent_t begin[N_PIECES], end[N_PIECES]; bool used[N_PIECES]; };
+	static constexpr int OptimizerLate = 4, N_EVENTS = 5;
+	struct Sample { hipEvent_t begin[N_EVENTS], end[N_EVENTS]; bool used[N_EVENTS]; };
 	std::vector<Sample> samples;
 	bool armed = false;
 	Sample* current = nullptr;
@@ -1956,13 +1978,13 @@
 		armed = false;
 		samples.emplace_back();
 		current = &samples.back();
-		for (int i = 0; i < N_PIECES; ++i) {
+		for (int i = 0; i < N_EVENTS; ++i) {
 			current->used[i] = false;
 			HIP_CHECK_THROW(hipEventCreateWithFlags(&current->begin[i], 0x20000000u));
 			HIP_CHECK_THROW(hipEventCreateWithFlags(&current->end[i], 0x20000000u));
 		}
 	}
-	void mark(hipStream_t stream, Piece p, bool end) {
+	void mark(hipStream_t stream, int p, bool end) {
 		if (!current) return;
 		HIP_CHECK_THROW(hipEventRecord(end ? current->end[p] : current->begin[p], stream));
 		if (end) current->used[p] = true;
@@ -1972,10 +1994,11 @@
 		HIP_CHECK_THROW(hipStreamSynchronize(stream));
 		for (int i = 0; i < N_PIECES; ++i) ms[i] = 0.0f;
 		for (Sample& s : samples) {
-			for (int i = 0; i < N_PIECES; ++i) {
+			for (int i = 0; i < N_EVENTS; ++i) {
 				float t = 0.0f;
+				if (s.used[i] && i == OptimizerLate) HIP_CHECK_THROW(hipEventSynchronize(s.end[i]));
 				if (s.used[i]) HIP_CHECK_THROW(hipEventElapsedTime(&t, s.begin[i], s.end[i]));
-				ms[i] += t;
+				ms[i == OptimizerLate ? (int)Optimizer : i] += t;
 				(void)hipEventDestroy(s.begin[i]);
 				(void)hipEventDestroy(s.end[i]);
 			}
@@ -1986,7 +2009,7 @@
 	}
 	~StepProfile() {
 		for (Sample& s : samples)
-			for (int i = 0; i < N_PIECES; ++i) {
+			for (int i = 0; i < N_EVENTS; ++i) {
 				(void)hipEventDestroy(s.begin[i]);
 				(void)hipEventDestroy(s.end[i]);
 			}
@@ -2008,6 +2031,7 @@
 	void* gradients = nullptr;
 	GradientMode mode = GradientMode::Overwrite;
 	StepProfile* profile = nullptr;
+	const ForwardSplit* split = nullptr;
 };
 enum class OptimizerPlace { None, InReduce, Prologue, OwnLaunch };
 struct OptimizerOffer {
@@ -2032,6 +2056,7 @@
 	Precision precision() const override { return m_network->precision(); }
 	std::vector<std::pair<uint32_t, uint32_t>> layer_sizes() const override { return m_network->layer_sizes(); }
 	Encoding& encoding() { return *m_encoding; }
+	size_t n_network_params() const { return m_network->n_params(); }
 	Encoding* input_encoding() override { return m_encoding.get(); }
 	Network& network() { return *m_network; }
 
@@ -2229,14 +2254,16 @@
 		GridItemMap item_map;
 		const bool mapped = sw.listgrad_in_mlp && route.recorded == GridRecorded::HitLists && route.plane_features &&
 		                    mlp_train_item_map(mlp_train_plan(m_network->desc(), step_request(n, step, route.plane_features, 0, true, route.plane_features, false)), item_map);
-		fused_encode(stream, *ctx, n, input, step.params, route, step.dL_dinput != nullptr, step.mode != GradientMode::Ignore, sw.side_jobs, mapped ? &item_map : nullptr);
+		const bool split_here = step.split && route.kernel == GridForwardKernel::Planes;
+		if (step.split && !split_here) HIP_CHECK_THROW(hipStreamWaitEvent(stream, step.split->ready, 0));
+		fused_encode(stream, *ctx, n, input, step.params, route, step.dL_dinput != nullptr, step.mode != GradientMode::Ignore, sw.side_jobs, mapped ? &item_map : nullptr, split_here ? step.split : nullptr);
 		if (step.profile) step.profile->mark(stream, StepProfile::Encode, true);
 		fused_mlp_and_scatter(stream, sw, *ctx, n, input, step, optimizer);
 		return ctx;
 	}
 
 	void fused_encode(hipStream_t stream, Ctx& ctx, uint32_t n, MatView input, const void* params, const GridForwardRoute& route, bool prepare_input_gradients, bool prepare_param_gradients,
-	                  bool prep_image = false, const GridItemMap* item_map = nullptr) {
+	                  bool prep_image = false, const GridItemMap* item_map = nullptr, const ForwardSplit* split = nullptr) {
 		const _Float16* p = (const _Float16*)params;
 		const uint32_t n_net = (uint32_t)m_network->n_params();
 		if (m_network->layerwise()) throw std::runtime_error{"NetworkWithInputEncoding::fused_encode: a layer-by-layer network has no fused training step"};
@@ -2247,7 +2274,7 @@
 			return;
 		}
 		ctx.network_input = ArenaBuf{stream, (size_t)n * m_encoding->padded_output_width() * 2};
-		ForwardPlan plan{route, nullptr, item_map};
+		ForwardPlan plan{route, nullptr, item_map, split};
 		MlpPrepJob job;
 		if (route.plane_features && prep_image) {
 			ctx.image = ArenaBuf{stream, mlp_image_bytes(m_network->desc())};
@@ -2495,7 +2522,10 @@
 	virtual AdamInReduce begin_step_in_reduce(hipStream_t stream, float loss_scale, float* weights_full_precision, void* weights) {
 		throw std::runtime_error{"Optimizer: this optimizer's step cannot be applied by the slab reduction"};
 	}
-	virtual bool step_with_prologue(hipStream_t stream, float loss_scale, float* weights_full_precision, void* weights, void* gradients, const AdamPrologue& prologue) { return false; }
+	virtual bool step_with_prologue(hipStream_t stream, float loss_scale, float* weights_full_precision, void* weights, void* gradients, const AdamPrologue& prologue, size_t bulk_end) { return false; }
+	virtual void step_late_range(hipStream_t stream, float loss_scale, float* weights_full_precision, void* weights, const void* gradients, size_t begin, uint32_t wgs_per_cu) {
+		throw std::runtime_error{"Optimizer::step_late_range: this optimizer does not split its step"};
+	}
 	virtual float learning_rate() const = 0;
 	virtual void set_learning_rate(float val) = 0;
 	virtual uint32_t step_count() const = 0;
@@ -2603,15 +2633,21 @@
 	}
 
 	bool takes_prologue() const override { return !fp32_weights(); }
-	bool step_with_prologue(hipStream_t stream, float loss_scale, float* weights_full_precision, void* weights, void* gradients, const AdamPrologue& prologue) override {
+	bool step_with_prologue(hipStream_t stream, float loss_scale, float* weights_full_precision, void* weights, void* gradients, const AdamPrologue& prologue, size_t bulk_end) override {
 		if (fp32_weights() || switches().adam_prologue_refused) return false;
 		++m_current_step;
 		ensure_debias_table(stream);
 		ensure_step_width(stream);
 		if (adam_step_with_prologue(stream, m_h, m_n_weights, m_n_matrix, loss_scale, m_current_step, weights_full_precision, weights, gradients, m_first_moments.as<float>(),
-		                            m_second_moments.as<float>(), m_param_steps.data(), m_steps16, m_debias.as<float>(), prologue)) return true;
+		                            m_second_moments.as<float>(), m_param_steps.data(), m_steps16, m_debias.as<float>(), prologue, bulk_end)) return true;
 		--m_current_step;
 		return false;
+	}
+
+	void step_late_range(hipStream_t stream, float loss_scale, float* weights_full_precision, void* weights, const void* gradients, size_t begin, uint32_t wgs_per_cu) override {
+		CHECK_THROW(!fp32_weights() && begin <= m_n_weights);
+		adam_step_range(stream, m_h, begin, m_n_weights, m_n_matrix, loss_scale, m_current_step, weights_full_precision, weights, gradients, m_first_moments.as<float>(),
+		                m_second_moments.as<float>(), m_param_steps.data(), m_steps16, m_debias.as<float>(), wgs_per_cu);
 	}
 
 	static constexpr uint32_t NARROW_STEP_LIMIT = 65535;
@@ -3356,7 +3392,18 @@
 		initialize_params();
 	}
 
+	~Trainer() {
+		if (m_late_done) {
+			(void)hipEventSynchronize(m_late_done);
+			(void)hipEventDestroy(m_late_done);
+			(void)hipEventDestroy(m_early_done);
+		}
+	}
+	Trainer(const Trainer&) = delete;
+	Trainer& operator=(const Trainer&) = delete;
+
 	void initialize_params() {
+		join_deferred_host();
 		const size_t n = m_model->n_params();
 		m_optimizer->allocate(n, m_model->layer_sizes(), precision());
 		m_params_fp.resize(n * sizeof(float));
@@ -3374,6 +3421,7 @@
 
 	std::unique_ptr<TrainContext> forward(hipStream_t stream, float loss_scale, uint32_t n, MatView input, const float* target, const float* data_pdf,
 	                                      bool use_inference_params, bool prepare_input_gradients, const void* external_dL_dy) {
+		join_deferred(stream);
 		auto ctx = std::make_unique<TrainContext>();
 		ctx->n = n;
 		const uint32_t pw = m_model->padded_output_width();
@@ -3393,12 +3441,76 @@
 	}
 
 	void backward(hipStream_t stream, const TrainContext& ctx, uint32_t n, MatView input, MatViewMut* dL_dinput, bool use_inference_params, GradientMode mode) {
+		join_deferred(stream);
 		const_cast<TrainContext&>(ctx).materialize();
 		m_model->backward(stream, *ctx.model_ctx, n, input, ctx.output.data(), ctx.dL_doutput_ptr, dL_dinput, use_inference_params ? params_inference() : working_params(), m_grads.data(), mode);
 	}
 
 	size_t params_updated_in_flush() const { return m_params_updated_in_flush; }
 	size_t m_prologue_steps = 0;
+
+	static hipStream_t side_stream() {
+		static std::mutex mutex;
+		static std::map<int, hipStream_t> streams;
+		int device = 0;
+		HIP_CHECK_THROW(hipGetDevice(&device));
+		std::lock_guard<std::mutex> lock{mutex};
+		auto it = streams.find(device);
+		if (it != streams.end()) return it->second;
+		hipStream_t s = nullptr;
+		HIP_CHECK_THROW(hipStreamCreateWithFlags(&s, hipStreamNonBlocking));
+		return streams[device] = s;
+	}
+	void join_deferred(hipStream_t stream) {
+		if (!m_late.pending) return;
+		HIP_CHECK_THROW(hipStreamWaitEvent(stream, m_late_done, 0));
+		m_late.pending = false;
+	}
+	void join_deferred_host() {
+		if (!m_late.pending) return;
+		HIP_CHECK_THROW(hipEventSynchronize(m_late_done));
+		m_late.pending = false;
+	}
+	OptimizerOverlapPlan overlap_plan(hipStream_t stream, const Switches& sw, uint32_t n, OptimizerPlace place, const AdamPrologue& prologue, bool want_dL_dinput, GradientMode mode) {
+		OptimizerOverlapFacts f;
+		GridFacts grid;
+		if (m_model->encoding().grid_facts(grid)) f.grid = &grid;
+		f.forward_kernel = m_model->encoding().forward_route(sw, n, true, want_dL_dinput, mode != GradientMode::Ignore).kernel;
+		f.batch = n;
+		f.n_params = m_model->n_params();
+		f.n_matrix = m_model->n_network_params();
+		f.grid_begin = m_model->n_network_params();
+		f.shared = prologue.ranges.data();
+		f.n_shared = (uint32_t)prologue.ranges.size();
+		f.shared_base = prologue.ranges.empty() ? 0 : (size_t)((const uint16_t*)prologue.grad_base - (const uint16_t*)m_grads.data());
+		f.adam_in_prologue = place == OptimizerPlace::Prologue && prologue.pending && m_optimizer->n_weights() == f.n_params;
+		f.params_exposed = m_params_exposed;
+		if (stream) {
+			hipStreamCaptureStatus status = hipStreamCaptureStatusNone;
+			f.capturing = hipStreamIsCapturing(stream, &status) != hipSuccess || status != hipStreamCaptureStatusNone;
+		}
+		return optimizer_overlap_plan(f, sw);
+	}
+	void defer_late_half(hipStream_t stream, const Switches& sw, float loss_scale, uint32_t n, const OptimizerOverlapPlan& plan) {
+		if (!m_late_done) {
+			HIP_CHECK_THROW(hipEventCreateWithFlags(&m_early_done, hipEventDisableTiming | 0x20000000u));
+			HIP_CHECK_THROW(hipEventCreateWithFlags(&m_late_done, hipEventDisableTiming | 0x20000000u));
+		}
+		const hipStream_t side = side_stream();
+		HIP_CHECK_THROW(hipEventRecord(m_early_done, stream));
+		HIP_CHECK_THROW(hipStreamWaitEvent(side, m_early_done, 0));
+		m_profile.mark(side, StepProfile::OptimizerLate, false);
+		m_optimizer->step_late_range(side, loss_scale, m_params_fp.as<float>(), m_params.data(), m_grads.data(), plan.early_end, sw.adam_overlap_wgs);
+		m_profile.mark(side, StepProfile::OptimizerLate, true);
+		HIP_CHECK_THROW(hipEventRecord(m_late_done, side));
+		m_late.pending = true, m_late.n = n, m_late.stream = stream, m_late.split_level = plan.split_level;
+		++m_deferred_steps;
+	}
+	size_t deferred_steps() const { return m_deferred_steps; }
+	uint32_t profile_collect(hipStream_t stream, float* ms) {
+		join_deferred(stream);
+		return m_profile.collect(stream, ms);
+	}
 
 	OptimizerPlace optimizer_place(bool run_optimizer, GradientMode mode, bool want_dL_dinput) const {
 		if (!run_optimizer) return OptimizerPlace::None;
@@ -3422,6 +3534,7 @@
 	}
 
 	void optimizer_step(hipStream_t stream, float loss_scale) {
+		join_deferred(stream);
 		m_model->invalidate_live_image();
 		m_optimizer->step(stream, loss_scale, m_params_fp.as<float>(), working_params(), m_grads.data(), m_fp32 ? GradientPrecision::Fp32 : GradientPrecision::Fp16);
 	}
@@ -3431,7 +3544,9 @@
 		const float loss_scale = m_fp32 ? 1.0f : LOSS_SCALE_FP16;
 		std::unique_ptr<TrainContext> ctx;
 		const bool other_weights = use_inference_params && params_inference() != working_params();
-		if (!m_fp32 && m_model->fused_step_supported(n) && (external_dL_dy || loss_in_fused_kernel(m_loss)) && !other_weights) {
+		const bool fused = !m_fp32 && m_model->fused_step_supported(n) && (external_dL_dy || loss_in_fused_kernel(m_loss)) && !other_weights;
+		if (!(fused && n == m_late.n && stream == m_late.stream)) join_deferred(stream);
+		if (fused) {
 			ctx = std::make_unique<TrainContext>();
 			ctx->n = n;
 			const uint32_t pw = m_model->padded_output_width();
@@ -3477,13 +3592,28 @@
 			step.params = m_params.data(), step.gradients = m_grads.data();
 			step.mode = mode;
 			step.profile = &m_profile;
+			ForwardSplit split;
+			if (m_late.pending) {
+				split.split_level = m_late.split_level, split.ready = m_late_done;
+				step.split = &split;
+				m_late.pending = false;
+			}
 			ctx->model_ctx = m_model->fused_step(stream, n, input, step, offer);
 			if (m_params_exposed || (place != OptimizerPlace::None && !m_model->live_image_kept())) m_model->invalidate_live_image();
 			if (place != OptimizerPlace::None) {
+				bool stepped = false;
 				m_profile.mark(stream, StepProfile::Optimizer, false);
 				if (place == OptimizerPlace::InReduce) m_params_updated_in_flush = m_model->n_params();
-				else if (prologue.pending && m_optimizer->step_with_prologue(stream, loss_scale, m_params_fp.as<float>(), m_params.data(), m_grads.data(), prologue)) ++m_prologue_steps;
-				else {
+				else if (prologue.pending) {
+					const Switches sw = switches();
+					const OptimizerOverlapPlan overlap = overlap_plan(stream, sw, n, place, prologue, dL_dinput != nullptr, mode);
+					if (m_optimizer->step_with_prologue(stream, loss_scale, m_params_fp.as<float>(), m_params.data(), m_grads.data(), prologue, overlap.active ? overlap.early_end : m_model->n_params())) {
+						++m_prologue_steps;
+						if (overlap.active) defer_late_half(stream, sw, loss_scale, n, overlap);
+						stepped = true;
+					}
+				}
+				if (place != OptimizerPlace::InReduce && !stepped) {
 					if (prologue.pending) run_prologue_alone(stream, prologue);
 					m_optimizer->step(stream, loss_scale, m_params_fp.as<float>(), m_params.data(), m_grads.data());
 				}
@@ -3516,17 +3646,20 @@
 	void inference(hipStream_t stream, uint32_t n, MatView input, MatViewMut output, bool use_inference_params) {
 		Model::check_batch(n);
 		if (n == 0) return;
+		join_deferred(stream);
 		m_model->inference_f32(stream, n, input, output, use_inference_params ? params_inference() : working_params());
 	}
 
 	void inference_mixed_precision(hipStream_t stream, uint32_t n, MatView input, void* output_half, bool use_inference_params) {
 		Model::check_batch(n);
 		if (n == 0) return;
+		join_deferred(stream);
 		m_model->inference(stream, n, input, output_half, use_inference_params ? params_inference() : working_params());
 	}
 
 	void set_params_full_precision(const float* params, size_t n_params, bool device_ptr) {
 		if (n_params != m_model->n_params()) throw std::runtime_error{"Can't set fp params because buffer has the wrong size."};
+		join_deferred_host();
 		m_model->invalidate_live_image();
 		HIP_CHECK_THROW(hipMemcpy(m_params_fp.data(), params, sizeof(float) * n_params, device_ptr ? hipMemcpyDeviceToDevice : hipMemcpyHostToDevice));
 		if (!m_fp32) cast_float_to_half(nullptr, n_params, m_params_fp.as<float>(), m_params.data());
@@ -3537,6 +3670,7 @@
 	void set_params(const void* params, size_t n_params, bool device_ptr) {
 		if (n_params != m_model->n_params()) throw std::runtime_error{"Can't set params because buffer has the wrong size."};
 		if (m_fp32) return set_params_full_precision((const float*)params, n_params, device_ptr);
+		join_deferred_host();
 		m_model->invalidate_live_image();
 		HIP_CHECK_THROW(hipMemcpy(m_params.data(), params, 2 * n_params, device_ptr ? hipMemcpyDeviceToDevice : hipMemcpyHostToDevice));
 		cast_half_to_float(nullptr, n_params, m_params.data(), m_params_fp.as<float>());
@@ -3549,6 +3683,7 @@
 	}
 
 	Json serialize(bool serialize_optimizer) {
+		join_deferred_host();
 		HIP_CHECK_THROW(hipDeviceSynchronize());
 		const size_t n = m_model->n_params();
 		Json data = Json::object();
@@ -3560,6 +3695,7 @@
 	}
 
 	void deserialize(const Json& data) {
+		join_deferred_host();
 		const std::string type = data.value("params_type", "__half");
 		const std::vector<uint8_t> bytes = binary_of(data["params_binary"]);
 		if (type == "float") {
@@ -3615,7 +3751,7 @@
 	uint64_t list_gradient_tails() const { return m_model->list_gradient_tails(); }
 	size_t prologue_steps() const { return m_prologue_steps; }
 	const char* last_step_kernel() const { return m_last_step_kernel; }
-	void* param_gradients() const { return m_grads.data(); }
+	void* param_gradients() { join_deferred_host(); return m_grads.data(); }
 
 private:
 	std::unique_ptr<NetworkWithInputEncoding> m_model;
@@ -3628,7 +3764,11 @@
 	const char* m_last_step_kernel = "";
 	bool m_params_exposed = false;
 	const bool m_fp32 = false;
+	struct { bool pending = false; uint32_t n = 0, split_level = 0; hipStream_t stream = nullptr; } m_late;
+	hipEvent_t m_early_done = nullptr, m_late_done = nullptr;
+	size_t m_deferred_steps = 0;
 	void expose_params() {
+		join_deferred_host();
 		m_params_exposed = true;
 		m_model->invalidate_live_image();
 	}
diff --git a/tiny-cuda-nn_amd/csrc/tcnn_common.h b/tiny-cuda-nn_amd/csrc/tcnn_common.h
--- a/tiny-cuda-nn_amd/csrc/tcnn_common.h
+++ b/tiny-cuda-nn_amd/csrc/tcnn_common.h
@@ -2,6 +2,7 @@
 
 #include <hip/hip_runtime.h>
 
+#include <algorithm>
 #include <cstddef>
 #include <cstdint>
 #include <stdexcept>
@@ -54,6 +55,9 @@
 	bool mlp_fast = true;
 	uint32_t mlp_prio = 1;
 	bool listgrad_in_mlp = true;
+	bool adam_overlap = true;
+	int adam_overlap_split = -1;
+	uint32_t adam_overlap_wgs = 2;
 	bool mlp_layerwise = false;
 };
 Switches switches();
@@ -102,7 +106,8 @@
 void grid_planes_to_rows(hipStream_t stream, const GridMeta& meta, uint32_t n, uint32_t width, const void* planes, void* rows, uint32_t row_stride);
 void grid_rows_to_planes(hipStream_t stream, const GridMeta& meta, uint32_t n, uint32_t width, const void* rows, uint32_t row_stride, void* planes);
 uint32_t grid_planes_spt(const GridMeta& meta);
-void grid_planes_plan(const GridMeta& meta, uint32_t n, bool hit_lists, std::vector<uint32_t>& work, uint32_t& max_items, uint32_t& blocks_per_xcd);
+void grid_planes_plan(const GridMeta& meta, uint32_t n, bool hit_lists, std::vector<uint32_t>& work, uint32_t& max_items, uint32_t& blocks_per_xcd, uint32_t level_begin = 0,
+                      uint32_t level_end = MAX_N_LEVELS);
 struct MlpPrepJob;
 inline constexpr uint32_t grid_hit_mask_shift(uint32_t n_pos_dims) { return 32u - (1u << n_pos_dims); }
 constexpr uint32_t GRID_HIT_COUNT_STRIDE = 64;
@@ -217,6 +222,69 @@
 	if (r.kernel == GridForwardKernel::Planes) r.plane_features = F;
 	if (param_gradients && r.lds) r.recorded = (r.kernel != GridForwardKernel::Rows && grid_hit_lists_wanted(g, sw, n)) ? GridRecorded::HitLists : GridRecorded::BitPlanes;
 	return r;
+}
+
+struct OptimizerOverlapFacts {
+	const GridFacts* grid = nullptr;
+	GridForwardKernel forward_kernel = GridForwardKernel::Rows;
+	uint32_t batch = 0;
+	size_t n_params = 0, n_matrix = 0;
+	size_t grid_begin = 0;
+	const GridScatterRange* shared = nullptr;
+	uint32_t n_shared = 0;
+	size_t shared_base = 0;
+	bool adam_in_prologue = false;
+	bool params_exposed = false;
+	bool capturing = false;
+};
+struct OptimizerOverlapPlan {
+	bool active = false;
+	uint32_t split_level = 0;
+	size_t early_end = 0, n_params = 0;
+};
+constexpr double OVERLAP_ADAM_US_PER_PARAM = 32.0 / 6.0e6;
+constexpr double OVERLAP_FWD_US_PER_SAMPLE_GATHER = 16.0e-6, OVERLAP_FWD_US_PER_SAMPLE_CACHED = 9.5e-6;
+constexpr size_t OVERLAP_CACHED_BYTES = 256u << 10;
+constexpr size_t OVERLAP_L2_BYTES = (size_t)4 << 20;
+constexpr double OVERLAP_MIN_HIDDEN_US = 10.0;
+inline double overlap_forward_level_us(const GridMeta& m, uint32_t level, uint32_t batch) {
+	const size_t bytes = (size_t)m.levels[level].size * m.n_features_per_level * 2;
+	return (double)batch * (bytes > OVERLAP_CACHED_BYTES ? OVERLAP_FWD_US_PER_SAMPLE_GATHER : OVERLAP_FWD_US_PER_SAMPLE_CACHED);
+}
+inline OptimizerOverlapPlan optimizer_overlap_plan(const OptimizerOverlapFacts& f, const Switches& sw) {
+	OptimizerOverlapPlan none;
+	if (!sw.adam_overlap || !f.grid || !f.adam_in_prologue || f.params_exposed || f.capturing || f.forward_kernel != GridForwardKernel::Planes) return none;
+	const GridMeta& m = *f.grid->meta;
+	const uint32_t F = m.n_features_per_level, L = m.n_levels;
+	if (f.grid->any_binned || L < 2) return none;
+	for (uint32_t l = 0; l < L; ++l) {
+		if ((size_t)m.levels[l].size * F * 2 > OVERLAP_L2_BYTES || m.levels[l].scatter_binned) return none;
+	}
+	const auto level_begin = [&](uint32_t l) { return f.grid_begin + (size_t)m.levels[l].offset * F; };
+	uint32_t first = 1;
+	size_t floor_param = f.n_matrix;
+	for (uint32_t r = 0; r < f.n_shared; ++r) floor_param = std::max(floor_param, f.shared_base + f.shared[r].grad_begin + f.shared[r].n_elems);
+	const auto allowed = [&](uint32_t s) { return s >= 1 && s < L && level_begin(s) % 4 == 0 && (f.n_params - level_begin(s)) % 4 == 0 && level_begin(s) >= floor_param; };
+	OptimizerOverlapPlan p;
+	p.n_params = f.n_params;
+	if (sw.adam_overlap_split >= 0) {
+		const uint32_t s = (uint32_t)sw.adam_overlap_split;
+		if (!allowed(s)) return none;
+		p.active = true, p.split_level = s, p.early_end = level_begin(s);
+		return p;
+	}
+	double best = 0;
+	for (uint32_t s = first; s < L; ++s) {
+		if (!allowed(s)) continue;
+		double fwd = 0;
+		for (uint32_t l = 0; l < s; ++l) fwd += overlap_forward_level_us(m, l, f.batch);
+		const double adam = (double)(f.n_params - level_begin(s)) * OVERLAP_ADAM_US_PER_PARAM;
+		const double hidden = std::min(fwd, adam);
+		if (hidden > best) best = hidden, p.split_level = s, p.early_end = level_begin(s);
+	}
+	if (best < OVERLAP_MIN_HIDDEN_US) return none;
+	p.active = true;
+	return p;
 }
 
 enum class GridDyForm : uint32_t { Rows, Planes, Records };
@@ -472,7 +540,10 @@
 	int reduce_accumulate = 0;
 };
 bool adam_step_with_prologue(hipStream_t stream, const AdamHyper& h, size_t n, size_t n_matrix, float loss_scale, uint32_t current_step,
-                             float* w_fp, void* w_half, void* g_half, float* m1, float* m2, void* steps, bool steps16, const float* debias_table, const AdamPrologue& p);
+                             float* w_fp, void* w_half, void* g_half, float* m1, float* m2, void* steps, bool steps16, const float* debias_table, const AdamPrologue& p,
+                             size_t bulk_end = ~(size_t)0);
+void adam_step_range(hipStream_t stream, const AdamHyper& h, size_t begin, size_t end, size_t n_matrix, float loss_scale, uint32_t current_step,
+                     float* w_fp, void* w_half, const void* g_half, float* m1, float* m2, void* steps, bool steps16, const float* debias_table, uint32_t wgs_per_cu);
 void adam_step(hipStream_t stream, const AdamHyper& h, size_t n, size_t n_matrix, float loss_scale, uint32_t current_step,
                float* w_fp, void* w_half, const void* gradients, float* m1, float* m2, void* steps, bool steps16, const float* debias_table,
                GradientPrecision precision = GradientPrecision::Fp16, Precision weight_precision = Precision::Fp16);
diff --git a/tiny-cuda-nn_amd/tinycudann/_C.py b/tiny-cuda-nn_amd/tinycudann/_C.py
--- a/tiny-cuda-nn_amd/tinycudann/_C.py
+++ b/tiny-cuda-nn_amd/tinycudann/_C.py
@@ -112,6 +112,7 @@
     "tcnn_trainer_image_preps": (C.c_size_t, [_vp]),
     "tcnn_trainer_scatter_wide_fallbacks": (C.c_size_t, [_vp]),
     "tcnn_trainer_optimizer_prologue_steps": (C.c_size_t, [_vp]),
+    "tcnn_trainer_deferred_optimizer_steps": (C.c_size_t, [_vp]),
     "tcnn_trainer_list_scatters": (C.c_size_t, [_vp]),
     "tcnn_trainer_list_gradient_tails": (C.c_size_t, [_vp]),
     "tcnn_trainer_last_step_kernel": (_cp, [_vp]),
diff --git a/tiny-cuda-nn_amd/tinycudann/native.py b/tiny-cuda-nn_amd/tinycudann/native.py
--- a/tiny-cuda-nn_amd/tinycudann/native.py
+++ b/tiny-cuda-nn_amd/tinycudann/native.py
@@ -111,6 +111,9 @@
     def optimizer_prologue_steps(self):
         return int(_C.lib.tcnn_trainer_optimizer_prologue_steps(self._h))
 
+    def deferred_optimizer_steps(self):
+        return int(_C.lib.tcnn_trainer_deferred_optimizer_steps(self._h))
+
     def list_scatters(self):
         return int(_C.lib.tcnn_trainer_list_scatters(self._h))
 
```

Result: slower. 1.092 billion (-22.6%).
